# PRBonn/semantic_suma

Hardware: NVIDIA B200
Metric: scans_per_sec (higher is better)
Workload: dtype f32

## Files before the change

include/suma_b200.h:

```cpp
#ifndef SUMA_B200_H_
#define SUMA_B200_H_

#include <stdint.h>

#ifdef __cplusplus
extern "C" {
#endif

#define SB_VERSION 100

typedef enum sb_status {
  SB_OK = 0,
  SB_ERR_INVALID = -1,
  SB_ERR_CUDA = -2,
  SB_ERR_NOMEM = -3,
  SB_ERR_CAPACITY = -4,
  SB_ERR_STATE = -5,
  SB_ERR_NOGPU = -6
} sb_status;

typedef struct sb_params {
  int32_t data_width, data_height;
  float data_fov_up, data_fov_down;
  float min_depth, max_depth;
  int32_t model_width, model_height;
  float model_fov_up, model_fov_down;
  float model_min_depth, model_max_depth;
  int32_t max_iterations;
  double stopping_threshold, delta;
  float icp_max_distance, icp_max_angle;
  int32_t weighting;
  float factor;
  int32_t initialize_identity;
  int32_t bilinear_sampling;
  int32_t fallback_mode;
  float fallback_max_distance, fallback_max_angle;
  int32_t compose_rendering;
  float max_loop_closure_distance;
  float min_radius, max_radius, max_angle;
  float map_max_distance, map_max_angle;
  int32_t unstable_age, confidence_mode;
  float confidence_threshold;
  float p_stable, p_prior, sigma_angle, sigma_distance;
  int32_t use_stability, active_timestamps;
  float max_weight;
  int32_t weighting_scheme, averaging_scheme, update_always;
  int32_t submap_dimension;
  float submap_extent;
  int32_t partial_extraction;
  int32_t label_offset_quirk;
  int32_t render_after_update;
} sb_params;

typedef struct sb_surfel {
  float x, y, z, radius;
  float nx, ny, nz, confidence;
  uint32_t timestamp;
  float color, weight, count;
  float r, g, b, w;
} sb_surfel;

typedef struct sb_ctx sb_ctx;
typedef struct sb_frame sb_frame;

enum { SB_MAP_VERTEX = 0, SB_MAP_NORMAL = 1, SB_MAP_SEMANTIC = 2 };
enum { SB_FRAME_OLD = 0, SB_FRAME_NEW = 1, SB_FRAME_COMPOSED = 2 };
enum { SB_SLAM_CURRENT = 0, SB_SLAM_LAST = 1, SB_SLAM_CURRENT_MODEL = 2, SB_SLAM_LAST_MODEL = 3 };

int sb_default_params(sb_params* p);
int sb_create(const sb_params* p, int device, sb_ctx** out);
int sb_destroy(sb_ctx* ctx);
int sb_reset(sb_ctx* ctx);
int sb_set_params(sb_ctx* ctx, const sb_params* p);
const char* sb_last_error(const sb_ctx* ctx);
int sb_synchronize(sb_ctx* ctx);
int sb_device_count(void);
void* sb_stream(sb_ctx* ctx);
uint64_t sb_launch_count(const sb_ctx* ctx);

int sb_frame_create(sb_ctx* ctx, int width, int height, sb_frame** out);
int sb_frame_destroy(sb_frame* f);
int sb_frame_copy(sb_frame* dst, const sb_frame* src);
int sb_frame_download(const sb_frame* f, int which, float* dst );
int sb_frame_upload(sb_frame* f, int which, const float* src );
int sb_frame_size(const sb_frame* f, int* width, int* height);

int sb_preprocess(sb_ctx* ctx, const float* pts4, const float* labels, const float* probs, uint32_t n,
                  uint32_t timestamp, int pts_on_device, sb_frame* out);

int sb_map_render(sb_ctx* ctx, const float pose_old[16], const float pose_new[16], float conf_thr, sb_frame* out);
int sb_map_render_active(sb_ctx* ctx, const float pose[16], float conf_thr);
int sb_map_render_inactive(sb_ctx* ctx, const float pose[16], float conf_thr);
int sb_map_render_composed(sb_ctx* ctx, const float pose_old[16], const float pose_new[16], float conf_thr);
int sb_map_frame(sb_ctx* ctx, int which, sb_frame** out);

int sb_icp_jacobian(sb_ctx* ctx, const sb_frame* data, const sb_frame* model, const double pose[16], int iteration,
                    float max_distance, float max_angle_deg, int row_begin, int row_end, double out48[48],
                    int64_t raw32[32]);
void sb_icp_unpack(const int64_t raw32[32], double out48[48]);

int sb_icp_minimize(sb_ctx* ctx, const sb_frame* data, const sb_frame* model, const double T0[16], int max_iter,
                    double eps, double delta, float max_distance, float max_angle_deg, double pose_out[16],
                    double out48[48], int* iters, double* history, int* history_len);
void sb_se3_exp(const double x[6], double T[16]);
void sb_se3_log(const double T[16], double x[6]);
int sb_ldlt_solve6(const double A[36], const double b[6], double x[6]);
int sb_gn_step(const double out48[48], double last_error, double eps, double delta, double pose[16], double dx[6]);

int sb_map_update(sb_ctx* ctx, const float pose[16], const sb_frame* frame);
int sb_map_update_poses(sb_ctx* ctx, const float* poses16, uint32_t count);
int sb_map_size(sb_ctx* ctx, uint32_t* n);
int sb_map_timestamp(sb_ctx* ctx, uint32_t* t);
int sb_map_download(sb_ctx* ctx, sb_surfel* dst, uint32_t cap, uint32_t* n);
int sb_map_upload(sb_ctx* ctx, const sb_surfel* src, uint32_t n, uint32_t timestamp);
int sb_map_set_pose(sb_ctx* ctx, uint32_t t, const float pose[16]);
int sb_map_update_debug(sb_ctx* ctx, uint32_t* index_map, float* radius_map4, uint8_t* integrated,
                        uint32_t* n_updated, uint32_t* n_new);
int sb_map_submap_origin(sb_ctx* ctx, int32_t* i, int32_t* j, uint32_t* pending);

int sb_process_scan(sb_ctx* ctx, const float* pts4, const float* labels, const float* probs, uint32_t n,
                    int pts_on_device);
int sb_prefetch_scan(sb_ctx* ctx, const float* pts4, const float* labels, const float* probs, uint32_t n);
typedef struct sb_loop_params {
  float search_distance;
  float min_trajectory_distance;
  int32_t min_verifications;
  float residual_threshold;
  float outlier_threshold;
  float valid_threshold;
} sb_loop_params;
typedef struct sb_loop_info {
  uint32_t enabled, loop_count, time_without_loop_closure, candidates_tested, loop_edges_added, unverified;
  uint32_t already_verified, found_candidate, use_candidate, optimisation_requested;
  int32_t last_added_candidate;
  uint32_t n_edges, n_poses;
  float valid_ratio, outlier_ratio, rel_error;
  double residual_old, residual_new;
  double current_pose_old[16];
} sb_loop_info;
typedef struct sb_loop_edge {
  int32_t from, to;
  double rel_pose[16];
} sb_loop_edge;
void sb_default_loop_params(sb_loop_params* p);
int sb_set_loop_closure(sb_ctx* ctx, int enabled, const sb_loop_params* p );
int sb_get_loop_info(sb_ctx* ctx, sb_loop_info* out);
int sb_get_loop_edges(sb_ctx* ctx, sb_loop_edge* dst, uint32_t cap, uint32_t* n_total);
int sb_integrate_loop_closures(sb_ctx* ctx, const double* poses16, uint32_t n, uint32_t* integrated);
int sb_set_current_pose(sb_ctx* ctx, const double pose[16]);

int sb_get_pose(sb_ctx* ctx, double pose[16]);
int sb_get_last_pose(sb_ctx* ctx, double pose[16]);
int sb_timestamp(sb_ctx* ctx, uint32_t* t);
int sb_slam_frame(sb_ctx* ctx, int which, sb_frame** out);
int sb_get_statistics(sb_ctx* ctx, double stats[16]);

int sb_profile_enable(sb_ctx* ctx, int on);
int sb_profile_kernels(void);
const char* sb_profile_name(int id);
int sb_profile_collect(sb_ctx* ctx, double* total_ms, uint64_t* count, int cap);

int sb_comm_export(sb_ctx* ctx, uint8_t handle[64]);
int sb_comm_init(sb_ctx* ctx, int rank, int nranks, const uint8_t* handles , int row_begin,
                 int row_end);
int sb_comm_shutdown(sb_ctx* ctx);
typedef int (*sb_allreduce_fn)(void* user, int64_t* sums32);
int sb_comm_set_callback(sb_ctx* ctx, sb_allreduce_fn fn, void* user, int row_begin, int row_end);

#ifdef __cplusplus
}
#endif
#endif
```

semantic_suma_b200/api.py:

```python
import ctypes as C
import os

import numpy as np

from . import build as _build

SB_OK = 0
_ERRORS = {-1: "SB_ERR_INVALID", -2: "SB_ERR_CUDA", -3: "SB_ERR_NOMEM", -4: "SB_ERR_CAPACITY", -5: "SB_ERR_STATE",
           -6: "SB_ERR_NOGPU"}


class SumaError(RuntimeError):
    pass


class LoopParams(C.Structure):
    _fields_ = [("search_distance", C.c_float), ("min_trajectory_distance", C.c_float), ("min_verifications", C.c_int32),
                ("residual_threshold", C.c_float), ("outlier_threshold", C.c_float), ("valid_threshold", C.c_float)]


class LoopInfo(C.Structure):
    _fields_ = [(n, C.c_uint32) for n in ("enabled", "loop_count", "time_without_loop_closure", "candidates_tested",
                                          "loop_edges_added", "unverified", "already_verified", "found_candidate",
                                          "use_candidate", "optimisation_requested")] + \
               [("last_added_candidate", C.c_int32), ("n_edges", C.c_uint32), ("n_poses", C.c_uint32),
                ("valid_ratio", C.c_float), ("outlier_ratio", C.c_float), ("rel_error", C.c_float),
                ("residual_old", C.c_double), ("residual_new", C.c_double), ("current_pose_old", C.c_double * 16)]


class LoopEdge(C.Structure):
    _fields_ = [("from_", C.c_int32), ("to", C.c_int32), ("rel_pose", C.c_double * 16)]


class Params(C.Structure):
    _fields_ = [
        ("data_width", C.c_int32), ("data_height", C.c_int32),
        ("data_fov_up", C.c_float), ("data_fov_down", C.c_float),
        ("min_depth", C.c_float), ("max_depth", C.c_float),
        ("model_width", C.c_int32), ("model_height", C.c_int32),
        ("model_fov_up", C.c_float), ("model_fov_down", C.c_float),
        ("model_min_depth", C.c_float), ("model_max_depth", C.c_float),
        ("max_iterations", C.c_int32),
        ("stopping_threshold", C.c_double), ("delta", C.c_double),
        ("icp_max_distance", C.c_float), ("icp_max_angle", C.c_float),
        ("weighting", C.c_int32), ("factor", C.c_float),
        ("initialize_identity", C.c_int32), ("bilinear_sampling", C.c_int32),
        ("fallback_mode", C.c_int32),
        ("fallback_max_distance", C.c_float), ("fallback_max_angle", C.c_float),
        ("compose_rendering", C.c_int32), ("max_loop_closure_distance", C.c_float),
        ("min_radius", C.c_float), ("max_radius", C.c_float), ("max_angle", C.c_float),
        ("map_max_distance", C.c_float), ("map_max_angle", C.c_float),
        ("unstable_age", C.c_int32), ("confidence_mode", C.c_int32),
        ("confidence_threshold", C.c_float),
        ("p_stable", C.c_float), ("p_prior", C.c_float), ("sigma_angle", C.c_float), ("sigma_distance", C.c_float),
        ("use_stability", C.c_int32), ("active_timestamps", C.c_int32),
        ("max_weight", C.c_float),
        ("weighting_scheme", C.c_int32), ("averaging_scheme", C.c_int32), ("update_always", C.c_int32),
        ("submap_dimension", C.c_int32), ("submap_extent", C.c_float), ("partial_extraction", C.c_int32),
        ("label_offset_quirk", C.c_int32), ("render_after_update", C.c_int32),
    ]

    def as_dict(self):
        return {k: getattr(self, k) for k, _ in self._fields_}


XML_KEYS = {
    "max iterations": "max_iterations", "stopping threshold": "stopping_threshold", "icp-max-distance": "icp_max_distance",
    "icp-max-angle": "icp_max_angle", "fallback-max-distance": "fallback_max_distance",
    "fallback-max-angle": "fallback_max_angle", "map-max-distance": "map_max_distance",
    "map-max-angle": "map_max_angle", "submap-dimension": "submap_dimension", "submap-extent": "submap_extent",
    "partial-extraction": "partial_extraction",
}
_WEIGHTING = {"none": 0, "huber": 1, "turkey": 2, "stability": 3}

SURFEL_DTYPE = np.dtype([
    ("x", "f4"), ("y", "f4"), ("z", "f4"), ("radius", "f4"),
    ("nx", "f4"), ("ny", "f4"), ("nz", "f4"), ("confidence", "f4"),
    ("timestamp", "u4"), ("color", "f4"), ("weight", "f4"), ("count", "f4"),
    ("r", "f4"), ("g", "f4"), ("b", "f4"), ("w", "f4"),
])

_lib = None


def library_path():
    return _build.LIB


def lib(build_if_missing=True):
    global _lib
    if _lib is not None:
        return _lib
    path = _build.LIB
    if build_if_missing:
        try:
            path = _build.build()
        except Exception as e:
            if not os.path.exists(_build.LIB):
                raise SumaError("libsuma_b200.so is missing and could not be built: %s" % e)
    if not os.path.exists(path):
        raise SumaError("libsuma_b200.so not found at %s (run python -m semantic_suma_b200.build)" % path)
    L = C.CDLL(path)
    vp, u32, i32, f32, f64 = C.c_void_p, C.c_uint32, C.c_int32, C.c_float, C.c_double
    pf, pd, pv = C.POINTER(C.c_float), C.POINTER(C.c_double), C.POINTER(C.c_void_p)
    sig = {
        "sb_default_params": [C.POINTER(Params)],
        "sb_create": [C.POINTER(Params), C.c_int, pv],
        "sb_destroy": [vp], "sb_reset": [vp], "sb_set_params": [vp, C.POINTER(Params)], "sb_synchronize": [vp],
        "sb_frame_create": [vp, C.c_int, C.c_int, pv], "sb_frame_destroy": [vp], "sb_frame_copy": [vp, vp],
        "sb_frame_download": [vp, C.c_int, vp], "sb_frame_upload": [vp, C.c_int, vp],
        "sb_frame_size": [vp, C.POINTER(C.c_int), C.POINTER(C.c_int)],
        "sb_preprocess": [vp, vp, vp, vp, u32, u32, C.c_int, vp],
        "sb_map_render": [vp, pf, pf, f32, vp], "sb_map_render_active": [vp, pf, f32],
        "sb_map_render_inactive": [vp, pf, f32], "sb_map_render_composed": [vp, pf, pf, f32],
        "sb_map_frame": [vp, C.c_int, pv],
        "sb_icp_jacobian": [vp, vp, vp, pd, C.c_int, f32, f32, C.c_int, C.c_int, pd, C.POINTER(C.c_int64)],
        "sb_icp_minimize": [vp, vp, vp, pd, C.c_int, f64, f64, f32, f32, pd, pd, C.POINTER(C.c_int), pd,
                            C.POINTER(C.c_int)],
        "sb_gn_step": [pd, f64, f64, f64, pd, pd],
        "sb_ldlt_solve6": [pd, pd, pd],
        "sb_map_update": [vp, pf, vp], "sb_map_update_poses": [vp, pf, u32], "sb_map_set_pose": [vp, u32, pf],
        "sb_map_size": [vp, C.POINTER(u32)], "sb_map_timestamp": [vp, C.POINTER(u32)],
        "sb_map_download": [vp, vp, u32, C.POINTER(u32)], "sb_map_upload": [vp, vp, u32, u32],
        "sb_map_update_debug": [vp, vp, vp, vp, C.POINTER(u32), C.POINTER(u32)],
        "sb_map_submap_origin": [vp, C.POINTER(i32), C.POINTER(i32), C.POINTER(u32)],
        "sb_process_scan": [vp, vp, vp, vp, u32, C.c_int], "sb_prefetch_scan": [vp, vp, vp, vp, u32],
        "sb_set_loop_closure": [vp, C.c_int, vp], "sb_get_loop_info": [vp, vp], "sb_get_loop_edges": [vp, vp, u32, C.POINTER(u32)],
        "sb_set_current_pose": [vp, pd], "sb_default_loop_params": [vp],
        "sb_integrate_loop_closures": [vp, pd, u32, C.POINTER(u32)],
        "sb_get_pose": [vp, pd], "sb_get_last_pose": [vp, pd], "sb_timestamp": [vp, C.POINTER(u32)], "sb_slam_frame": [vp, C.c_int, pv],
        "sb_get_statistics": [vp, pd],
        "sb_comm_export": [vp, vp], "sb_comm_init": [vp, C.c_int, C.c_int, vp, C.c_int, C.c_int],
        "sb_comm_shutdown": [vp],
        "sb_comm_set_callback": [vp, vp, vp, C.c_int, C.c_int],
        "sb_profile_enable": [vp, C.c_int], "sb_profile_collect": [vp, pd, C.POINTER(C.c_uint64), C.c_int],
        "sb_profile_kernels": [],
    }
    for name, args in sig.items():
        fn = getattr(L, name)
        fn.argtypes = args
        fn.restype = C.c_int
    L.sb_last_error.argtypes = [vp]; L.sb_last_error.restype = C.c_char_p
    L.sb_stream.argtypes = [vp]; L.sb_stream.restype = vp
    L.sb_launch_count.argtypes = [vp]; L.sb_launch_count.restype = C.c_uint64
    L.sb_device_count.argtypes = []; L.sb_device_count.restype = C.c_int
    L.sb_profile_name.argtypes = [C.c_int]; L.sb_profile_name.restype = C.c_char_p
    L.sb_se3_exp.argtypes = [pd, pd]; L.sb_se3_exp.restype = None
    L.sb_se3_log.argtypes = [pd, pd]; L.sb_se3_log.restype = None
    L.sb_icp_unpack.argtypes = [C.POINTER(C.c_int64), pd]; L.sb_icp_unpack.restype = None
    _lib = L
    return L


EXPORTED_SYMBOLS = [
    "sb_default_params", "sb_create", "sb_destroy", "sb_reset", "sb_set_params", "sb_last_error", "sb_synchronize",
    "sb_device_count", "sb_stream", "sb_launch_count", "sb_frame_create", "sb_frame_destroy", "sb_frame_copy",
    "sb_frame_download", "sb_frame_upload", "sb_frame_size", "sb_preprocess", "sb_map_render", "sb_map_render_active",
    "sb_map_render_inactive", "sb_map_render_composed", "sb_map_frame", "sb_icp_jacobian", "sb_icp_unpack",
    "sb_icp_minimize", "sb_se3_exp", "sb_se3_log", "sb_ldlt_solve6", "sb_gn_step", "sb_map_update",
    "sb_map_update_poses", "sb_map_size", "sb_map_timestamp", "sb_map_download", "sb_map_upload", "sb_map_set_pose",
    "sb_map_update_debug", "sb_map_submap_origin", "sb_process_scan", "sb_prefetch_scan", "sb_get_pose", "sb_get_last_pose", "sb_timestamp", "sb_slam_frame",
    "sb_get_statistics", "sb_comm_export", "sb_comm_init", "sb_comm_shutdown", "sb_comm_set_callback",
    "sb_profile_enable", "sb_default_loop_params", "sb_set_loop_closure", "sb_get_loop_info", "sb_get_loop_edges",
    "sb_set_current_pose", "sb_integrate_loop_closures",
    "sb_profile_kernels", "sb_profile_name", "sb_profile_collect",
]


def default_params(**kw):
    p = Params()
    lib().sb_default_params(C.byref(p))
    for k, v in kw.items():
        k = XML_KEYS.get(k, k)
        if k == "weighting" and isinstance(v, str):
            v = _WEIGHTING[v]
        if not hasattr(p, k):
            raise KeyError(k)
        setattr(p, k, v)
    return p


def colmajor(T, dtype):
    return np.ascontiguousarray(np.asarray(T, dtype=dtype).T).reshape(16)


def from_colmajor(a):
    return np.asarray(a).reshape(4, 4).T.copy()


def _fp(a):
    return a.ctypes.data_as(C.POINTER(C.c_float))


def _dp(a):
    return a.ctypes.data_as(C.POINTER(C.c_double))


def _vp(a):
    if a is None:
        return None
    return C.c_void_p(a.ctypes.data)


class Context:

    def __init__(self, params, device=0):
        self.params = params
        self.h = C.c_void_p()
        rc = lib().sb_create(C.byref(params), device, C.byref(self.h))
        if rc != SB_OK:
            raise SumaError("sb_create failed: %s (libsuma_b200 needs a CUDA device; there is no CPU fallback)" %
                            _ERRORS.get(rc, rc))

    def check(self, rc, what=""):
        if rc != SB_OK:
            msg = lib().sb_last_error(self.h)
            raise SumaError("%s: %s %s" % (what, _ERRORS.get(rc, rc), msg.decode() if msg else ""))

    def close(self):
        if self.h:
            lib().sb_destroy(self.h)
            self.h = C.c_void_p()

    def __del__(self):
        try:
            self.close()
        except Exception:
            pass

    def synchronize(self):
        self.check(lib().sb_synchronize(self.h), "synchronize")

    def launch_count(self):
        return int(lib().sb_launch_count(self.h))

    def stream(self):
        return lib().sb_stream(self.h)

    def profile(self, on):
        self.check(lib().sb_profile_enable(self.h, 1 if on else 0), "profile_enable")

    def profile_collect(self):
        n = lib().sb_profile_kernels()
        ms = np.zeros(n); cnt = np.zeros(n, np.uint64)
        self.check(lib().sb_profile_collect(self.h, _dp(ms), cnt.ctypes.data_as(C.POINTER(C.c_uint64)), n), "profile")
        return {lib().sb_profile_name(i).decode(): (float(ms[i]), int(cnt[i])) for i in range(n) if cnt[i]}

    def set_params(self, params):
        self.check(lib().sb_set_params(self.h, C.byref(params)), "set_params")
        self.params = params


class Frame:

    def __init__(self, ctx, width=None, height=None, handle=None):
        self.ctx = ctx
        self._own = handle is None
        if handle is None:
            self.h = C.c_void_p()
            ctx.check(lib().sb_frame_create(ctx.h, width, height, C.byref(self.h)), "frame_create")
        else:
            self.h = C.c_void_p(handle)
        w, h = C.c_int(), C.c_int()
        lib().sb_frame_size(self.h, C.byref(w), C.byref(h))
        self.width, self.height = w.value, h.value

    def __del__(self):
        if getattr(self, "_own", False) and self.h and self.ctx.h:
            lib().sb_frame_destroy(self.h)
            self.h = None

    def _get(self, which):
        a = np.empty((self.height, self.width, 4), np.float32)
        self.ctx.check(lib().sb_frame_download(self.h, which, _vp(a)), "frame_download")
        return a

    def _set(self, which, a):
        a = np.ascontiguousarray(a, np.float32)
        assert a.shape == (self.height, self.width, 4)
        self.ctx.check(lib().sb_frame_upload(self.h, which, _vp(a)), "frame_upload")

    vertex_map = property(lambda s: s._get(0), lambda s, a: s._set(0, a))
    normal_map = property(lambda s: s._get(1), lambda s, a: s._set(1, a))
    semantic_map = property(lambda s: s._get(2), lambda s, a: s._set(2, a))

    def maps(self):
        return self._get(0), self._get(1), self._get(2)

    def upload(self, maps):
        for i, a in enumerate(maps):
            self._set(i, a)

    def copy(self, other):
        self.ctx.check(lib().sb_frame_copy(self.h, other.h), "frame_copy")


class Preprocessing:

    def __init__(self, ctx):
        self.ctx = ctx

    def process(self, points, frame, labels=None, probs=None, timestamp=100):
        pts = np.ascontiguousarray(points, np.float32)
        lab = None if labels is None else np.ascontiguousarray(labels, np.float32)
        prb = None if probs is None else np.ascontiguousarray(probs, np.float32)
        self.ctx.check(lib().sb_preprocess(self.ctx.h, _vp(pts), _vp(lab), _vp(prb), pts.shape[0], timestamp, 0, frame.h),
                       "preprocess")


class Frame2Model:

    def __init__(self, ctx, max_distance=None, max_angle=None):
        self.ctx = ctx
        p = ctx.params
        self.max_distance = p.icp_max_distance if max_distance is None else max_distance
        self.max_angle = p.icp_max_angle if max_angle is None else max_angle
        self.pose_ = np.eye(4)
        self.iteration_ = 0
        self.current = self.last = None
        self.out48 = np.zeros(48)
        self.raw32 = np.zeros(32, np.int64)

    def setData(self, current, last):
        self.current, self.last = current, last
        self.iteration_ = 0

    def initialize(self, T0):
        self.pose_ = np.array(T0, np.float64)

    def num_parameters(self):
        return 6

    def jacobianProducts(self, rows=None):
        pc = colmajor(self.pose_, np.float64)
        r0, r1 = rows if rows is not None else (0, self.ctx.params.data_height)
        self.ctx.check(lib().sb_icp_jacobian(self.ctx.h, self.current.h, self.last.h, _dp(pc), self.iteration_,
                                             self.max_distance, self.max_angle, r0, r1, _dp(self.out48),
                                             self.raw32.ctypes.data_as(C.POINTER(C.c_int64))), "icp_jacobian")
        o = self.out48
        return o[43], o[:36].reshape(6, 6).T.copy(), o[36:42].copy()

    def increment(self, delta):
        T = np.zeros(16)
        d = np.ascontiguousarray(delta, np.float64)
        lib().sb_se3_exp(_dp(d), _dp(T))
        self.pose_ = from_colmajor(T) @ self.pose_
        self.iteration_ += 1

    def pose(self):
        return self.pose_

    def valid(self):
        return int(self.out48[42])

    def outlier(self):
        return int(self.out48[44])

    def inlier(self):
        return int(self.out48[42]) - int(self.out48[44])

    def invalid(self):
        return int(self.out48[46])

    def inlier_residual(self):
        return float(np.float32(self.out48[45]))


class LieGaussNewton:

    def __init__(self, ctx):
        self.ctx = ctx
        p = ctx.params
        self.maxIter, self.epsilon, self.delta = p.max_iterations, p.stopping_threshold, p.delta
        self.Tk_ = np.eye(4)
        self.k_ = 0
        self.history_ = []
        self.out48 = np.zeros(48)

    def minimize(self, F, T0):
        T0c = colmajor(T0, np.float64)
        pose = np.zeros(16); out48 = np.zeros(48); it = C.c_int(0); hl = C.c_int(0)
        bounded = 1 <= self.maxIter <= 256
        hist = np.zeros((self.maxIter + 1) * 16 if bounded else 16)
        self.ctx.check(lib().sb_icp_minimize(self.ctx.h, F.current.h, F.last.h, _dp(T0c), self.maxIter, self.epsilon,
                                             self.delta, F.max_distance, F.max_angle, _dp(pose), _dp(out48),
                                             C.byref(it), _dp(hist) if bounded else None, C.byref(hl)), "icp_minimize")
        if not bounded:
            hl.value = 0
        self.Tk_ = from_colmajor(pose)
        self.k_ = it.value
        self.out48 = out48
        self.history_ = [from_colmajor(hist[16 * i:16 * i + 16]) for i in range(hl.value)]
        F.pose_ = self.Tk_.copy()
        F.out48 = out48
        return 0

    def minimize_host(self, F, T0):
        F.initialize(T0)
        last_error = float(np.finfo(np.float32).max)
        self.history_ = []
        k = 0
        while True:
            self.history_.append(F.pose().copy())
            if self.maxIter > 0 and k >= self.maxIter:
                break
            F.jacobianProducts()
            pose = colmajor(F.pose_, np.float64); dx = np.zeros(6)
            res = lib().sb_gn_step(_dp(F.out48), last_error, self.epsilon, self.delta, _dp(pose), _dp(dx))
            F.pose_ = from_colmajor(pose)
            F.iteration_ += 1
            last_error = F.out48[43]
            if res == 0:
                break
            k += 1
        self.Tk_, self.k_ = F.pose_.copy(), k
        return 0

    def pose(self):
        return self.Tk_

    def iterationCount(self):
        return self.k_

    def history(self):
        return self.history_


class SurfelMap:

    def __init__(self, ctx):
        self.ctx = ctx

    def update(self, pose, frame):
        pc = colmajor(pose, np.float32)
        self.ctx.check(lib().sb_map_update(self.ctx.h, _fp(pc), frame.h), "map_update")

    def render(self, pose_old, pose_new, frame, confidence_threshold):
        po, pn = colmajor(pose_old, np.float32), colmajor(pose_new, np.float32)
        self.ctx.check(lib().sb_map_render(self.ctx.h, _fp(po), _fp(pn), confidence_threshold, frame.h), "map_render")

    def render_active(self, pose, confidence_threshold):
        pc = colmajor(pose, np.float32)
        self.ctx.check(lib().sb_map_render_active(self.ctx.h, _fp(pc), confidence_threshold), "render_active")

    def render_inactive(self, pose, confidence_threshold):
        pc = colmajor(pose, np.float32)
        self.ctx.check(lib().sb_map_render_inactive(self.ctx.h, _fp(pc), confidence_threshold), "render_inactive")

    def render_composed(self, pose_old, pose_new, confidence_threshold):
        po, pn = colmajor(pose_old, np.float32), colmajor(pose_new, np.float32)
        self.ctx.check(lib().sb_map_render_composed(self.ctx.h, _fp(po), _fp(pn), confidence_threshold), "render_composed")

    def _frame(self, which):
        h = C.c_void_p()
        self.ctx.check(lib().sb_map_frame(self.ctx.h, which, C.byref(h)), "map_frame")
        return Frame(self.ctx, handle=h.value)

    def oldMapFrame(self):
        return self._frame(0)

    def newMapFrame(self):
        return self._frame(1)

    def composedFrame(self):
        return self._frame(2)

    def size(self):
        n = C.c_uint32()
        lib().sb_map_size(self.ctx.h, C.byref(n))
        return n.value

    def timestamp(self):
        n = C.c_uint32()
        lib().sb_map_timestamp(self.ctx.h, C.byref(n))
        return n.value

    def getAllSurfels(self):
        n = self.size()
        a = np.zeros(max(n, 1), SURFEL_DTYPE)
        k = C.c_uint32()
        self.ctx.check(lib().sb_map_download(self.ctx.h, _vp(a), n, C.byref(k)), "map_download")
        return a[:k.value]

    def upload(self, surfels, timestamp):
        a = np.ascontiguousarray(surfels, SURFEL_DTYPE)
        self.ctx.check(lib().sb_map_upload(self.ctx.h, _vp(a), a.shape[0], timestamp), "map_upload")

    def set_pose(self, t, pose):
        pc = colmajor(pose, np.float32)
        self.ctx.check(lib().sb_map_set_pose(self.ctx.h, t, _fp(pc)), "map_set_pose")

    def updatePoses(self, poses):
        a = np.ascontiguousarray(np.stack([colmajor(p, np.float32) for p in poses]), np.float32)
        self.ctx.check(lib().sb_map_update_poses(self.ctx.h, _fp(a), len(poses)), "update_poses")

    def update_debug(self):
        H, W = self.ctx.params.data_height, self.ctx.params.data_width
        idx = np.zeros((H, W), np.uint32); rad = np.zeros((H, W, 4), np.float32); integ = np.zeros((H, W), np.uint8)
        nu, nn = C.c_uint32(), C.c_uint32()
        self.ctx.check(lib().sb_map_update_debug(self.ctx.h, _vp(idx), _vp(rad), _vp(integ), C.byref(nu), C.byref(nn)),
                       "update_debug")
        return idx, rad, integ, nu.value, nn.value

    def submap_origin(self):
        i, j, p = C.c_int32(), C.c_int32(), C.c_uint32()
        lib().sb_map_submap_origin(self.ctx.h, C.byref(i), C.byref(j), C.byref(p))
        return i.value, j.value, p.value

    def reset(self):
        self.ctx.check(lib().sb_reset(self.ctx.h), "reset")


class SurfelMapping:

    def __init__(self, params, device=0):
        self.ctx = Context(params, device)
        self.map_ = SurfelMap(self.ctx)

    def enableLoopClosure(self, enabled=True, **kw):
        lp = LoopParams()
        lib().sb_default_loop_params(C.byref(lp))
        for k, v in kw.items():
            if not hasattr(lp, k):
                raise KeyError(k)
            setattr(lp, k, v)
        self.ctx.check(lib().sb_set_loop_closure(self.ctx.h, 1 if enabled else 0, C.byref(lp)), "set_loop_closure")

    def getLoopInfo(self):
        li = LoopInfo()
        self.ctx.check(lib().sb_get_loop_info(self.ctx.h, C.byref(li)), "get_loop_info")
        d = {n: getattr(li, n) for n, _ in LoopInfo._fields_ if n != "current_pose_old"}
        d["valid_ratio"] = np.float32(d["valid_ratio"]); d["outlier_ratio"] = np.float32(d["outlier_ratio"])
        d["rel_error"] = np.float32(d["rel_error"])
        d["current_pose_old"] = from_colmajor(np.array(li.current_pose_old))
        return d

    def getLoopEdges(self):
        n = C.c_uint32(0)
        self.ctx.check(lib().sb_get_loop_edges(self.ctx.h, None, 0, C.byref(n)), "get_loop_edges")
        arr = (LoopEdge * max(n.value, 1))()
        self.ctx.check(lib().sb_get_loop_edges(self.ctx.h, arr, n.value, C.byref(n)), "get_loop_edges")
        return [(arr[i].from_, arr[i].to, from_colmajor(np.array(arr[i].rel_pose))) for i in range(n.value)]

    def integrateLoopClosures(self, poses=None):
        n = C.c_uint32(0)
        if poses is None:
            self.ctx.check(lib().sb_integrate_loop_closures(self.ctx.h, None, 0, C.byref(n)), "integrate_loop_closures")
        else:
            a = np.ascontiguousarray([colmajor(P, np.float64) for P in poses], np.float64)
            self.ctx.check(lib().sb_integrate_loop_closures(self.ctx.h, _dp(a), a.shape[0], C.byref(n)),
                           "integrate_loop_closures")
        return int(n.value)

    def setCurrentPose(self, pose):
        self.ctx.check(lib().sb_set_current_pose(self.ctx.h, _dp(colmajor(pose, np.float64))), "set_current_pose")

    def processScan(self, points, labels=None, probs=None, on_device=False):
        if on_device:
            pp, pl, pq, n = points
            rc = lib().sb_process_scan(self.ctx.h, C.c_void_p(pp), C.c_void_p(pl) if pl else None,
                                       C.c_void_p(pq) if pq else None, n, 1)
        else:
            pts = np.ascontiguousarray(points, np.float32)
            lab = None if labels is None else np.ascontiguousarray(labels, np.float32)
            prb = None if probs is None else np.ascontiguousarray(probs, np.float32)
            rc = lib().sb_process_scan(self.ctx.h, _vp(pts), _vp(lab), _vp(prb), pts.shape[0], 0)
        self.ctx.check(rc, "process_scan")

    def process_scan_raw(self, ptr_pts, ptr_labels, ptr_probs, n, on_device):
        rc = lib().sb_process_scan(self.ctx.h, C.c_void_p(ptr_pts), C.c_void_p(ptr_labels) if ptr_labels else None,
                                   C.c_void_p(ptr_probs) if ptr_probs else None, n, 1 if on_device else 0)
        self.ctx.check(rc, "process_scan")

    def prefetch_scan_raw(self, ptr_pts, ptr_labels, ptr_probs, n):
        rc = lib().sb_prefetch_scan(self.ctx.h, C.c_void_p(ptr_pts), C.c_void_p(ptr_labels) if ptr_labels else None,
                                    C.c_void_p(ptr_probs) if ptr_probs else None, n)
        self.ctx.check(rc, "prefetch_scan")

    def getCurrentPose(self):
        a = np.zeros(16)
        lib().sb_get_pose(self.ctx.h, _dp(a))
        return from_colmajor(a)

    def getLastPose(self):
        a = np.zeros(16)
        lib().sb_get_last_pose(self.ctx.h, _dp(a))
        return from_colmajor(a)

    def timestamp(self):
        t = C.c_uint32()
        lib().sb_timestamp(self.ctx.h, C.byref(t))
        return t.value

    def getMap(self):
        return self.map_

    def _frame(self, which):
        h = C.c_void_p()
        self.ctx.check(lib().sb_slam_frame(self.ctx.h, which, C.byref(h)), "slam_frame")
        return Frame(self.ctx, handle=h.value)

    def getCurrentFrame(self):
        return self._frame(0)

    def getLastFrame(self):
        return self._frame(1)

    def getCurrentModelFrame(self):
        return self._frame(2)

    def getLastModelFrame(self):
        return self._frame(3)

    def getStatistics(self):
        a = np.zeros(16)
        lib().sb_get_statistics(self.ctx.h, _dp(a))
        return {"num_iterations": a[0], "F": a[1], "inlier": a[2], "outlier": a[3], "invalid": a[4],
                "inlier_residual": a[5], "track_loss": a[6], "surfels": a[7], "preprocessing-time": a[8],
                "icp-time": a[9], "mapping-time": a[10], "complete-time": a[11]}

    def reset(self):
        self.ctx.check(lib().sb_reset(self.ctx.h), "reset")
```

semantic_suma_b200/csrc/sb_api.cu:

```cuda
#include <chrono>
#include <cmath>
#include <cstddef>
#include <cstdio>
#include <cstdlib>
#include <map>
#include <string>
#include <utility>
#include <vector>

#include "sb_gn.cuh"
#include "sb_internal.cuh"
#include "../../include/suma_b200_loop.hpp"

using namespace sb;

struct sb_frame {
  sb_ctx* ctx;
  FrameDev d;
  float4* base;
};

struct DevTile {
  uint32_t slot = 0;
  bool known = false;
  uint32_t base = 0, count = 0;
};

struct sb_ctx {
  int device = 0;
  int sm_count = 148;
  cudaStream_t stream = nullptr;
  sb_params p;
  KParams kp;
  std::string err;
  uint64_t launches = 0;
  Profiler prof;

  PrepKeys prep;
  bool prepped_for_update = false;
  float4* d_pts = nullptr;
  float* d_labels = nullptr;
  float* d_probs = nullptr;
  size_t pts_cap = 0;
  struct PrefetchSlot {
    float4* pts = nullptr;
    float* labels = nullptr;
    float* probs = nullptr;
    const float* host_pts = nullptr;
    uint32_t n = 0;
    bool has_labels = false, has_probs = false, valid = false, in_use = false;
    cudaEvent_t done = nullptr;
    cudaEvent_t released = nullptr;
    bool has_released = false;
  };
  PrefetchSlot prefetch[3];
  cudaStream_t copy_stream = nullptr;

  GnState* gn = nullptr;
  GnState* gn2 = nullptr;
  long long* acc32 = nullptr;
  long long* acc_slots = nullptr;
  unsigned int* ticket = nullptr;
  void* h_pinned = nullptr;
  int icp_blocks = 296;
  int icp_coop_blocks = 0;
  unsigned int epoch_base = 1;
  unsigned long long* gn_pub = nullptr;
  int gn_use_cache = 1;
  bool close_loops = false;
  suma_b200::loop::State loop;
  double lastPose_old[16];

  SurfelPlanes A{}, T{}, G{}, X{};
  uint8_t* keep = nullptr;
  uint32_t* block_counts = nullptr;
  uint32_t* block_offsets = nullptr;
  unsigned long long* lb_desc = nullptr;
  uint32_t* lb_ticket = nullptr;
  uint32_t lb_gen = 0;
  uint32_t* d_counts = nullptr;
  float* poses = nullptr;
  float* poses_inv = nullptr;
  std::vector<float> h_poses, h_poses_inv;
  float* Mtab_old = nullptr;
  float* Mtab_new = nullptr;
  unsigned long long* key_old = nullptr;
  unsigned long long* key_new = nullptr;
  unsigned long long* key_comp = nullptr;
  unsigned long long* key_index = nullptr;
  float4* radius_map = nullptr;
  uint8_t* integrated = nullptr;
  uint32_t* group_counts = nullptr;
  sb_frame* f_old = nullptr;
  sb_frame* f_new = nullptr;
  sb_frame* f_comp = nullptr;
  uint32_t n_host = 0;
  uint32_t n_upper = 0;
  char* result_block = nullptr;
  PoseDev* pd = nullptr;
  uint32_t n_updated = 0, n_new = 0;
  uint32_t map_timestamp = 0;
  int32_t origin_i = 0, origin_j = 0;
  std::vector<std::pair<int32_t, int32_t>> extraction;
  std::map<std::pair<int32_t, int32_t>, DevTile> tiles;
  SurfelPlanes pool{};
  uint32_t* d_pool_top = nullptr;
  uint2* d_tile_rec = nullptr;
  uint32_t n_slots = 0;
  bool tiles_pending = false;

  struct RenderKey {
    float pose_old[16], pose_new[16];
    float conf_thr;
    uint32_t map_timestamp;
    uint64_t map_version;
    int compose;
    const sb_frame* out;
  } rkey{};
  bool rkey_valid = false;
  uint64_t map_version = 0;
  uint64_t renders_skipped = 0;

  sb_frame* cur = nullptr;
  sb_frame* last = nullptr;
  sb_frame* cur_model = nullptr;
  sb_frame* last_model = nullptr;
  uint32_t timestamp = 0;
  double currentPose[16], lastPose[16], currentPose_old[16], currentPose_new[16], lastIncrement[16];
  float confidence_threshold = 0.f, log_unstable_slam = 0.f;
  double stats[16];
  uint32_t trackLoss = 0;
  bool cur_has_semantics = false, last_has_semantics = false;

  long long* mailbox = nullptr;
  unsigned int* comm_epoch = nullptr;
  CommDev comm{};
  bool comm_on = false;
  sb_allreduce_fn comm_cb = nullptr;
  void* comm_cb_user = nullptr;
  int row_begin = 0, row_end = 0;
  std::vector<void*> peer_ptrs;
};

namespace {

int fail(sb_ctx* c, int code, const std::string& msg) {
  if (c) c->err = msg;
  return code;
}

#define SB_CUDA(ctx, call)                                                                              \
  do {                                                                                                  \
    cudaError_t e__ = (call);                                                                           \
    if (e__ != cudaSuccess)                                                                             \
      return fail(ctx, SB_ERR_CUDA, std::string(#call) + ": " + cudaGetErrorString(e__));               \
  } while (0)

Launch L_(sb_ctx* c) { return Launch{c->stream, &c->launches, &c->prof}; }

void ident_d(double* M) {
  for (int i = 0; i < 16; ++i) M[i] = (i % 5 == 0) ? 1.0 : 0.0;
}
Mat4 mat4_from(const float* m) {
  Mat4 r;
  memcpy(r.m, m, 64);
  return r;
}
void cast_f(const double* M, float* F) {
  for (int i = 0; i < 16; ++i) F[i] = (float)M[i];
}
double now_s() {
  return std::chrono::duration<double>(std::chrono::steady_clock::now().time_since_epoch()).count();
}
float deg2rad_f(float d) { return d * (float)(3.14159265358979323846 / 180.0); }

void derive(sb_ctx* c) {
  const sb_params& p = c->p;
  KParams& k = c->kp;
  memset(&k, 0, sizeof(k));
  k.W = p.data_width; k.H = p.data_height; k.Wm = p.model_width; k.Hm = p.model_height;
  k.fov_up = fabsf(p.data_fov_up); k.fov = fabsf(p.data_fov_up) + fabsf(p.data_fov_down);
  k.min_depth = p.min_depth; k.max_depth = p.max_depth;
  k.m_fov_up = fabsf(p.model_fov_up); k.m_fov = fabsf(p.model_fov_up) + fabsf(p.model_fov_down);
  k.m_min_depth = p.model_min_depth; k.m_max_depth = p.model_max_depth;
  k.weighting = p.weighting; k.bilinear = p.bilinear_sampling; k.factor = p.factor;
  k.use_stability = p.use_stability; k.unstable_age = p.unstable_age; k.confidence_mode = p.confidence_mode;
  k.active_timestamps = p.active_timestamps; k.weighting_scheme = p.weighting_scheme;
  k.averaging_scheme = p.averaging_scheme; k.update_always = p.update_always;
  k.confidence_threshold = p.confidence_threshold; k.p_stable = p.p_stable;
  k.p_unstable = 1.0f - p.p_stable;
  k.log_prior = (float)log(p.p_prior / (1.0 - p.p_prior));
  k.log_unstable = (float)log(k.p_unstable / (1.0 - k.p_unstable));
  k.sigma_angle = p.sigma_angle; k.sigma_distance = p.sigma_distance; k.max_weight = p.max_weight;
  float vfov = fabsf(p.data_fov_up) + fabsf(p.data_fov_down);
  float vpix = (float)tan(0.5f * ((double)vfov * 3.14159265358979323846 / 180.0) / (uint32_t)p.data_height);
  float hpix = (float)tan(0.5f * ((double)360.0f * 3.14159265358979323846 / 180.0) / (uint32_t)p.data_width);
  k.pixel_size = vpix > hpix ? vpix : hpix;
  k.min_radius = p.min_radius; k.max_radius = p.max_radius;
  k.radconf_angle_thresh = (float)cos((double)deg2rad_f(p.max_angle));
  k.update_angle_thresh = (float)sin((double)deg2rad_f(p.map_max_angle));
  k.map_max_distance = p.map_max_distance;
  k.max_loop_closure_distance = p.max_loop_closure_distance;
  k.label_offset_quirk = p.label_offset_quirk;
  c->confidence_threshold = p.confidence_threshold;
  float pu = 0.1f;
  c->log_unstable_slam = logf(pu / (1.0f - pu));
}

int alloc_planes(sb_ctx* c, SurfelPlanes* s, size_t n) {
  float4* base = nullptr;
  SB_CUDA(c, cudaMalloc(&base, n * 4 * sizeof(float4)));
  s->p0 = base; s->p1 = base + n; s->p2 = base + 2 * n; s->p3 = base + 3 * n;
  return SB_OK;
}
void free_planes(SurfelPlanes* s) {
  if (s->p0) cudaFree(s->p0);
  s->p0 = s->p1 = s->p2 = s->p3 = nullptr;
}

int frame_create(sb_ctx* c, int w, int h, sb_frame** out) {
  if (!c || w <= 0 || h <= 0 || !out) return fail(c, SB_ERR_INVALID, "frame_create: bad arguments");
  sb_frame* f = new sb_frame();
  f->ctx = c;
  size_t P = (size_t)w * h;
  cudaError_t e = cudaMalloc(&f->base, P * 3 * sizeof(float4));
  if (e != cudaSuccess) {
    delete f;
    return fail(c, SB_ERR_NOMEM, std::string("frame alloc: ") + cudaGetErrorString(e));
  }
  cudaMemsetAsync(f->base, 0, P * 3 * sizeof(float4), c->stream);
  f->d.W = w; f->d.H = h;
  f->d.vertex = f->base; f->d.normal = f->base + P; f->d.semantic = f->base + 2 * P;
  *out = f;
  return SB_OK;
}

int release_buffers(sb_ctx* c) {
  cudaFree(c->prep.img[0]); cudaFree(c->prep.img[1]);
  cudaFree(c->d_pts); cudaFree(c->d_labels); cudaFree(c->d_probs);
  cudaFree(c->gn); cudaFree(c->gn2); cudaFree(c->acc_slots); cudaFree(c->ticket); cudaFree(c->gn_pub);
  if (c->h_pinned) cudaFreeHost(c->h_pinned);
  free_planes(&c->A); free_planes(&c->T); free_planes(&c->G); free_planes(&c->X); free_planes(&c->pool);
  cudaFree(c->d_pool_top); cudaFree(c->d_tile_rec);
  cudaFree(c->keep); cudaFree(c->block_counts); cudaFree(c->block_offsets);
  cudaFree(c->lb_desc); cudaFree(c->lb_ticket);
  cudaFree(c->poses); cudaFree(c->poses_inv); cudaFree(c->Mtab_old); cudaFree(c->Mtab_new);
  cudaFree(c->key_old); cudaFree(c->key_index); cudaFree(c->radius_map); cudaFree(c->integrated); cudaFree(c->group_counts);
  sb_frame* fr[] = {c->f_old, c->f_new, c->f_comp, c->cur, c->last, c->cur_model, c->last_model};
  for (sb_frame* f : fr)
    if (f) {
      cudaFree(f->base);
      delete f;
    }
  cudaFree(c->mailbox);
  cudaFree(c->comm_epoch);
  cudaFree(c->result_block);
  return SB_OK;
}

int reset_state(sb_ctx* c) {
  c->rkey_valid = false;
  c->map_version += 1;
  c->n_host = 0; c->n_updated = 0; c->n_new = 0; c->map_timestamp = 0;
  c->origin_i = c->origin_j = 0;
  c->extraction.clear();
  c->tiles.clear();
  c->n_slots = 0;
  c->tiles_pending = false;
  c->stats[12] = 0.0;
  c->loop.reset();
  for (int i = 0; i < 16; ++i) c->lastPose_old[i] = (i % 5 == 0) ? 1.0 : 0.0;
  SB_CUDA(c, cudaMemsetAsync(c->d_pool_top, 0, 64, c->stream));
  c->h_poses.assign((size_t)kMaxPoses * 16, 0.0f);
  for (uint32_t t = 0; t < kMaxPoses; ++t)
    for (int i = 0; i < 4; ++i) c->h_poses[16 * (size_t)t + 5 * i] = 1.0f;
  c->h_poses_inv = c->h_poses;
  SB_CUDA(c, cudaMemcpyAsync(c->poses, c->h_poses.data(), (size_t)kMaxPoses * 64, cudaMemcpyHostToDevice, c->stream));
  SB_CUDA(c, cudaMemcpyAsync(c->poses_inv, c->h_poses.data(), (size_t)kMaxPoses * 64, cudaMemcpyHostToDevice, c->stream));
  SB_CUDA(c, cudaMemsetAsync(c->d_counts, 0, 16 * sizeof(uint32_t), c->stream));
  c->timestamp = 0;
  ident_d(c->currentPose); ident_d(c->lastPose); ident_d(c->currentPose_old); ident_d(c->currentPose_new);
  ident_d(c->lastIncrement);
  memset(c->stats, 0, sizeof(c->stats));
  c->trackLoss = 0;
  c->n_upper = 0;
  {
    static_assert(sizeof(PoseDev) <= 4096, "pinned staging");
    PoseDev& h = *reinterpret_cast<PoseDev*>(c->h_pinned);
    memset(&h, 0, sizeof(h));
    ident_d(h.currentPose); ident_d(h.lastPose); ident_d(h.lastIncrement); ident_d(h.increment); ident_d(h.T0);
    for (int i = 0; i < 4; ++i) h.P_active.m[5 * i] = h.invP_active.m[5 * i] = h.P_cur.m[5 * i] = h.invP_cur.m[5 * i] = 1.0f;
    SB_CUDA(c, cudaMemcpyAsync(c->pd, &h, sizeof(h), cudaMemcpyHostToDevice, c->stream));
  }
  c->cur_has_semantics = c->last_has_semantics = false;
  sb_frame* fr[] = {c->f_old, c->f_new, c->f_comp, c->cur, c->last, c->cur_model, c->last_model};
  for (sb_frame* f : fr)
    if (f) SB_CUDA(c, cudaMemsetAsync(f->base, 0, (size_t)f->d.W * f->d.H * 3 * sizeof(float4), c->stream));
  SB_CUDA(c, cudaStreamSynchronize(c->stream));
  return SB_OK;
}

int alloc_buffers(sb_ctx* c) {
  const sb_params& p = c->p;
  size_t Pd = (size_t)p.data_width * p.data_height, Pm = (size_t)p.model_width * p.model_height;
  static_assert(sizeof(PoseDev) <= 4096, "PoseDev must fit the first page of the result block");
  SB_CUDA(c, cudaMalloc(&c->result_block, 8192 + 64));
  SB_CUDA(c, cudaMemsetAsync(c->result_block, 0, 8192 + 64, c->stream));
  c->pd = reinterpret_cast<PoseDev*>(c->result_block);
  c->acc32 = reinterpret_cast<long long*>(c->result_block + 4096);
  c->d_counts = reinterpret_cast<uint32_t*>(c->result_block + 8192);
  const size_t Pk = preprocess_key_elems(p.data_width, p.data_height);
  for (int i = 0; i < 2; ++i) {
    SB_CUDA(c, cudaMalloc(&c->prep.img[i], Pk * 8));
    c->prep.tmap_ok[i] = make_key_tensor_map(&c->prep.tmap[i], c->prep.img[i], p.data_width, p.data_height);
  }
  c->prep.use_tma = true;
  if (const char* e = getenv("SUMA_B200_PREP_TMA")) c->prep.use_tma = atoi(e) != 0;
  c->pts_cap = Pd * 2 + 1024;
  SB_CUDA(c, cudaMalloc(&c->d_pts, c->pts_cap * 16));
  SB_CUDA(c, cudaMalloc(&c->d_labels, c->pts_cap * 4));
  SB_CUDA(c, cudaMalloc(&c->d_probs, c->pts_cap * 4));
  SB_CUDA(c, cudaMalloc(&c->gn, sizeof(GnState)));
  SB_CUDA(c, cudaMalloc(&c->gn2, sizeof(GnState)));
  SB_CUDA(c, cudaMemsetAsync(c->gn2, 0, sizeof(GnState), c->stream));
  SB_CUDA(c, cudaMalloc(&c->acc_slots, 1024 * 32 * sizeof(long long)));
  SB_CUDA(c, cudaMemsetAsync(c->acc_slots, 0, 1024 * 32 * sizeof(long long), c->stream));
  SB_CUDA(c, cudaMalloc(&c->ticket, 128));
  SB_CUDA(c, cudaMalloc(&c->gn_pub, 64 * 8));
  SB_CUDA(c, cudaMemsetAsync(c->gn_pub, 0, 64 * 8, c->stream));
  if (const char* e = getenv("SUMA_B200_GN_CACHE")) c->gn_use_cache = atoi(e) != 0;
  SB_CUDA(c, cudaMemsetAsync(c->ticket, 0, 128, c->stream));
  SB_CUDA(c, cudaMallocHost(&c->h_pinned, 65536));
  int r;
  if ((r = alloc_planes(c, &c->A, kMaxSurfels))) return r;
  if ((r = alloc_planes(c, &c->T, kMaxSurfels))) return r;
  if ((r = alloc_planes(c, &c->G, Pd))) return r;
  if ((r = alloc_planes(c, &c->X, 16))) return r;
  if ((r = alloc_planes(c, &c->pool, kTilePoolCap))) return r;
  SB_CUDA(c, cudaMalloc(&c->d_pool_top, 64));
  SB_CUDA(c, cudaMalloc(&c->d_tile_rec, (size_t)kMaxTileSlots * sizeof(uint2)));
  SB_CUDA(c, cudaMalloc(&c->keep, kMaxSurfels));
  size_t nb = (kMaxSurfels + 127) / 128 + 16;
  SB_CUDA(c, cudaMalloc(&c->block_counts, nb * 4));
  SB_CUDA(c, cudaMalloc(&c->block_offsets, nb * 4));
  SB_CUDA(c, cudaMalloc(&c->lb_desc, (nb + 16) * 8));
  SB_CUDA(c, cudaMemsetAsync(c->lb_desc, 0, (nb + 16) * 8, c->stream));
  SB_CUDA(c, cudaMalloc(&c->lb_ticket, 64));
  SB_CUDA(c, cudaMemsetAsync(c->lb_ticket, 0, 64, c->stream));
  SB_CUDA(c, cudaMalloc(&c->poses, (size_t)kMaxPoses * 64));
  SB_CUDA(c, cudaMalloc(&c->poses_inv, (size_t)kMaxPoses * 64));
  SB_CUDA(c, cudaMalloc(&c->Mtab_old, (size_t)kMaxPoses * 64));
  SB_CUDA(c, cudaMalloc(&c->Mtab_new, (size_t)kMaxPoses * 64));
  SB_CUDA(c, cudaMalloc(&c->key_old, Pm * 8 * 3));
  c->key_new = c->key_old + Pm;
  c->key_comp = c->key_old + 2 * Pm;
  SB_CUDA(c, cudaMemsetAsync(c->key_old, 0xff, Pm * 8 * 3, c->stream));
  for (int i = 0; i < 2; ++i)
    SB_CUDA(c, cudaMemsetAsync(c->prep.img[i], 0xff, preprocess_key_elems(c->p.data_width, c->p.data_height) * 8, c->stream));
  c->prep.cur = 0;
  SB_CUDA(c, cudaMalloc(&c->key_index, Pd * 8));
  SB_CUDA(c, cudaMalloc(&c->radius_map, Pd * 16));
  SB_CUDA(c, cudaMalloc(&c->integrated, Pd));
  SB_CUDA(c, cudaMalloc(&c->group_counts, kGroupCounts * 4));
  SB_CUDA(c, cudaMemsetAsync(c->group_counts, 0, kGroupCounts * 4, c->stream));
  SB_CUDA(c, cudaMalloc(&c->comm_epoch, 64));
  SB_CUDA(c, cudaMemsetAsync(c->comm_epoch, 0, 64, c->stream));
  if ((r = frame_create(c, p.model_width, p.model_height, &c->f_old))) return r;
  if ((r = frame_create(c, p.model_width, p.model_height, &c->f_new))) return r;
  if ((r = frame_create(c, p.model_width, p.model_height, &c->f_comp))) return r;
  if ((r = frame_create(c, p.data_width, p.data_height, &c->cur))) return r;
  if ((r = frame_create(c, p.data_width, p.data_height, &c->last))) return r;
  if ((r = frame_create(c, p.model_width, p.model_height, &c->cur_model))) return r;
  if ((r = frame_create(c, p.model_width, p.model_height, &c->last_model))) return r;
  return reset_state(c);
}

uint32_t n_grid(const sb_ctx* c) { return c->n_upper > c->n_host ? c->n_upper : c->n_host; }

int t_threshold(const sb_ctx* c) { return (int)(c->map_timestamp - kComposeAge); }

uint32_t pose_table_count(const sb_ctx* c) {
  uint32_t n = c->map_timestamp + 1;
  return n < kMaxPoses ? n : kMaxPoses;
}

int set_pose_entry(sb_ctx* c, uint32_t t, const float* pose) {
  c->map_version += 1;
  if (t >= kMaxPoses) return fail(c, SB_ERR_CAPACITY, "pose table full (10000 poses, SurfelMap.h:205)");
  memcpy(&c->h_poses[16 * (size_t)t], pose, 64);
  sbg::rigid_inverse_f(pose, &c->h_poses_inv[16 * (size_t)t]);
  SB_CUDA(c, cudaMemcpyAsync(c->poses + 16 * (size_t)t, &c->h_poses[16 * (size_t)t], 64, cudaMemcpyHostToDevice, c->stream));
  SB_CUDA(c, cudaMemcpyAsync(c->poses_inv + 16 * (size_t)t, &c->h_poses_inv[16 * (size_t)t], 64, cudaMemcpyHostToDevice,
                             c->stream));
  return SB_OK;
}

FrameDev null_frame() {
  FrameDev f;
  f.W = f.H = 0;
  f.vertex = f.normal = f.semantic = nullptr;
  return f;
}

int render_full(sb_ctx* c, const float* pose_old, const float* pose_new, float conf_thr, sb_frame* out,
                const Mat4* inv_dev = nullptr, bool table_ready = false) {
  if (!inv_dev && c->rkey_valid && c->rkey.out == out && c->rkey.map_version == c->map_version &&
      c->rkey.map_timestamp == c->map_timestamp && c->rkey.compose == c->p.compose_rendering &&
      memcmp(&c->rkey.conf_thr, &conf_thr, 4) == 0 && memcmp(c->rkey.pose_old, pose_old, 64) == 0 &&
      memcmp(c->rkey.pose_new, pose_new, 64) == 0) {
    c->renders_skipped += 1;
    return SB_OK;
  }
  const KParams& kp = c->kp;
  Launch L = L_(c);
  size_t Pm = (size_t)kp.Wm * kp.Hm;
  float inv_old[16] = {0}, inv_new[16] = {0};
  if (!inv_dev) {
    sbg::rigid_inverse_f(pose_old, inv_old);
    sbg::rigid_inverse_f(pose_new, inv_new);
  }
  const bool same = inv_dev != nullptr || memcmp(pose_old, pose_new, 64) == 0;
  uint32_t np = pose_table_count(c);
  if (!table_ready) launch_pose_products(L, mat4_from(inv_old), inv_dev, c->poses, c->Mtab_old, np);
  float* Mnew = c->Mtab_old;
  if (!same) {
    launch_pose_products(L, mat4_from(inv_new), nullptr, c->poses, c->Mtab_new, np);
    Mnew = c->Mtab_new;
  }
  if (c->p.compose_rendering) {
    RenderTargets t{c->key_old, c->key_new, nullptr};
    int thr = t_threshold(c);
    if (same) {
      launch_render_scatter(L, kp, c->A, c->d_counts, n_grid(c), c->Mtab_old, conf_thr, thr, 1, 1, 0, t);
    } else {
      RenderTargets to{c->key_old, nullptr, nullptr}, tn{nullptr, c->key_new, nullptr};
      launch_render_scatter(L, kp, c->A, c->d_counts, n_grid(c), c->Mtab_old, conf_thr, thr, 1, 0, 0, to);
      launch_render_scatter(L, kp, c->A, c->d_counts, n_grid(c), Mnew, conf_thr, thr, 0, 1, 0, tn);
    }
    launch_render_resolve(L, kp, c->A, c->Mtab_old, Mnew, t, c->f_old->d, c->f_new->d, c->f_comp->d, out->d, null_frame(), 0, 0);
  } else {
    RenderTargets t{nullptr, c->key_new, nullptr};
    launch_render_scatter(L, kp, c->A, c->d_counts, n_grid(c), c->Mtab_old, conf_thr, 0, 0, 1, 0, t);
    launch_render_resolve(L, kp, c->A, c->Mtab_old, c->Mtab_old, t, null_frame(), c->f_new->d, null_frame(), null_frame(),
                          null_frame(), 0, 0);
    SB_CUDA(c, cudaMemcpyAsync(c->f_old->base, c->f_new->base, Pm * 48, cudaMemcpyDeviceToDevice, c->stream));
    SB_CUDA(c, cudaMemcpyAsync(out->base, c->f_new->base, Pm * 48, cudaMemcpyDeviceToDevice, c->stream));
  }
  if (inv_dev) {
    c->rkey_valid = false;
    return SB_OK;
  }
  memcpy(c->rkey.pose_old, pose_old, 64);
  memcpy(c->rkey.pose_new, pose_new, 64);
  c->rkey.conf_thr = conf_thr;
  c->rkey.map_timestamp = c->map_timestamp;
  c->rkey.map_version = c->map_version;
  c->rkey.compose = c->p.compose_rendering;
  c->rkey.out = out;
  c->rkey_valid = true;
  return SB_OK;
}

int render_single(sb_ctx* c, const float* pose, float conf_thr, int which, const Mat4* inv_dev = nullptr,
                  bool table_ready = false, sb_frame* copy_to = nullptr) {
  c->rkey_valid = false;
  const KParams& kp = c->kp;
  Launch L = L_(c);
  size_t Pm = (size_t)kp.Wm * kp.Hm;
  float inv[16] = {0};
  if (pose) sbg::rigid_inverse_f(pose, inv);
  if (!table_ready) launch_pose_products(L, mat4_from(inv), inv_dev, c->poses, c->Mtab_old, pose_table_count(c));
  unsigned long long* key = which ? c->key_new : c->key_old;
  RenderTargets t{which ? nullptr : key, which ? key : nullptr, nullptr};
  launch_render_scatter(L, kp, c->A, c->d_counts, n_grid(c), c->Mtab_old, conf_thr, t_threshold(c), which ? 0 : 1,
                        which ? 1 : 0, 0, t);
  launch_render_resolve(L, kp, c->A, c->Mtab_old, c->Mtab_old, t, c->f_old->d, c->f_new->d, null_frame(), null_frame(),
                        (copy_to && which) ? copy_to->d : null_frame(), 1, 0);
  if (copy_to && !which)
    SB_CUDA(c, cudaMemcpyAsync(copy_to->base, c->f_old->base, Pm * 48, cudaMemcpyDeviceToDevice, c->stream));
  return SB_OK;
}

int gn_fail(sb_ctx* c) {
  cudaMemsetAsync(c->ticket, 0, 128, c->stream);
  cudaMemsetAsync(c->acc_slots, 0, 1024 * 32 * sizeof(long long), c->stream);
  cudaMemsetAsync(&c->pd->gn_error, 0, sizeof(int), c->stream);
  cudaStreamSynchronize(c->stream);
  return fail(c, SB_ERR_STATE, "Gauss-Newton kernel timed out waiting for a block or a peer GPU");
}

unsigned int next_epoch_base(sb_ctx* c, int max_iter) {
  unsigned int b = c->epoch_base;
  c->epoch_base += (unsigned int)max_iter + 8u;
  return b;
}

IcpArgs icp_args(sb_ctx* c, const sb_frame* data, const sb_frame* model, float max_distance, float max_angle_deg,
                 int row_begin, int row_end, bool semantics) {
  IcpArgs a;
  a.data_v = data->d.vertex; a.data_n = data->d.normal; a.data_s = data->d.semantic;
  a.model_v = model->d.vertex; a.model_n = model->d.normal; a.model_s = model->d.semantic;
  a.distance_thresh = max_distance;
  a.angle_thresh = (float)cos((double)max_angle_deg * 3.14159265358979323846 / 180.0);
  a.row_begin = row_begin; a.row_end = row_end;
  a.has_semantics = semantics ? 1 : 0;
  a.Wm = model->d.W; a.Hm = model->d.H;
  {
    int rows = row_end - row_begin;
    int step = (int)(rows * 0.6180339887) | 1;
    auto gcd = [](int x, int y) { while (y) { int t = x % y; x = y; y = t; } return x; };
    while (rows > 1 && gcd(step, rows) != 1) step += 2;
    a.row_step = rows > 1 ? step % rows : 1;
    if (a.row_step == 0) a.row_step = 1;
  }
  return a;
}

int icp_check(sb_ctx* c, const sb_frame* data, const sb_frame* model) {
  if (!c || !data || !model) return fail(c, SB_ERR_INVALID, "icp: null argument");
  const bool model_ok = (model->d.W == c->kp.Wm && model->d.H == c->kp.Hm) || (model->d.W == c->kp.W && model->d.H == c->kp.H);
  if (data->d.W != c->kp.W || data->d.H != c->kp.H || !model_ok)
    return fail(c, SB_ERR_INVALID, "icp: frame size does not match data_/model_ width/height");
  return SB_OK;
}

int icp_jacobian_raw(sb_ctx* c, const sb_frame* data, const sb_frame* model, const double* pose, int iteration,
                     float max_distance, float max_angle_deg, int r0, int r1, bool semantics, long long* raw) {
  IcpArgs a = icp_args(c, data, model, max_distance, max_angle_deg, r0, r1, semantics);
  Mat4 P;
  for (int i = 0; i < 16; ++i) P.m[i] = (float)pose[i];
  launch_icp_jacobian(L_(c), c->kp, a, P, iteration, c->acc32, c->acc_slots, c->ticket + 16, c->icp_blocks);
  SB_CUDA(c, cudaMemcpyAsync(c->h_pinned, c->acc32, 32 * sizeof(long long), cudaMemcpyDeviceToHost, c->stream));
  SB_CUDA(c, cudaStreamSynchronize(c->stream));
  memcpy(raw, c->h_pinned, 32 * sizeof(long long));
  return SB_OK;
}

struct GnHead {
  double pose[16];
  double last_error;
  double out48[48];
  int k, done, history_len, error;
};

int icp_minimize_callback(sb_ctx* c, const sb_frame* data, const sb_frame* model, const double* T0, int max_iter,
                          double eps, double delta, float max_distance, float max_angle_deg, bool semantics) {
  const bool striped = c->comm_cb != nullptr;
  IcpArgs a = icp_args(c, data, model, max_distance, max_angle_deg, striped ? c->row_begin : 0, striped ? c->row_end : c->kp.H,
                       semantics);
  std::vector<double> hist;
  GnHead h;
  memset(&h, 0, sizeof(h));
  memcpy(h.pose, T0, sizeof(h.pose));
  h.last_error = (double)3.402823466e+38f;
  int k = 0;
  for (;;) {
    hist.insert(hist.end(), h.pose, h.pose + 16);
    if (k >= max_iter) break;
    Mat4 P;
    for (int i = 0; i < 16; ++i) P.m[i] = (float)h.pose[i];
    launch_icp_jacobian(L_(c), c->kp, a, P, k, c->acc32, c->acc_slots, c->ticket + 16, c->icp_blocks);
    SB_CUDA(c, cudaMemcpyAsync(c->h_pinned, c->acc32, 32 * sizeof(long long), cudaMemcpyDeviceToHost, c->stream));
    SB_CUDA(c, cudaStreamSynchronize(c->stream));
    long long raw[32];
    memcpy(raw, c->h_pinned, sizeof(raw));
    if (c->comm_cb && c->comm_cb(c->comm_cb_user, (int64_t*)raw) != 0) return fail(c, SB_ERR_STATE, "all-reduce callback failed");
    sbg::unpack48(raw, h.out48);
    double dx[6];
    int result = sbg::gn_step(h.out48, h.last_error, eps, delta, h.pose, dx);
    h.last_error = h.out48[43];
    if (result == 0) break;
    ++k;
  }
  h.k = k;
  h.done = 1;
  size_t hb = hist.size() * sizeof(double);
  if (hb > 32768) hb = 32768;
  h.history_len = (int)(hb / 128);
  char* hp = (char*)c->h_pinned + 16384;
  memcpy(hp, &h, sizeof(h));
  memcpy(hp + 1024, hist.data(), hb);
  SB_CUDA(c, cudaMemcpyAsync(c->gn, hp, sizeof(h), cudaMemcpyHostToDevice, c->stream));
  SB_CUDA(c, cudaMemcpyAsync((char*)c->gn + offsetof(GnState, history), hp + 1024, hb, cudaMemcpyHostToDevice, c->stream));
  SB_CUDA(c, cudaStreamSynchronize(c->stream));
  return SB_OK;
}

int icp_minimize_enqueue(sb_ctx* c, const sb_frame* data, const sb_frame* model, const double* T0, int max_iter,
                         double eps, double delta, float max_distance, float max_angle_deg, bool semantics) {
  if (max_iter <= 0 || max_iter > kMaxGnIter) max_iter = kMaxGnIter;
  if (c->comm_cb) return icp_minimize_callback(c, data, model, T0, max_iter, eps, delta, max_distance, max_angle_deg, semantics);
  int r0 = 0, r1 = c->kp.H;
  if (c->comm_on) {
    r0 = c->row_begin;
    r1 = c->row_end;
  }
  if (const char* dr = getenv("SUMA_B200_DEBUG_ROWS")) {
    int a0 = 0, a1 = 0;
    if (sscanf(dr, "%d,%d", &a0, &a1) == 2 && a0 >= 0 && a1 <= c->kp.H && a0 < a1) {
      r0 = a0;
      r1 = a1;
    }
  }
  IcpArgs a = icp_args(c, data, model, max_distance, max_angle_deg, r0, r1, semantics);
  Mat4d T;
  memcpy(T.m, T0, sizeof(T.m));
  Launch L = L_(c);
  if (c->icp_coop_blocks > 0) {
    launch_gn_init(L, c->gn, T, c->acc32);
    GnJob job;
    memset(&job, 0, sizeof(job));
    job.mode = GN_PLAIN;
    job.a = a;
    job.st = c->gn;
    job.max_iter = max_iter;
    job.eps = eps;
    job.delta = delta;
    job.epoch_base = next_epoch_base(c, max_iter);
    job.use_cache = c->gn_use_cache;
    if (launch_gn_persistent(L, c->kp, job, c->acc_slots, c->ticket, c->gn_pub, c->comm_on ? &c->comm : nullptr,
                             c->icp_coop_blocks) == 0)
      return SB_OK;
    cudaGetLastError();
    c->icp_coop_blocks = 0;
  }
  if (c->comm_on) return fail(c, SB_ERR_STATE, "the fused peer exchange needs a cooperative launch");
  return icp_minimize_callback(c, data, model, T0, max_iter, eps, delta, max_distance, max_angle_deg, semantics);
}

int icp_minimize_fetch(sb_ctx* c, double* pose_out, double* out48, int* iters, double* history, int* history_len) {
  SB_CUDA(c, cudaMemcpyAsync(c->h_pinned, c->gn, sizeof(GnHead), cudaMemcpyDeviceToHost, c->stream));
  SB_CUDA(c, cudaStreamSynchronize(c->stream));
  GnHead h;
  memcpy(&h, c->h_pinned, sizeof(h));
  if (h.error) return gn_fail(c);
  if (pose_out) memcpy(pose_out, h.pose, sizeof(h.pose));
  if (out48) memcpy(out48, h.out48, sizeof(h.out48));
  if (iters) *iters = h.k;
  if (history_len) *history_len = h.history_len;
  if (history && h.history_len > 0) {
    SB_CUDA(c, cudaMemcpy(history, (const char*)c->gn + offsetof(GnState, history), (size_t)h.history_len * 128,
                          cudaMemcpyDeviceToHost));
  }
  return SB_OK;
}

float2 submap_center(const sb_ctx* c, int32_t i, int32_t j) {
  return make_float2((float)(2.0 * i * c->p.submap_extent), (float)(2.0 * j * c->p.submap_extent));
}

int fetch_counts(sb_ctx* c, uint32_t* dst, int n) {
  SB_CUDA(c, cudaMemcpyAsync(c->h_pinned, c->d_counts, n * sizeof(uint32_t), cudaMemcpyDeviceToHost, c->stream));
  SB_CUDA(c, cudaStreamSynchronize(c->stream));
  memcpy(dst, c->h_pinned, n * sizeof(uint32_t));
  return SB_OK;
}

int refresh_tile_records(sb_ctx* c) {
  if (!c->tiles_pending || c->n_slots == 0) return SB_OK;
  std::vector<uint2> rec(c->n_slots);
  SB_CUDA(c, cudaMemcpyAsync(rec.data(), c->d_tile_rec, (size_t)c->n_slots * sizeof(uint2), cudaMemcpyDeviceToHost,
                             c->stream));
  SB_CUDA(c, cudaStreamSynchronize(c->stream));
  {
    uint32_t top[2] = {0, 0};
    SB_CUDA(c, cudaMemcpy(top, c->d_pool_top, sizeof(top), cudaMemcpyDeviceToHost));
    if (top[1] != (uint32_t)c->stats[12]) {
      c->stats[12] = top[1];
      c->err = "submap tile pool exhausted: " + std::to_string(top[1]) + " surfels of leaving tiles were dropped";
    }
  }
  for (auto& kv : c->tiles) {
    DevTile& t = kv.second;
    if (!t.known) {
      t.base = rec[t.slot].x;
      t.count = rec[t.slot].y;
      t.known = true;
    }
  }
  c->tiles_pending = false;
  return SB_OK;
}

int append_tiles(sb_ctx* c, int32_t i0, int32_t j0, int di, int dj) {
  const int dim = c->p.submap_dimension;
  int r;
  bool appended = false;
  for (int32_t k = -dim; k <= dim; ++k) {
    auto it = c->tiles.find(std::make_pair(i0 + di * k, j0 + dj * k));
    if (it == c->tiles.end()) continue;
    if (!it->second.known && (r = refresh_tile_records(c))) return r;
    const DevTile& t = it->second;
    uint32_t room = kMaxSurfels - c->n_host;
    uint32_t n = t.count < room ? t.count : room;
    if (n == 0) continue;
    SB_CUDA(c, cudaMemcpyAsync(c->A.p0 + c->n_host, c->pool.p0 + t.base, (size_t)n * 16, cudaMemcpyDeviceToDevice, c->stream));
    SB_CUDA(c, cudaMemcpyAsync(c->A.p1 + c->n_host, c->pool.p1 + t.base, (size_t)n * 16, cudaMemcpyDeviceToDevice, c->stream));
    SB_CUDA(c, cudaMemcpyAsync(c->A.p2 + c->n_host, c->pool.p2 + t.base, (size_t)n * 16, cudaMemcpyDeviceToDevice, c->stream));
    SB_CUDA(c, cudaMemcpyAsync(c->A.p3 + c->n_host, c->pool.p3 + t.base, (size_t)n * 16, cudaMemcpyDeviceToDevice, c->stream));
    c->n_host += n;
    c->n_upper = c->n_host;
    appended = true;
  }
  if (appended) {
    SB_CUDA(c, cudaMemcpyAsync(c->d_counts, &c->n_host, 4, cudaMemcpyHostToDevice, c->stream));
    SB_CUDA(c, cudaStreamSynchronize(c->stream));
  }
  return SB_OK;
}

int extract_surfels(sb_ctx* c, bool partially) {
  Launch L = L_(c);
  while (!c->extraction.empty()) {
    std::pair<int32_t, int32_t> idx = c->extraction.back();
    c->extraction.pop_back();
    if (c->n_slots >= kMaxTileSlots) return fail(c, SB_ERR_CAPACITY, "tile cache: out of record slots");
    float2 ctr = submap_center(c, idx.first, idx.second);
    uint32_t slot = c->n_slots++;
    launch_extract_to_pool(L, c->A, c->d_counts, c->n_host, c->poses, ctr, c->p.submap_extent, c->keep, c->block_counts,
                           c->block_offsets, c->pool, kTilePoolCap, c->d_pool_top, c->d_tile_rec + slot, kExtractCap);
    DevTile t;
    t.slot = slot;
    t.known = false;
    c->tiles[idx] = t;
    c->tiles_pending = true;
    if (partially) break;
  }
  return SB_OK;
}

int update_active_submaps(sb_ctx* c, const float* pose) {
  const int dim = c->p.submap_dimension;
  const float ext = c->p.submap_extent;
  float2 ctr = submap_center(c, c->origin_i, c->origin_j);
  float changex = pose[12] - ctr.x, changey = pose[13] - ctr.y;
  float factor = 1.1f;
  int r;
  if (fabsf(changex) > factor * ext || fabsf(changey) > factor * ext) {
    if (fabsf(changex) > factor * ext) {
      int dir = changex < 0 ? -1 : 1;
      for (int32_t k = -dim; k <= dim; ++k) c->extraction.push_back(std::make_pair(c->origin_i - dir * dim, c->origin_j + k));
      c->origin_i += dir;
      if ((r = append_tiles(c, c->origin_i + dir * dim, c->origin_j, 0, 1))) return r;
    }
    if (fabsf(changey) > factor * ext) {
      int dir = changey < 0 ? -1 : 1;
      for (int32_t k = -dim; k <= dim; ++k) c->extraction.push_back(std::make_pair(c->origin_i + k, c->origin_j - dir * dim));
      c->origin_j += dir;
      if ((r = append_tiles(c, c->origin_i, c->origin_j + dir * dim, 1, 0))) return r;
    }
  }
  if (!c->extraction.empty()) return extract_surfels(c, c->p.partial_extraction != 0);
  return SB_OK;
}

int map_update(sb_ctx* c, const float* pose, const sb_frame* frame, const Mat4* pose_dev = nullptr,
               const Mat4* inv_dev = nullptr, bool table_ready = false) {
  c->map_version += 1;
  const KParams& kp = c->kp;
  Launch L = L_(c);
  const size_t Pd = (size_t)kp.W * kp.H;
  const bool deferred = pose_dev != nullptr;
  int r;
  float inv_pose[16] = {0}, pose_h[16] = {0};
  if (!deferred) {
    if (c->map_timestamp < kMaxPoses) {
      if ((r = set_pose_entry(c, c->map_timestamp, pose))) return r;
    }
    sbg::rigid_inverse_f(pose, inv_pose);
    memcpy(pose_h, pose, 64);
  }
  if (!table_ready) launch_pose_products(L, mat4_from(inv_pose), inv_dev, c->poses, c->Mtab_old, pose_table_count(c));
  if (!(c->prepped_for_update && frame == c->cur)) launch_radius(L, kp, frame->d, c->radius_map, c->key_index, c->integrated, c->group_counts);
  c->prepped_for_update = false;
  launch_index_scatter(L, kp, c->A, c->d_counts, n_grid(c), c->Mtab_old, c->key_index);
  float2 ctr = submap_center(c, c->origin_i, c->origin_j);
  float extent = 2.0f * c->p.submap_dimension * c->p.submap_extent + c->p.submap_extent;
  if (c->p.partial_extraction && !c->extraction.empty()) extent += 2.0f * c->p.submap_extent;
  launch_update_surfels(L, kp, c->A, c->T, c->d_counts, n_grid(c), mat4_from(pose_h), mat4_from(inv_pose), pose_dev,
                        inv_dev, c->poses, c->poses_inv, c->key_index, c->radius_map, frame->d, (int)c->map_timestamp,
                        ctr, extent, c->integrated, c->keep, c->block_counts, c->group_counts);
  launch_compact_update(L, c->T, c->keep, c->block_counts, c->group_counts, c->d_counts, n_grid(c), c->A, kMaxSurfels,
                        c->d_counts + 1, c->d_counts + 2);
  c->lb_gen = (c->lb_gen + 1) & 0x3fffffffu;
  if (c->lb_gen == 0) c->lb_gen = 1;
  launch_gen_compact(L, kp, frame->d, c->radius_map, c->integrated, c->poses, (int)c->map_timestamp, ctr, extent, c->A,
                     c->lb_desc, c->lb_ticket, c->lb_gen, kMaxSurfels, c->d_counts);
  uint64_t up = (uint64_t)n_grid(c) + Pd;
  c->n_upper = up > kMaxSurfels ? kMaxSurfels : (uint32_t)up;
  if (deferred) {
    c->map_timestamp += 1;
    return SB_OK;
  }
  uint32_t cnt[4];
  if ((r = fetch_counts(c, cnt, 4))) return r;
  c->n_host = cnt[0];
  c->n_upper = cnt[0];
  c->n_updated = cnt[2];
  c->n_new = cnt[3];
  if ((r = update_active_submaps(c, pose))) return r;
  c->map_timestamp += 1;
  return SB_OK;
}

float conf_threshold(const sb_ctx* c) {
  float ct = c->confidence_threshold;
  if (c->timestamp < 10) {
    float alpha = (float)c->timestamp / 10.0f;
    ct = (float)((1.0 - (double)alpha) * (double)c->log_unstable_slam + (double)(alpha * c->confidence_threshold));
  }
  return ct;
}

int grow_point_buffers(sb_ctx* c, size_t n) {
  if (n <= c->pts_cap) return SB_OK;
  size_t cap = n + n / 4 + 1024;
  SB_CUDA(c, cudaStreamSynchronize(c->stream));
  if (c->copy_stream) SB_CUDA(c, cudaStreamSynchronize(c->copy_stream));
  float4* np = nullptr; float* nl = nullptr; float* nq = nullptr;
  if (cudaMalloc(&np, cap * 16) != cudaSuccess || cudaMalloc(&nl, cap * 4) != cudaSuccess ||
      cudaMalloc(&nq, cap * 4) != cudaSuccess) {
    cudaFree(np); cudaFree(nl); cudaFree(nq);
    cudaGetLastError();
    return fail(c, SB_ERR_CAPACITY, "out of device memory for the scan staging buffers");
  }
  cudaFree(c->d_pts); cudaFree(c->d_labels); cudaFree(c->d_probs);
  c->d_pts = np; c->d_labels = nl; c->d_probs = nq;
  for (auto& sl : c->prefetch) {
    cudaFree(sl.pts); cudaFree(sl.labels); cudaFree(sl.probs);
    sl.pts = nullptr; sl.labels = nullptr; sl.probs = nullptr;
    sl.valid = false; sl.in_use = false; sl.has_released = false;
  }
  c->pts_cap = cap;
  return SB_OK;
}

int upload_scan(sb_ctx* c, const float* pts4, const float* labels, const float* probs, uint32_t n, int on_device,
                const float4** d_pts, const float** d_labels, const float** d_probs) {
  if (on_device) {
    *d_pts = reinterpret_cast<const float4*>(pts4);
    *d_labels = labels;
    *d_probs = probs;
    return SB_OK;
  }
  int rg = grow_point_buffers(c, n);
  if (rg) return rg;
  if (c->copy_stream) {
    for (auto& sl : c->prefetch)
      if (sl.in_use) {
        SB_CUDA(c, cudaEventRecord(sl.released, c->stream));
        sl.has_released = true;
        sl.in_use = false;
      }
    for (auto& sl : c->prefetch) {
      if (!sl.valid || sl.host_pts != pts4 || sl.n != n || sl.has_labels != (labels != nullptr) ||
          sl.has_probs != (probs != nullptr))
        continue;
      SB_CUDA(c, cudaStreamWaitEvent(c->stream, sl.done, 0));
      sl.valid = false;
      sl.in_use = true;
      *d_pts = sl.pts;
      *d_labels = labels ? sl.labels : nullptr;
      *d_probs = probs ? sl.probs : nullptr;
      return SB_OK;
    }
  }
  if (n) SB_CUDA(c, cudaMemcpyAsync(c->d_pts, pts4, (size_t)n * 16, cudaMemcpyHostToDevice, c->stream));
  if (labels && n) SB_CUDA(c, cudaMemcpyAsync(c->d_labels, labels, (size_t)n * 4, cudaMemcpyHostToDevice, c->stream));
  if (probs && n) SB_CUDA(c, cudaMemcpyAsync(c->d_probs, probs, (size_t)n * 4, cudaMemcpyHostToDevice, c->stream));
  *d_pts = c->d_pts;
  *d_labels = labels ? c->d_labels : nullptr;
  *d_probs = probs ? c->d_probs : nullptr;
  return SB_OK;
}

int render_composed_internal(sb_ctx* c, const float* pose_old, const float* pose_new, float conf_thr) {
  c->rkey_valid = false;
  const KParams& kp = c->kp;
  Launch L = L_(c);
  size_t Pm = (size_t)kp.Wm * kp.Hm;
  float inv_old[16], inv_new[16];
  sbg::rigid_inverse_f(pose_old, inv_old);
  sbg::rigid_inverse_f(pose_new, inv_new);
  uint32_t np = pose_table_count(c);
  launch_pose_products(L, mat4_from(inv_old), nullptr, c->poses, c->Mtab_old, np);
  launch_pose_products(L, mat4_from(inv_new), nullptr, c->poses, c->Mtab_new, np);
  RenderTargets t{nullptr, nullptr, c->key_comp};
  int thr = t_threshold(c);
  launch_render_scatter(L, kp, c->A, c->d_counts, n_grid(c), c->Mtab_old, conf_thr, thr, 1, 0, 1, t);
  launch_render_scatter(L, kp, c->A, c->d_counts, n_grid(c), c->Mtab_new, conf_thr, thr, 0, 1, 1, t);
  launch_render_resolve(L, kp, c->A, c->Mtab_old, c->Mtab_new, t, null_frame(), null_frame(), c->f_comp->d, null_frame(),
                        null_frame(), 1, 1);
  SB_CUDA(c, cudaGetLastError());
  return SB_OK;
}

int update_pose_enqueue(sb_ctx* c, bool* tables_ready) {
  const sb_params& p = c->p;
  const bool sem = c->cur_has_semantics;
  *tables_ready = false;
  int r;
  Launch L = L_(c);
  const uint32_t np = pose_table_count(c);
  int max_iter = p.max_iterations;
  if (max_iter <= 0 || max_iter > kMaxGnIter) max_iter = kMaxGnIter;
  const int r0 = c->comm_on ? c->row_begin : 0, r1 = c->comm_on ? c->row_end : c->kp.H;
  if (!c->comm_cb && c->icp_coop_blocks > 0) {
    GnJob job;
    memset(&job, 0, sizeof(job));
    job.mode = GN_MAIN;
    job.a = icp_args(c, c->cur, c->f_new, p.icp_max_distance, p.icp_max_angle, r0, r1, sem);
    job.st = c->gn;
    job.pd = c->pd;
    job.Mtab = c->Mtab_old;
    job.poses = c->poses;
    job.n_poses = np;
    job.initialize_identity = p.initialize_identity;
    job.fallback_mode = p.fallback_mode;
    job.timestamp = c->timestamp;
    job.max_iter = max_iter;
    job.eps = p.stopping_threshold;
    job.delta = p.delta;
    job.epoch_base = next_epoch_base(c, max_iter);
    job.use_cache = c->gn_use_cache;
    if (launch_gn_persistent(L, c->kp, job, c->acc_slots, c->ticket, c->gn_pub, c->comm_on ? &c->comm : nullptr,
                             c->icp_coop_blocks) != 0) {
      cudaGetLastError();
      return fail(c, SB_ERR_CUDA, "cooperative launch of the Gauss-Newton kernel failed");
    }
    if ((r = render_single(c, nullptr, conf_threshold(c), 1, &c->pd->invP_active, true, c->last_model))) return r;
    GnJob post;
    memset(&post, 0, sizeof(post));
    post.mode = GN_POST;
    post.a = icp_args(c, c->cur, c->f_new, p.icp_max_distance, p.icp_max_angle, 0, c->kp.H, sem);
    post.fb = icp_args(c, c->cur, c->last, p.fallback_max_distance, p.fallback_max_angle, r0, r1,
                       sem && c->last_has_semantics);
    post.st = c->gn2;
    post.pd = c->pd;
    post.stats32 = c->acc32;
    post.poses = c->poses;
    post.poses_inv = c->poses_inv;
    post.t_map = c->map_timestamp;
    post.Mtab = c->Mtab_old;
    post.n_poses = np;
    post.fallback_mode = p.fallback_mode;
    post.timestamp = c->timestamp;
    post.max_iter = max_iter;
    post.eps = p.stopping_threshold;
    post.delta = p.delta;
    post.epoch_base = next_epoch_base(c, max_iter);
    post.use_cache = 0;
    if (launch_gn_persistent(L, c->kp, post, c->acc_slots, c->ticket, c->gn_pub, c->comm_on ? &c->comm : nullptr,
                             c->icp_coop_blocks) != 0) {
      cudaGetLastError();
      return fail(c, SB_ERR_CUDA, "cooperative launch of the Gauss-Newton kernel failed");
    }
    *tables_ready = true;
    return SB_OK;
  }
  double T0[16];
  if (!p.initialize_identity) memcpy(T0, c->lastIncrement, sizeof(T0)); else ident_d(T0);
  if ((r = icp_minimize_enqueue(c, c->cur, c->f_new, T0, p.max_iterations, p.stopping_threshold, p.delta,
                                p.icp_max_distance, p.icp_max_angle, sem)))
    return r;
  Mat4d T0v;
  memcpy(T0v.m, T0, sizeof(T0v.m));
  launch_pose_after_icp(L, c->gn, c->pd, T0v, c->timestamp, p.fallback_mode);
  if ((r = render_single(c, nullptr, conf_threshold(c), 1, &c->pd->invP_active, false, c->last_model))) return r;
  {
    IcpArgs a = icp_args(c, c->cur, c->f_new, p.icp_max_distance, p.icp_max_angle, 0, c->kp.H, sem);
    Mat4 I;
    for (int i = 0; i < 16; ++i) I.m[i] = (i % 5 == 0) ? 1.0f : 0.0f;
    launch_icp_jacobian(L, c->kp, a, I, 0, c->acc32, c->acc_slots, c->ticket + 16, c->icp_blocks);
  }
  if (p.fallback_mode) {
    int fb = 0;
    SB_CUDA(c, cudaMemcpyAsync(c->h_pinned, (const char*)c->pd + offsetof(PoseDev, fallback), sizeof(int),
                               cudaMemcpyDeviceToHost, c->stream));
    SB_CUDA(c, cudaStreamSynchronize(c->stream));
    memcpy(&fb, c->h_pinned, sizeof(int));
    if (fb) {
      GnState* keep = c->gn;
      c->gn = c->gn2;
      int rr = icp_minimize_callback(c, c->cur, c->last, T0, max_iter, p.stopping_threshold, p.delta,
                                     p.fallback_max_distance, p.fallback_max_angle, sem && c->last_has_semantics);
      c->gn = keep;
      if (rr) return rr;
    }
  }
  launch_pose_finalize(L, c->gn2, c->pd, 1, c->poses, c->poses_inv, c->map_timestamp);
  return SB_OK;
}

struct CudaLoopBackend {
  sb_ctx* c;
  int err = 0;
  float confidence_threshold() { return conf_threshold(c); }
  void render_inactive(const float* pose, float ct) {
    if (!err) err = render_single(c, pose, ct, 0);
  }
  void render_composed(const float* pose_old, const float* pose_new, float ct) {
    if (!err) err = render_composed_internal(c, pose_old, pose_new, ct);
  }
  int minimize_old(const double* T0, double* pose_out, double* out48) {
    int iters = 0;
    if (!err)
      err = icp_minimize_enqueue(c, c->cur, c->f_old, T0, c->p.max_iterations, c->p.stopping_threshold, c->p.delta,
                                 c->p.icp_max_distance, c->p.icp_max_angle, c->cur_has_semantics);
    if (!err) err = icp_minimize_fetch(c, pose_out, out48, &iters, nullptr, nullptr);
    return iters;
  }
  void evaluate(int model, const double* pose, int iteration, double* out48) {
    long long raw[32];
    memset(raw, 0, sizeof(raw));
    if (!err)
      err = icp_jacobian_raw(c, c->cur, model == 0 ? c->f_old : c->f_comp, pose, iteration, c->p.icp_max_distance,
                             c->p.icp_max_angle, 0, c->kp.H, c->cur_has_semantics, raw);
    sbg::unpack48(raw, out48);
  }
};

void absorb_pose_block(sb_ctx* c, const PoseDev& pdh, const char* hp, bool had_icp) {
  memcpy(c->lastPose, pdh.lastPose, sizeof(c->lastPose));
  memcpy(c->currentPose, pdh.currentPose, sizeof(c->currentPose));
  memcpy(c->lastPose_old, c->currentPose_old, sizeof(c->lastPose_old));
  memcpy(c->currentPose_old, pdh.currentPose, sizeof(c->currentPose));
  memcpy(c->currentPose_new, pdh.currentPose, sizeof(c->currentPose));
  memcpy(c->lastIncrement, pdh.lastIncrement, sizeof(c->lastIncrement));
  c->trackLoss = (uint32_t)pdh.trackLoss;
  if (had_icp) {
    long long raw[32];
    double r48[48];
    memcpy(raw, hp + 4096, sizeof(raw));
    sbg::unpack48(raw, r48);
    c->stats[0] = pdh.icp_iterations;
    c->stats[1] = r48[43];
    c->stats[3] = r48[44];
    c->stats[2] = (double)((uint32_t)r48[42] - (uint32_t)r48[44]);
    c->stats[4] = r48[46];
    c->stats[5] = (float)r48[45];
    suma_b200::loop::OptResult& rn = c->loop.result_new;
    rn.error = r48[43];
    rn.outlier = (uint32_t)(float)r48[44];
    rn.valid = (uint32_t)r48[42];
    rn.inlier = rn.valid - rn.outlier;
    rn.invalid = (uint32_t)(float)r48[46];
    rn.residual = rn.error / (rn.inlier + rn.outlier);
    rn.inlier_residual = (float)r48[45] / rn.inlier;
  }
  c->stats[6] = c->trackLoss;
}

int loop_closure_step(sb_ctx* c) {
  namespace lp = suma_b200::loop;
  if (c->comm_on || c->comm_cb) return fail(c, SB_ERR_STATE, "loop closure is not available in row-striped multi-GPU mode");
  char* hp = (char*)c->h_pinned;
  SB_CUDA(c, cudaMemcpyAsync(hp, c->result_block, 8192 + 64, cudaMemcpyDeviceToHost, c->stream));
  const double t_enqueued = now_s();
  SB_CUDA(c, cudaStreamSynchronize(c->stream));
  const double t_synced = now_s();
  PoseDev pdh;
  memcpy(&pdh, hp, sizeof(pdh));
  if (pdh.gn_error) return gn_fail(c);
  absorb_pose_block(c, pdh, hp, true);
  lp::Poses P;
  memcpy(P.current.m, c->currentPose, 128);
  memcpy(P.current_old.m, c->currentPose_old, 128);
  memcpy(P.current_new.m, c->currentPose_new, 128);
  memcpy(P.last_old.m, c->lastPose_old, 128);
  memcpy(P.last_increment.m, c->lastIncrement, 128);
  lp::M4 inc;
  memcpy(inc.m, pdh.increment, 128);
  c->loop.after_update_pose(c->timestamp, inc, P.current);
  CudaLoopBackend be{c};
  lp::check_loop_closure(c->loop, be, c->timestamp, P);
  if (be.err) return be.err;
  memcpy(c->currentPose_old, P.current_old.m, 128);
  return SB_OK;
}

}

extern "C" {

int sb_default_params(sb_params* p) {
  if (!p) return SB_ERR_INVALID;
  memset(p, 0, sizeof(*p));
  p->data_width = 900; p->data_height = 64;
  p->data_fov_up = 3.0f; p->data_fov_down = -25.0f;
  p->min_depth = 2.0f; p->max_depth = 75.0f;
  p->model_width = 900; p->model_height = 64;
  p->model_fov_up = 3.0f; p->model_fov_down = -25.0f;
  p->model_min_depth = 2.0f; p->model_max_depth = 75.0f;
  p->max_iterations = 33; p->stopping_threshold = 0.0001f; p->delta = 0.0001f;
  p->icp_max_distance = 2.0f; p->icp_max_angle = 30.0f;
  p->weighting = 1; p->factor = 0.5f;
  p->initialize_identity = 0; p->bilinear_sampling = 1;
  p->fallback_mode = 1; p->fallback_max_distance = 0.5f; p->fallback_max_angle = 30.0f;
  p->compose_rendering = 1; p->max_loop_closure_distance = 8.0f;
  p->min_radius = 0.03f; p->max_radius = 1.0f; p->max_angle = 90.0f;
  p->map_max_distance = 0.2f; p->map_max_angle = 45.0f;
  p->unstable_age = 3; p->confidence_mode = 3; p->confidence_threshold = 0.0f;
  p->p_stable = 0.6f; p->p_prior = 0.5f; p->sigma_angle = 1.0f; p->sigma_distance = 1.0f;
  p->use_stability = 1; p->active_timestamps = 100; p->max_weight = 20.0f;
  p->weighting_scheme = 0; p->averaging_scheme = 0; p->update_always = 0;
  p->submap_dimension = 4; p->submap_extent = 10.0f; p->partial_extraction = 1;
  p->label_offset_quirk = 1; p->render_after_update = 1;
  return SB_OK;
}

int sb_device_count(void) {
  int n = 0;
  if (cudaGetDeviceCount(&n) != cudaSuccess) return 0;
  return n;
}

static int check_params(const sb_params* p) {
  if (!p) return SB_ERR_INVALID;
  if (p->data_width <= 0 || p->data_height <= 0 || p->model_width <= 0 || p->model_height <= 0) return SB_ERR_INVALID;
  if ((size_t)p->data_width * p->data_height > (1u << 24)) return SB_ERR_INVALID;
  if (!(p->max_depth > p->min_depth) || !(p->model_max_depth > p->model_min_depth)) return SB_ERR_INVALID;
  return SB_OK;
}

int sb_create(const sb_params* p, int device, sb_ctx** out) {
  if (!out || check_params(p)) return SB_ERR_INVALID;
  int n = 0;
  if (cudaGetDeviceCount(&n) != cudaSuccess || n == 0) return SB_ERR_NOGPU;
  if (device < 0 || device >= n) return SB_ERR_INVALID;
  sb_ctx* c = new sb_ctx();
  c->device = device;
  c->p = *p;
  if (cudaSetDevice(device) != cudaSuccess) {
    delete c;
    return SB_ERR_CUDA;
  }
  cudaDeviceProp prop;
  if (cudaGetDeviceProperties(&prop, device) == cudaSuccess) c->sm_count = prop.multiProcessorCount;
  c->icp_blocks = icp_grid_blocks(c->sm_count);
  {
    int coop = 0;
    cudaDeviceGetAttribute(&coop, cudaDevAttrCooperativeLaunch, device);
    int maxb = coop ? gn_persistent_max_blocks(c->sm_count) : 0;
    c->icp_coop_blocks = maxb < c->icp_blocks ? maxb : c->icp_blocks;
    if (c->icp_coop_blocks > 0) c->icp_coop_blocks = icp_balanced_blocks(p->data_width * p->data_height, c->icp_coop_blocks);
    c->icp_blocks = icp_balanced_blocks(p->data_width * p->data_height, c->icp_blocks);
    if (getenv("SUMA_B200_NO_PERSISTENT_GN")) c->icp_coop_blocks = 0;
    if (getenv("SUMA_B200_ICP_BLOCKS")) {
      int b = atoi(getenv("SUMA_B200_ICP_BLOCKS"));
      if (b > 0 && b <= maxb && b <= 1024) c->icp_coop_blocks = b;
    }
  }
  if (cudaStreamCreateWithFlags(&c->stream, cudaStreamNonBlocking) != cudaSuccess) {
    delete c;
    return SB_ERR_CUDA;
  }
  derive(c);
  int r = alloc_buffers(c);
  if (r != SB_OK) {
    fprintf(stderr, "sb_create: %s\n", c->err.c_str());
    release_buffers(c);
    cudaStreamDestroy(c->stream);
    delete c;
    return r;
  }
  *out = c;
  return SB_OK;
}

int sb_destroy(sb_ctx* c) {
  if (!c) return SB_ERR_INVALID;
  cudaSetDevice(c->device);
  cudaStreamSynchronize(c->stream);
  sb_comm_shutdown(c);
  release_buffers(c);
  for (auto& sl : c->prefetch) {
    cudaFree(sl.pts); cudaFree(sl.labels); cudaFree(sl.probs);
    if (sl.done) cudaEventDestroy(sl.done);
    if (sl.released) cudaEventDestroy(sl.released);
  }
  if (c->copy_stream) cudaStreamDestroy(c->copy_stream);
  for (auto& r : c->prof.recs) {
    cudaEventDestroy(r.e0);
    cudaEventDestroy(r.e1);
  }
  for (cudaEvent_t e : c->prof.pool) cudaEventDestroy(e);
  cudaStreamDestroy(c->stream);
  delete c;
  return SB_OK;
}

int sb_reset(sb_ctx* c) {
  if (!c) return SB_ERR_INVALID;
  cudaSetDevice(c->device);
  return reset_state(c);
}

int sb_set_params(sb_ctx* c, const sb_params* p) {
  if (!c || check_params(p)) return fail(c, SB_ERR_INVALID, "set_params: bad parameters");
  if (p->data_width != c->p.data_width || p->data_height != c->p.data_height || p->model_width != c->p.model_width ||
      p->model_height != c->p.model_height)
    return fail(c, SB_ERR_STATE, "set_params: image sizes are fixed at sb_create (as in SurfelMapping's constructor)");
  c->p = *p;
  derive(c);
  c->rkey_valid = false;
  return SB_OK;
}

const char* sb_last_error(const sb_ctx* c) { return c ? c->err.c_str() : "null context"; }

int sb_synchronize(sb_ctx* c) {
  if (!c) return SB_ERR_INVALID;
  SB_CUDA(c, cudaStreamSynchronize(c->stream));
  return SB_OK;
}

void* sb_stream(sb_ctx* c) { return c ? (void*)c->stream : nullptr; }
uint64_t sb_launch_count(const sb_ctx* c) { return c ? c->launches : 0; }

int sb_frame_create(sb_ctx* c, int w, int h, sb_frame** out) {
  if (!c) return SB_ERR_INVALID;
  cudaSetDevice(c->device);
  return frame_create(c, w, h, out);
}
int sb_frame_destroy(sb_frame* f) {
  if (!f) return SB_ERR_INVALID;
  cudaStreamSynchronize(f->ctx->stream);
  cudaFree(f->base);
  delete f;
  return SB_OK;
}
int sb_frame_copy(sb_frame* dst, const sb_frame* src) {
  if (!dst || !src || dst->d.W != src->d.W || dst->d.H != src->d.H) return SB_ERR_INVALID;
  sb_ctx* c = dst->ctx;
  c->rkey_valid = false;
  SB_CUDA(c, cudaMemcpyAsync(dst->base, src->base, (size_t)src->d.W * src->d.H * 48, cudaMemcpyDeviceToDevice, c->stream));
  return SB_OK;
}
static float4* frame_plane(const sb_frame* f, int which) {
  return which == SB_MAP_VERTEX ? f->d.vertex : (which == SB_MAP_NORMAL ? f->d.normal : f->d.semantic);
}
int sb_frame_download(const sb_frame* f, int which, float* dst) {
  if (!f || !dst || which < 0 || which > 2) return SB_ERR_INVALID;
  sb_ctx* c = f->ctx;
  SB_CUDA(c, cudaMemcpyAsync(dst, frame_plane(f, which), (size_t)f->d.W * f->d.H * 16, cudaMemcpyDeviceToHost, c->stream));
  SB_CUDA(c, cudaStreamSynchronize(c->stream));
  return SB_OK;
}
int sb_frame_upload(sb_frame* f, int which, const float* src) {
  if (!f || !src || which < 0 || which > 2) return SB_ERR_INVALID;
  sb_ctx* c = f->ctx;
  c->rkey_valid = false;
  SB_CUDA(c, cudaMemcpyAsync(frame_plane(f, which), src, (size_t)f->d.W * f->d.H * 16, cudaMemcpyHostToDevice, c->stream));
  SB_CUDA(c, cudaStreamSynchronize(c->stream));
  return SB_OK;
}
int sb_frame_size(const sb_frame* f, int* w, int* h) {
  if (!f) return SB_ERR_INVALID;
  if (w) *w = f->d.W;
  if (h) *h = f->d.H;
  return SB_OK;
}

int sb_preprocess(sb_ctx* c, const float* pts4, const float* labels, const float* probs, uint32_t n, uint32_t timestamp,
                  int on_device, sb_frame* out) {
  if (!c || !out || (!pts4 && n)) return fail(c, SB_ERR_INVALID, "preprocess: null argument");
  if (out->d.W != c->kp.W || out->d.H != c->kp.H) return fail(c, SB_ERR_INVALID, "preprocess: frame size mismatch");
  cudaSetDevice(c->device);
  const float4* dp; const float* dl; const float* dq;
  int r = upload_scan(c, pts4, labels, probs, n, on_device, &dp, &dl, &dq);
  if (r) return r;
  launch_preprocess(L_(c), c->kp, dp, dl, dq, n, timestamp, c->prep, out->d, nullptr, nullptr, nullptr, nullptr);
  SB_CUDA(c, cudaGetLastError());
  return SB_OK;
}

int sb_map_render(sb_ctx* c, const float pose_old[16], const float pose_new[16], float conf_thr, sb_frame* out) {
  if (!c || !pose_old || !pose_new || !out) return fail(c, SB_ERR_INVALID, "map_render: null argument");
  if (out->d.W != c->kp.Wm || out->d.H != c->kp.Hm) return fail(c, SB_ERR_INVALID, "map_render: frame size mismatch");
  cudaSetDevice(c->device);
  int r = render_full(c, pose_old, pose_new, conf_thr, out);
  if (r) return r;
  SB_CUDA(c, cudaGetLastError());
  return SB_OK;
}
int sb_map_render_active(sb_ctx* c, const float pose[16], float conf_thr) {
  if (!c || !pose) return fail(c, SB_ERR_INVALID, "map_render_active: null argument");
  cudaSetDevice(c->device);
  int r = render_single(c, pose, conf_thr, 1);
  if (r) return r;
  SB_CUDA(c, cudaGetLastError());
  return SB_OK;
}
int sb_map_render_inactive(sb_ctx* c, const float pose[16], float conf_thr) {
  if (!c || !pose) return fail(c, SB_ERR_INVALID, "map_render_inactive: null argument");
  cudaSetDevice(c->device);
  int r = render_single(c, pose, conf_thr, 0);
  if (r) return r;
  SB_CUDA(c, cudaGetLastError());
  return SB_OK;
}
int sb_map_render_composed(sb_ctx* c, const float pose_old[16], const float pose_new[16], float conf_thr) {
  if (!c || !pose_old || !pose_new) return fail(c, SB_ERR_INVALID, "map_render_composed: null argument");
  cudaSetDevice(c->device);
  return render_composed_internal(c, pose_old, pose_new, conf_thr);
}
int sb_map_frame(sb_ctx* c, int which, sb_frame** out) {
  if (!c || !out || which < 0 || which > 2) return SB_ERR_INVALID;
  *out = which == SB_FRAME_OLD ? c->f_old : (which == SB_FRAME_NEW ? c->f_new : c->f_comp);
  return SB_OK;
}

void sb_icp_unpack(const int64_t raw32[32], double out48[48]) { sbg::unpack48((const long long*)raw32, out48); }

int sb_icp_jacobian(sb_ctx* c, const sb_frame* data, const sb_frame* model, const double pose[16], int iteration,
                    float max_distance, float max_angle_deg, int row_begin, int row_end, double out48[48],
                    int64_t raw32[32]) {
  int r = icp_check(c, data, model);
  if (r) return r;
  if (!pose || row_begin < 0 || row_end > c->kp.H || row_begin > row_end)
    return fail(c, SB_ERR_INVALID, "icp_jacobian: bad pose / row range");
  cudaSetDevice(c->device);
  long long raw[32];
  if ((r = icp_jacobian_raw(c, data, model, pose, iteration, max_distance, max_angle_deg, row_begin, row_end, true, raw)))
    return r;
  if (raw32) memcpy(raw32, raw, sizeof(raw));
  if (out48) sbg::unpack48(raw, out48);
  return SB_OK;
}

int sb_icp_minimize(sb_ctx* c, const sb_frame* data, const sb_frame* model, const double T0[16], int max_iter, double eps,
                    double delta, float max_distance, float max_angle_deg, double pose_out[16], double out48[48],
                    int* iters, double* history, int* history_len) {
  int r = icp_check(c, data, model);
  if (r) return r;
  if (!T0) return fail(c, SB_ERR_INVALID, "icp_minimize: null T0");
  if (history && (max_iter <= 0 || max_iter > kMaxGnIter))
    return fail(c, SB_ERR_INVALID, "icp_minimize: with a history buffer max_iter must be in [1, 256]");
  cudaSetDevice(c->device);
  if ((r = icp_minimize_enqueue(c, data, model, T0, max_iter, eps, delta, max_distance, max_angle_deg, true))) return r;
  if ((r = icp_minimize_fetch(c, pose_out, out48, iters, history, history_len))) return r;
  SB_CUDA(c, cudaGetLastError());
  return SB_OK;
}

void sb_se3_exp(const double x[6], double T[16]) { sbg::se3_exp(x, T); }

void sb_se3_log(const double M[16], double x[6]) {
  for (int i = 0; i < 6; ++i) x[i] = 0.0;
  double d = 0.5 * (((M[0] + M[5]) + M[10]) - 1.0);
  double K[9] = {0, 0, 0, 0, 0, 0, 0, 0, 0};
  if (d < 1 - 1e-10) {
    double theta = acos(d);
    double f = theta / (2 * sin(theta));
    for (int r = 0; r < 3; ++r)
      for (int cc = 0; cc < 3; ++cc) K[r * 3 + cc] = f * (M[cc * 4 + r] - M[r * 4 + cc]);
    x[3] = K[2 * 3 + 1]; x[4] = K[0 * 3 + 2]; x[5] = K[1 * 3 + 0];
  }
  double theta = sqrt((x[3] * x[3] + x[4] * x[4]) + x[5] * x[5]);
  x[0] = M[12]; x[1] = M[13]; x[2] = M[14];
  if (fabs(theta) > 1e-10) {
    double half = 0.5 * theta;
    double beta = 1 / (theta * theta) * (1 - theta * cos(half) / (2 * sin(half)));
    double t[3] = {M[12], M[13], M[14]};
    for (int r = 0; r < 3; ++r) {
      double acc = 0;
      for (int cc = 0; cc < 3; ++cc) {
        double k2 = (K[r * 3 + 0] * K[0 * 3 + cc] + K[r * 3 + 1] * K[1 * 3 + cc]) + K[r * 3 + 2] * K[2 * 3 + cc];
        double Vi = ((r == cc ? 1.0 : 0.0) + (-0.5) * K[r * 3 + cc]) + beta * k2;
        acc += Vi * t[cc];
      }
      x[r] = acc;
    }
  }
}

int sb_ldlt_solve6(const double A[36], const double b[6], double x[6]) {
  sbg::ldlt_solve6(A, b, x);
  return SB_OK;
}
int sb_gn_step(const double out48[48], double last_error, double eps, double delta, double pose[16], double dx[6]) {
  return sbg::gn_step(out48, last_error, eps, delta, pose, dx);
}

int sb_map_update(sb_ctx* c, const float pose[16], const sb_frame* frame) {
  if (!c || !pose || !frame) return fail(c, SB_ERR_INVALID, "map_update: null argument");
  if (frame->d.W != c->kp.W || frame->d.H != c->kp.H) return fail(c, SB_ERR_INVALID, "map_update: frame size mismatch");
  cudaSetDevice(c->device);
  int r = map_update(c, pose, frame);
  if (r) return r;
  SB_CUDA(c, cudaGetLastError());
  return SB_OK;
}

int sb_map_update_poses(sb_ctx* c, const float* poses16, uint32_t count) {
  if (!c || (!poses16 && count)) return SB_ERR_INVALID;
  cudaSetDevice(c->device);
  for (uint32_t t = 0; t < count && t < kMaxPoses; ++t) {
    int r = set_pose_entry(c, t, poses16 + 16 * (size_t)t);
    if (r) return r;
  }
  return SB_OK;
}
int sb_map_set_pose(sb_ctx* c, uint32_t t, const float pose[16]) {
  if (!c || !pose) return SB_ERR_INVALID;
  cudaSetDevice(c->device);
  return set_pose_entry(c, t, pose);
}
int sb_map_size(sb_ctx* c, uint32_t* n) {
  if (!c || !n) return SB_ERR_INVALID;
  *n = c->n_host;
  return SB_OK;
}
int sb_map_timestamp(sb_ctx* c, uint32_t* t) {
  if (!c || !t) return SB_ERR_INVALID;
  *t = c->map_timestamp;
  return SB_OK;
}
int sb_map_download(sb_ctx* c, sb_surfel* dst, uint32_t cap, uint32_t* n) {
  if (!c || (!dst && cap)) return SB_ERR_INVALID;
  cudaSetDevice(c->device);
  uint32_t k = c->n_host < cap ? c->n_host : cap;
  if (n) *n = k;
  if (k == 0) return SB_OK;
  launch_soa_to_aos(L_(c), c->A, reinterpret_cast<sb_surfel*>(c->T.p0), k);
  SB_CUDA(c, cudaMemcpyAsync(dst, c->T.p0, (size_t)k * 64, cudaMemcpyDeviceToHost, c->stream));
  SB_CUDA(c, cudaStreamSynchronize(c->stream));
  return SB_OK;
}
int sb_map_upload(sb_ctx* c, const sb_surfel* src, uint32_t n, uint32_t timestamp) {
  if (!c || (!src && n)) return SB_ERR_INVALID;
  if (n > kMaxSurfels) return fail(c, SB_ERR_CAPACITY, "map_upload: more than 4194304 surfels");
  cudaSetDevice(c->device);
  if (n) {
    SB_CUDA(c, cudaMemcpyAsync(c->T.p0, src, (size_t)n * 64, cudaMemcpyHostToDevice, c->stream));
    launch_aos_to_soa(L_(c), reinterpret_cast<const sb_surfel*>(c->T.p0), c->A, 0, n);
  }
  c->n_host = n;
  c->n_upper = n;
  c->map_timestamp = timestamp;
  c->map_version += 1;
  SB_CUDA(c, cudaMemcpyAsync(c->d_counts, &c->n_host, 4, cudaMemcpyHostToDevice, c->stream));
  SB_CUDA(c, cudaStreamSynchronize(c->stream));
  return SB_OK;
}
int sb_map_update_debug(sb_ctx* c, uint32_t* index_map, float* radius_map4, uint8_t* integrated, uint32_t* n_updated,
                        uint32_t* n_new) {
  if (!c) return SB_ERR_INVALID;
  cudaSetDevice(c->device);
  size_t Pd = (size_t)c->kp.W * c->kp.H;
  SB_CUDA(c, cudaStreamSynchronize(c->stream));
  if (index_map) {
    std::vector<unsigned long long> keys(Pd);
    SB_CUDA(c, cudaMemcpy(keys.data(), c->key_index, Pd * 8, cudaMemcpyDeviceToHost));
    for (size_t i = 0; i < Pd; ++i) index_map[i] = keys[i] == ~0ull ? 0u : (uint32_t)(keys[i] & 0xffffffffull) + 1u;
  }
  if (radius_map4) SB_CUDA(c, cudaMemcpy(radius_map4, c->radius_map, Pd * 16, cudaMemcpyDeviceToHost));
  if (integrated) SB_CUDA(c, cudaMemcpy(integrated, c->integrated, Pd, cudaMemcpyDeviceToHost));
  if (n_updated) *n_updated = c->n_updated;
  if (n_new) *n_new = c->n_new;
  return SB_OK;
}
int sb_map_submap_origin(sb_ctx* c, int32_t* i, int32_t* j, uint32_t* pending) {
  if (!c) return SB_ERR_INVALID;
  if (i) *i = c->origin_i;
  if (j) *j = c->origin_j;
  if (pending) *pending = (uint32_t)c->extraction.size();
  return SB_OK;
}

int sb_process_scan(sb_ctx* c, const float* pts4, const float* labels, const float* probs, uint32_t n, int on_device) {
  if (!c || (!pts4 && n)) return fail(c, SB_ERR_INVALID, "process_scan: null argument");
  cudaSetDevice(c->device);
  const sb_params& p = c->p;
  Launch L = L_(c);
  double t_all = now_s();
  const float4* dp; const float* dl; const float* dq;
  int r = upload_scan(c, pts4, labels, probs, n, on_device, &dp, &dl, &dq);
  if (r) return r;
  std::swap(c->cur, c->last);
  std::swap(c->cur_model, c->last_model);
  c->last_has_semantics = c->cur_has_semantics;
  c->cur_has_semantics = labels != nullptr;
  launch_preprocess(L, c->kp, dp, dl, dq, n, c->timestamp, c->prep, c->cur->d, c->radius_map, c->key_index, c->integrated,
                    c->group_counts);
  c->prepped_for_update = true;
  float ct = conf_threshold(c);
  float Pold[16], Pnew[16];
  cast_f(c->currentPose_old, Pold);
  cast_f(c->currentPose_new, Pnew);
  if ((r = render_full(c, Pold, Pnew, ct, c->last_model))) return r;
  const bool had_icp = c->timestamp > 0;
  bool tables_ready = false;
  bool loop_ran = false;
  if (had_icp) {
    if ((r = update_pose_enqueue(c, &tables_ready))) return r;
    if (c->close_loops) {
      if ((r = loop_closure_step(c))) return r;
      tables_ready = false;
      loop_ran = true;
    }
  } else {
    launch_pose_finalize(L, c->gn2, c->pd, 0, c->poses, c->poses_inv, c->map_timestamp);
  }
  const uint32_t t_map = c->map_timestamp;
  if ((r = map_update(c, nullptr, c->cur, &c->pd->P_cur, &c->pd->invP_cur, tables_ready))) return r;
  float ct2 = conf_threshold(c);
  if (p.render_after_update) {
    if ((r = render_full(c, nullptr, nullptr, ct2, c->cur_model, &c->pd->invP_cur, true))) return r;
  }
  char* hp = (char*)c->h_pinned;
  SB_CUDA(c, cudaMemcpyAsync(hp, c->result_block, 8192 + 64, cudaMemcpyDeviceToHost, c->stream));
  const double t_enqueued = now_s();
  SB_CUDA(c, cudaStreamSynchronize(c->stream));
  const double t_synced = now_s();
  SB_CUDA(c, cudaGetLastError());
  PoseDev pdh;
  memcpy(&pdh, hp, sizeof(pdh));
  if (pdh.gn_error) return gn_fail(c);
  if (!loop_ran) absorb_pose_block(c, pdh, hp, had_icp);
  uint32_t cnt[4];
  memcpy(cnt, hp + 8192, sizeof(cnt));
  c->n_host = cnt[0];
  c->n_upper = cnt[0];
  c->n_updated = cnt[2];
  c->n_new = cnt[3];
  if (t_map < kMaxPoses) {
    memcpy(&c->h_poses[16 * (size_t)t_map], pdh.P_cur.m, 64);
    sbg::rigid_inverse_f(pdh.P_cur.m, &c->h_poses_inv[16 * (size_t)t_map]);
  }
  if (p.render_after_update) {
    memcpy(c->rkey.pose_old, pdh.P_cur.m, 64);
    memcpy(c->rkey.pose_new, pdh.P_cur.m, 64);
    c->rkey.conf_thr = ct2;
    c->rkey.map_timestamp = c->map_timestamp;
    c->rkey.map_version = c->map_version;
    c->rkey.compose = c->p.compose_rendering;
    c->rkey.out = c->cur_model;
    c->rkey_valid = true;
  }
  {
    const uint64_t v0 = c->map_version;
    const uint32_t n0 = c->n_host;
    if ((r = update_active_submaps(c, pdh.P_cur.m))) return r;
    if (c->n_host != n0) {
      c->map_version = v0 + 1;
      c->rkey_valid = false;
      if (p.render_after_update && (r = render_full(c, pdh.P_cur.m, pdh.P_cur.m, ct2, c->cur_model))) return r;
    }
  }
  c->stats[7] = c->n_host;
  const double t_end = now_s();
  c->stats[8] = t_enqueued - t_all;
  c->stats[9] = t_synced - t_enqueued;
  c->stats[10] = t_end - t_synced;
  c->stats[11] = t_end - t_all;
  c->timestamp += 1;
  return SB_OK;
}

int sb_prefetch_scan(sb_ctx* c, const float* pts4, const float* labels, const float* probs, uint32_t n) {
  if (!c || (!pts4 && n)) return fail(c, SB_ERR_INVALID, "prefetch_scan: null argument");
  cudaSetDevice(c->device);
  int rg = grow_point_buffers(c, n);
  if (rg) return rg;
  if (!c->copy_stream) {
    SB_CUDA(c, cudaStreamCreateWithFlags(&c->copy_stream, cudaStreamNonBlocking));
    for (auto& sl : c->prefetch) {
      SB_CUDA(c, cudaEventCreateWithFlags(&sl.done, cudaEventDisableTiming));
      SB_CUDA(c, cudaEventCreateWithFlags(&sl.released, cudaEventDisableTiming));
    }
  }
  for (auto& sl : c->prefetch)
    if (!sl.pts) {
      SB_CUDA(c, cudaMalloc(&sl.pts, c->pts_cap * 16));
      SB_CUDA(c, cudaMalloc(&sl.labels, c->pts_cap * 4));
      SB_CUDA(c, cudaMalloc(&sl.probs, c->pts_cap * 4));
    }
  sb_ctx::PrefetchSlot* slot = nullptr;
  for (auto& sl : c->prefetch)
    if (!sl.valid && !sl.in_use) {
      slot = &sl;
      break;
    }
  if (!slot) return fail(c, SB_ERR_STATE, "prefetch_scan: two scans are already staged");
  if (slot->has_released) SB_CUDA(c, cudaStreamWaitEvent(c->copy_stream, slot->released, 0));
  if (n) SB_CUDA(c, cudaMemcpyAsync(slot->pts, pts4, (size_t)n * 16, cudaMemcpyHostToDevice, c->copy_stream));
  if (labels && n) SB_CUDA(c, cudaMemcpyAsync(slot->labels, labels, (size_t)n * 4, cudaMemcpyHostToDevice, c->copy_stream));
  if (probs && n) SB_CUDA(c, cudaMemcpyAsync(slot->probs, probs, (size_t)n * 4, cudaMemcpyHostToDevice, c->copy_stream));
  SB_CUDA(c, cudaEventRecord(slot->done, c->copy_stream));
  slot->host_pts = pts4;
  slot->n = n;
  slot->has_labels = labels != nullptr;
  slot->has_probs = probs != nullptr;
  slot->valid = true;
  return SB_OK;
}

void sb_default_loop_params(sb_loop_params* p) {
  if (!p) return;
  p->search_distance = 50.0f;
  p->min_trajectory_distance = 200.0f;
  p->min_verifications = 5;
  p->residual_threshold = 1.15f;
  p->outlier_threshold = 1.1f;
  p->valid_threshold = 0.95f;
}

int sb_set_loop_closure(sb_ctx* c, int enabled, const sb_loop_params* p) {
  if (!c) return SB_ERR_INVALID;
  sb_loop_params d;
  sb_default_loop_params(&d);
  if (p) d = *p;
  c->loop.p.search_distance = d.search_distance;
  c->loop.p.min_trajectory_distance = d.min_trajectory_distance;
  c->loop.p.min_verifications = d.min_verifications;
  c->loop.p.residual_threshold = d.residual_threshold;
  c->loop.p.outlier_threshold = d.outlier_threshold;
  c->loop.p.valid_threshold = d.valid_threshold;
  if (enabled && !c->close_loops) c->loop.reset();
  c->close_loops = enabled != 0;
  return SB_OK;
}

int sb_get_loop_info(sb_ctx* c, sb_loop_info* o) {
  if (!c || !o) return SB_ERR_INVALID;
  const suma_b200::loop::State& L = c->loop;
  memset(o, 0, sizeof(*o));
  o->enabled = c->close_loops ? 1u : 0u;
  o->loop_count = L.loop_count;
  o->time_without_loop_closure = L.time_without_loop_closure;
  o->candidates_tested = L.candidates_tested;
  o->loop_edges_added = L.loop_edges_added;
  o->unverified = (uint32_t)L.unverified.size();
  o->already_verified = L.already_verified ? 1u : 0u;
  o->found_candidate = L.found_candidate ? 1u : 0u;
  o->use_candidate = L.use_candidate ? 1u : 0u;
  o->optimisation_requested = L.optimisation_requested ? 1u : 0u;
  o->last_added_candidate = L.last_added_candidate;
  o->n_edges = (uint32_t)L.graph.edges.size();
  o->n_poses = (uint32_t)L.graph.poses.size();
  o->valid_ratio = L.stat_valid_ratio;
  o->outlier_ratio = L.stat_outlier_ratio;
  o->rel_error = L.stat_rel_error;
  o->residual_old = L.result_old.residual;
  o->residual_new = L.result_new.residual;
  memcpy(o->current_pose_old, c->currentPose_old, sizeof(o->current_pose_old));
  return SB_OK;
}

int sb_get_loop_edges(sb_ctx* c, sb_loop_edge* dst, uint32_t cap, uint32_t* n) {
  if (!c || (!dst && cap)) return SB_ERR_INVALID;
  const auto& E = c->loop.graph.edges;
  uint32_t k = (uint32_t)E.size() < cap ? (uint32_t)E.size() : cap;
  for (uint32_t i = 0; i < k; ++i) {
    dst[i].from = E[i].from;
    dst[i].to = E[i].to;
    memcpy(dst[i].rel_pose, E[i].rel.m, 128);
  }
  if (n) *n = (uint32_t)E.size();
  return SB_OK;
}

int sb_integrate_loop_closures(sb_ctx* c, const double* poses16, uint32_t n, uint32_t* integrated) {
  namespace lp = suma_b200::loop;
  if (integrated) *integrated = 0;
  if (!c) return SB_ERR_INVALID;
  cudaSetDevice(c->device);
  lp::State& S = c->loop;
  if (!c->close_loops || !S.optimisation_requested) return SB_OK;
  std::vector<lp::M4> opt;
  if (poses16) {
    if (n <= (uint32_t)S.before_id) return fail(c, SB_ERR_INVALID, "integrate_loop_closures: fewer poses than the graph held at the request");
    opt.resize(n);
    for (uint32_t i = 0; i < n; ++i) memcpy(opt[i].m, poses16 + 16 * (size_t)i, 128);
  } else {
    opt.assign(S.graph.poses.begin(), S.graph.poses.begin() + (long)S.requested_size);
  }
  lp::M4 cur, cold, cnew;
  memcpy(cur.m, c->currentPose, 128);
  memcpy(cold.m, c->currentPose_old, 128);
  memcpy(cnew.m, c->currentPose_new, 128);
  std::vector<lp::M4> all = S.integrate(opt, cur, cold, cnew);
  if (all.empty()) return fail(c, SB_ERR_STATE, "integrate_loop_closures: no optimisation request pending");
  std::vector<float> pf(all.size() * 16);
  for (size_t t = 0; t < all.size(); ++t) lp::to_float(all[t], &pf[16 * t]);
  int r = sb_map_update_poses(c, pf.data(), (uint32_t)all.size());
  if (r) return r;
  memcpy(c->currentPose_old, cold.m, 128);
  memcpy(c->currentPose_new, cnew.m, 128);
  if ((r = sb_set_current_pose(c, cur.m))) return r;
  if (integrated) *integrated = (uint32_t)all.size();
  return SB_OK;
}

int sb_set_current_pose(sb_ctx* c, const double pose[16]) {
  if (!c || !pose) return SB_ERR_INVALID;
  cudaSetDevice(c->device);
  memcpy(c->currentPose, pose, sizeof(c->currentPose));
  SB_CUDA(c, cudaMemcpyAsync((char*)c->pd + offsetof(PoseDev, currentPose), c->currentPose, sizeof(c->currentPose),
                             cudaMemcpyHostToDevice, c->stream));
  SB_CUDA(c, cudaStreamSynchronize(c->stream));
  c->rkey_valid = false;
  return SB_OK;
}

int sb_get_pose(sb_ctx* c, double pose[16]) {
  if (!c || !pose) return SB_ERR_INVALID;
  memcpy(pose, c->currentPose, sizeof(c->currentPose));
  return SB_OK;
}
int sb_get_last_pose(sb_ctx* c, double pose[16]) {
  if (!c || !pose) return SB_ERR_INVALID;
  memcpy(pose, c->lastPose, sizeof(c->lastPose));
  return SB_OK;
}
int sb_timestamp(sb_ctx* c, uint32_t* t) {
  if (!c || !t) return SB_ERR_INVALID;
  *t = c->timestamp;
  return SB_OK;
}
int sb_slam_frame(sb_ctx* c, int which, sb_frame** out) {
  if (!c || !out || which < 0 || which > 3) return SB_ERR_INVALID;
  sb_frame* f[4] = {c->cur, c->last, c->cur_model, c->last_model};
  *out = f[which];
  return SB_OK;
}
int sb_get_statistics(sb_ctx* c, double stats[16]) {
  if (!c || !stats) return SB_ERR_INVALID;
  memcpy(stats, c->stats, sizeof(c->stats));
  return SB_OK;
}


int sb_profile_enable(sb_ctx* c, int on) {
  if (!c) return SB_ERR_INVALID;
  c->prof.on = on != 0;
  return SB_OK;
}
int sb_profile_kernels(void) { return K_COUNT; }
const char* sb_profile_name(int id) { return kernel_name(id); }
int sb_profile_collect(sb_ctx* c, double* total_ms, uint64_t* count, int cap) {
  if (!c || !total_ms || !count || cap < K_COUNT) return SB_ERR_INVALID;
  cudaSetDevice(c->device);
  SB_CUDA(c, cudaStreamSynchronize(c->stream));
  for (int i = 0; i < K_COUNT; ++i) {
    total_ms[i] = 0.0;
    count[i] = 0;
  }
  for (auto& r : c->prof.recs) {
    float ms = 0.f;
    if (cudaEventElapsedTime(&ms, r.e0, r.e1) == cudaSuccess) {
      total_ms[r.id] += ms;
      count[r.id] += 1;
    }
    c->prof.pool.push_back(r.e0);
    c->prof.pool.push_back(r.e1);
  }
  c->prof.recs.clear();
  return SB_OK;
}

int sb_comm_export(sb_ctx* c, uint8_t handle[64]) {
  if (!c || !handle) return SB_ERR_INVALID;
  cudaSetDevice(c->device);
  if (!c->mailbox) {
    SB_CUDA(c, cudaMalloc(&c->mailbox, 2u << 20));
  }
  SB_CUDA(c, cudaStreamSynchronize(c->stream));
  SB_CUDA(c, cudaMemset(c->mailbox, 0, 2u << 20));
  cudaIpcMemHandle_t h;
  SB_CUDA(c, cudaIpcGetMemHandle(&h, c->mailbox));
  static_assert(sizeof(h) == 64, "cudaIpcMemHandle_t is 64 bytes");
  memcpy(handle, &h, 64);
  return SB_OK;
}

int sb_comm_init(sb_ctx* c, int rank, int nranks, const uint8_t* handles, int row_begin, int row_end) {
  if (!c || !handles || nranks < 1 || nranks > 8 || rank < 0 || rank >= nranks)
    return fail(c, SB_ERR_INVALID, "comm_init: bad rank / nranks (max 8)");
  if (row_begin < 0 || row_end > c->kp.H || row_begin > row_end) return fail(c, SB_ERR_INVALID, "comm_init: bad rows");
  if (!c->mailbox) return fail(c, SB_ERR_STATE, "comm_init: call sb_comm_export first");
  cudaSetDevice(c->device);
  memset(&c->comm, 0, sizeof(c->comm));
  c->comm.rank = rank;
  c->comm.nranks = nranks;
  c->comm.epoch = c->comm_epoch;
  c->peer_ptrs.clear();
  for (int r = 0; r < nranks; ++r) {
    if (r == rank) {
      c->comm.mailbox[r] = c->mailbox;
      continue;
    }
    cudaIpcMemHandle_t h;
    memcpy(&h, handles + 64 * (size_t)r, 64);
    void* ptr = nullptr;
    SB_CUDA(c, cudaIpcOpenMemHandle(&ptr, h, cudaIpcMemLazyEnablePeerAccess));
    c->comm.mailbox[r] = (long long*)ptr;
    c->peer_ptrs.push_back(ptr);
  }
  SB_CUDA(c, cudaMemset(c->comm_epoch, 0, 64));
  c->row_begin = row_begin;
  c->row_end = row_end;
  c->comm_on = nranks > 1 || getenv("SUMA_B200_SELF_COMM") != nullptr;
  return SB_OK;
}

int sb_comm_set_callback(sb_ctx* c, sb_allreduce_fn fn, void* user, int row_begin, int row_end) {
  if (!c) return SB_ERR_INVALID;
  if (fn && (row_begin < 0 || row_end > c->kp.H || row_begin > row_end)) return fail(c, SB_ERR_INVALID, "comm: bad rows");
  if (fn && c->comm_on) return fail(c, SB_ERR_STATE, "comm: the fused peer-memory mode is already active");
  c->comm_cb = fn;
  c->comm_cb_user = user;
  if (fn) {
    c->row_begin = row_begin;
    c->row_end = row_end;
  }
  return SB_OK;
}

int sb_comm_shutdown(sb_ctx* c) {
  if (!c) return SB_ERR_INVALID;
  c->comm_cb = nullptr;
  for (void* p : c->peer_ptrs) cudaIpcCloseMemHandle(p);
  c->peer_ptrs.clear();
  c->comm_on = false;
  return SB_OK;
}

}
```

semantic_suma_b200/csrc/sb_icp.cu:

```cuda
#include "sb_gn.cuh"
#include "sb_internal.cuh"

namespace sb {
using namespace sbm;

constexpr int kIcpThreads = 256;

int icp_grid_blocks(int sm_count) { return sm_count * 2; }

int icp_balanced_blocks(int pixels, int max_blocks) {
  int units = (pixels + kIcpThreads - 1) / kIcpThreads;
  if (max_blocks < 1) max_blocks = 1;
  int u = (units + max_blocks - 1) / max_blocks;
  int blocks = (units + u - 1) / u;
  return blocks < 1 ? 1 : blocks;
}

__device__ __forceinline__ float4 tex_border(const float4* __restrict__ img, int W, int H, int x, int y) {
  if (x < 0 || x >= W || y < 0 || y >= H) return make_float4(0.f, 0.f, 0.f, 0.f);
  return __ldg(img + (size_t)y * W + x);
}

struct Bilin {
  int i0, j0;
  float w00, w10, w01, w11;
};
__device__ __forceinline__ Bilin bilin_setup(float u, float v) {
  Bilin b;
  float a = u - 0.5f, c = v - 0.5f;
  float fa = floorf(a), fc = floorf(c);
  b.i0 = (int)fa;
  b.j0 = (int)fc;
  float al = a - fa, be = c - fc;
  b.w00 = (1.0f - al) * (1.0f - be);
  b.w10 = al * (1.0f - be);
  b.w01 = (1.0f - al) * be;
  b.w11 = al * be;
  return b;
}
__device__ __forceinline__ float4 sample_bilin(const float4* __restrict__ img, int W, int H, const Bilin& b) {
  float4 t00 = tex_border(img, W, H, b.i0, b.j0);
  float4 t10 = tex_border(img, W, H, b.i0 + 1, b.j0);
  float4 t01 = tex_border(img, W, H, b.i0, b.j0 + 1);
  float4 t11 = tex_border(img, W, H, b.i0 + 1, b.j0 + 1);
  float4 r;
  r.x = ((b.w00 * t00.x + b.w10 * t10.x) + b.w01 * t01.x) + b.w11 * t11.x;
  r.y = ((b.w00 * t00.y + b.w10 * t10.y) + b.w01 * t01.y) + b.w11 * t11.y;
  r.z = ((b.w00 * t00.z + b.w10 * t10.z) + b.w01 * t01.z) + b.w11 * t11.z;
  r.w = ((b.w00 * t00.w + b.w10 * t10.w) + b.w01 * t01.w) + b.w11 * t11.w;
  return r;
}

struct Acc {
  long long s[29];
  int n_valid, n_outlier, n_invalid;
};

__device__ __forceinline__ void icp_pixel_v(const KParams& kp, const IcpArgs& a, const float* M, int pix, float4 Vd, float4 Nd,
                                            int iteration, Acc& acc) {
  float e_d = Vd.w + Nd.w;
  if (!(e_d > 1.5f)) {
    acc.n_invalid += 1;
    return;
  }
  V3 v_d = xform_point(M, mk3(Vd.x, Vd.y, Vd.z));
  V3 n_d = xform_dir(M, mk3(Nd.x, Nd.y, Nd.z));
  float depth = len3(v_d);
  float yaw = atan2f_(v_d.y, v_d.x);
  float pitch = -asinf_(v_d.z / depth);
  float px = 0.5f * ((-yaw * kInvPi) + 1.0f);
  float py = 1.0f - (kRad2Deg * pitch + kp.fov_up) / kp.fov;
  float ix = px * (float)a.Wm, iy = py * (float)a.Hm;
  if (!(ix >= 0.0f && ix < (float)a.Wm && iy >= 0.0f && iy < (float)a.Hm)) {
    acc.n_invalid += 1;
    return;
  }
  float4 Vm, Nm;
  Bilin b;
  int tx = 0, ty = 0;
  if (kp.bilinear) {
    b = bilin_setup(ix, iy);
    Vm = sample_bilin(a.model_v, a.Wm, a.Hm, b);
    Nm = sample_bilin(a.model_n, a.Wm, a.Hm, b);
  } else {
    tx = (int)floorf(ix);
    ty = (int)floorf(iy);
    Vm = tex_border(a.model_v, a.Wm, a.Hm, tx, ty);
    Nm = tex_border(a.model_n, a.Wm, a.Hm, tx, ty);
  }
  float e_m = Vm.w + Nm.w;
  if (!(e_m > 1.5f)) {
    acc.n_invalid += 1;
    return;
  }
  V3 v_m = mk3(Vm.x, Vm.y, Vm.z), n_m = mk3(Nm.x, Nm.y, Nm.z);
  bool inlier = true;
  if (len3(sub3(v_m, v_d)) > a.distance_thresh) inlier = false;
  if (dot3(n_m, n_d) < a.angle_thresh) inlier = false;
  float residual = dot3(n_m, sub3(v_d, v_m));
  V3 cp = cross3(v_d, n_m);
  float weight = 1.0f;
  if (kp.weighting == 4 || kp.weighting == 1) {
    if (fabsf(residual) > kp.factor) weight = kp.factor / fabsf(residual);
  } else if (kp.weighting == 2 && iteration > 0) {
    if (fabsf(residual) > kp.factor) {
      weight = 0.0f;
    } else {
      float alpha = residual / kp.factor;
      weight = 1.0f - alpha * alpha;
      weight = weight * weight;
    }
  }
  if (a.has_semantics) {
    float4 Sm = kp.bilinear ? sample_bilin(a.model_s, a.Wm, a.Hm, b) : tex_border(a.model_s, a.Wm, a.Hm, tx, ty);
    float4 Sd = __ldg(a.data_s + pix);
    float data_label = Sd.x * 255.0f, data_prob = Sd.w, model_label = Sm.x * 255.0f;
    if (is_movable(model_label)) {
      if (roundf_(data_label) != roundf_(model_label))
        weight = weight * (1.0f - data_prob);
      else
        weight = weight * data_prob;
    }
  }
  acc.n_valid += 1;
  float wr = weight * residual;
  acc.s[27] += fix30(wr * residual);
  if (inlier) {
    const float J[6] = {n_m.x, n_m.y, n_m.z, cp.x, cp.y, cp.z};
    int k = 0;
#pragma unroll
    for (int c = 0; c < 6; ++c) {
      float wc = weight * J[c];
#pragma unroll
      for (int r = c; r < 6; ++r) acc.s[k++] += fix30(wc * J[r]);
    }
#pragma unroll
    for (int r = 0; r < 6; ++r) acc.s[21 + r] += fix30(wr * J[r]);
    acc.s[28] += fix30(wr * residual);
  } else {
    acc.n_outlier += 1;
  }
}

__device__ __forceinline__ void icp_pixel(const KParams& kp, const IcpArgs& a, const float* M, int pix, int iteration,
                                          Acc& acc) {
  icp_pixel_v(kp, a, M, pix, __ldg(a.data_v + pix), __ldg(a.data_n + pix), iteration, acc);
}

__device__ __forceinline__ long long warp_sum_ll(long long v) {
#pragma unroll
  for (int o = 16; o > 0; o >>= 1) v += __shfl_down_sync(0xffffffffu, v, o);
  return v;
}

template <bool kFence>
__device__ __forceinline__ void block_reduce_to_global(Acc& acc, long long* __restrict__ g_acc) {
  __shared__ long long sm[kIcpThreads / 32][32];
  const int lane = threadIdx.x & 31, warp = threadIdx.x >> 5;
#pragma unroll
  for (int i = 0; i < 29; ++i) {
    long long v = warp_sum_ll(acc.s[i]);
    if (lane == 0) sm[warp][i] = v;
  }
  int nv = __reduce_add_sync(0xffffffffu, acc.n_valid);
  int no = __reduce_add_sync(0xffffffffu, acc.n_outlier);
  int ni = __reduce_add_sync(0xffffffffu, acc.n_invalid);
  if (lane == 0) {
    sm[warp][29] = nv;
    sm[warp][30] = no;
    sm[warp][31] = ni;
  }
  __syncthreads();
  if (warp == 0) {
    long long v = 0;
#pragma unroll
    for (int w = 0; w < kIcpThreads / 32; ++w) v += sm[w][lane];
    if (v != 0) atomicAdd((unsigned long long*)(g_acc + lane), (unsigned long long)v);
    if (kFence) __threadfence();
  }
}

__device__ __forceinline__ long long warp_transpose_reduce(long long (&v)[32], int lane) {
#pragma unroll
  for (int half = 16; half >= 1; half >>= 1) {
    const bool upper = (lane & half) != 0;
#pragma unroll
    for (int i = 0; i < half; ++i) {
      long long keep = upper ? v[i + half] : v[i];
      long long send = upper ? v[i] : v[i + half];
      long long recv = __shfl_xor_sync(0xffffffffu, send, half);
      v[i] = keep + recv;
    }
  }
  return v[0];
}

constexpr int kAccReplicas = 8;

__device__ __forceinline__ void block_reduce_to_replica(Acc& acc, long long* __restrict__ replicas) {
  __shared__ long long sm[kIcpThreads / 32][32];
  const int lane = threadIdx.x & 31, warp = threadIdx.x >> 5;
  long long v[32];
#pragma unroll
  for (int i = 0; i < 29; ++i) v[i] = acc.s[i];
  v[29] = acc.n_valid;
  v[30] = acc.n_outlier;
  v[31] = acc.n_invalid;
  sm[warp][lane] = warp_transpose_reduce(v, lane);
  __syncthreads();
  if (warp == 0) {
    long long t = 0;
#pragma unroll
    for (int w = 0; w < kIcpThreads / 32; ++w) t += sm[w][lane];
    if (t != 0)
      atomicAdd((unsigned long long*)(replicas + (size_t)(blockIdx.x % kAccReplicas) * 32 + lane), (unsigned long long)t);
  }
}

__device__ __forceinline__ long long sum_replicas(const long long* __restrict__ replicas, int lane) {
  long long r[kAccReplicas];
#pragma unroll
  for (int i = 0; i < kAccReplicas; ++i) r[i] = *(const volatile long long*)(replicas + (size_t)i * 32 + lane);
  long long tot = 0;
#pragma unroll
  for (int i = 0; i < kAccReplicas; ++i) tot += r[i];
  return tot;
}
__device__ __forceinline__ void clear_replicas(long long* __restrict__ replicas, int lane) {
#pragma unroll
  for (int i = 0; i < kAccReplicas; ++i) replicas[(size_t)i * 32 + lane] = 0;
}

__device__ __forceinline__ void icp_accumulate(const KParams& kp, const IcpArgs& a, const float* M, int iteration,
                                               Acc& acc) {
#pragma unroll
  for (int i = 0; i < 29; ++i) acc.s[i] = 0;
  acc.n_valid = acc.n_outlier = acc.n_invalid = 0;
  const int begin = a.row_begin * kp.W, end = a.row_end * kp.W;
  for (int pix = begin + blockIdx.x * blockDim.x + threadIdx.x; pix < end; pix += gridDim.x * blockDim.x)
    icp_pixel(kp, a, M, pix, iteration, acc);
}

__global__ void __launch_bounds__(kIcpThreads) k_icp_jacobian(KParams kp, IcpArgs a, Mat4 pose, int iteration,
                                                              long long* __restrict__ g_acc,
                                                              long long* __restrict__ slots, unsigned int* ticket) {
  float M[16];
#pragma unroll
  for (int i = 0; i < 16; ++i) M[i] = pose.m[i];
  Acc acc;
  icp_accumulate(kp, a, M, iteration, acc);
  block_reduce_to_replica(acc, slots);
  __shared__ bool is_last;
  __syncthreads();
  if (threadIdx.x == 0) {
    __threadfence();
    unsigned int t = atomicAdd(ticket, 1u);
    is_last = (t == gridDim.x - 1);
  }
  __syncthreads();
  if (!is_last || threadIdx.x >= 32) return;
  __threadfence();
  long long tot = sum_replicas(slots, threadIdx.x);
  clear_replicas(slots, threadIdx.x);
  g_acc[threadIdx.x] = tot;
  if (threadIdx.x == 0) *ticket = 0;
}

void launch_icp_jacobian(const Launch& L, const KParams& kp, const IcpArgs& a, const Mat4& pose, int iteration,
                         long long* acc32, long long* slots, unsigned int* ticket, int blocks) {
  {
    ScopedKernel sk(L, K_ICP_JACOBIAN);
    k_icp_jacobian<<<blocks, kIcpThreads, 0, L.stream>>>(kp, a, pose, iteration, acc32, slots, ticket);
  }
}

__device__ void pose_after_icp_body(const double* gn_pose, int gn_k, PoseDev* pd, const double* T0, uint32_t timestamp,
                                    int fallback_mode) {
  double inc[16], inv_last[16], delta[16], Pn[16];
  for (int i = 0; i < 16; ++i) pd->T0[i] = T0[i];
  for (int i = 0; i < 16; ++i) inc[i] = gn_pose[i];
  for (int i = 0; i < 16; ++i) pd->increment[i] = inc[i];
  pd->icp_iterations = gn_k;
  sbg::rigid_inverse_d(pd->lastIncrement, inv_last);
  mat4_mul<double>(inv_last, inc, delta);
  mat4_mul<double>(pd->currentPose, inc, Pn);
  for (int i = 0; i < 16; ++i) pd->P_active.m[i] = (float)Pn[i];
  sbg::rigid_inverse_f(pd->P_active.m, pd->invP_active.m);
  float t_err = (float)sqrt((delta[12] * delta[12] + delta[13] * delta[13]) + delta[14] * delta[14]);
  float angle = (float)(0.5 * (((delta[0] + delta[5]) + delta[10]) - 1.0));
  float ca = angle < 1.0f ? angle : 1.0f;
  ca = ca > -1.0f ? ca : -1.0f;
  float r_err = acosf_(ca);
  pd->t_err = t_err;
  pd->r_err = r_err;
  int fb = (timestamp > 1 && ((double)t_err > 0.4 || (double)r_err > 0.1) && fallback_mode) ? 1 : 0;
  pd->fallback = fb;
  if (fb) pd->trackLoss += 1;
}

__device__ void pose_finalize_body(const double* recovery_pose, PoseDev* pd, int had_icp, float* poses, float* poses_inv,
                                   uint32_t t) {
  if (had_icp) {
    double inc[16], np[16];
    if (pd->fallback)
      for (int i = 0; i < 16; ++i) inc[i] = recovery_pose[i];
    else
      for (int i = 0; i < 16; ++i) inc[i] = pd->increment[i];
    for (int i = 0; i < 16; ++i) pd->lastPose[i] = pd->currentPose[i];
    mat4_mul<double>(pd->currentPose, inc, np);
    for (int i = 0; i < 16; ++i) {
      pd->currentPose[i] = np[i];
      pd->lastIncrement[i] = inc[i];
      pd->increment[i] = inc[i];
    }
  }
  for (int i = 0; i < 16; ++i) pd->P_cur.m[i] = (float)pd->currentPose[i];
  sbg::rigid_inverse_f(pd->P_cur.m, pd->invP_cur.m);
  if (t < kMaxPoses) {
    float inv[16];
    sbg::rigid_inverse_f(pd->P_cur.m, inv);
    for (int i = 0; i < 16; ++i) {
      poses[16 * (size_t)t + i] = pd->P_cur.m[i];
      poses_inv[16 * (size_t)t + i] = inv[i];
    }
  }
}

__global__ void k_gn_init(GnState* st, Mat4d T0, long long* acc32) {
  int i = threadIdx.x;
  if (i < 16) st->pose[i] = T0.m[i];
  if (i < 32) acc32[i] = 0;
  if (i < 48) st->out48[i] = 0.0;
  if (i == 0) {
    st->last_error = (double)3.402823466e+38f;
    st->k = 0;
    st->done = 0;
    st->history_len = 0;
    st->error = 0;
  }
}

void launch_gn_init(const Launch& L, GnState* st, const Mat4d& T0, long long* acc32) {
  {
    ScopedKernel sk(L, K_GN_INIT);
    k_gn_init<<<1, 64, 0, L.stream>>>(st, T0, acc32);
  }
}

__global__ void k_pose_after_icp(const GnState* __restrict__ gn, PoseDev* __restrict__ pd, Mat4d T0, uint32_t timestamp,
                                 int fallback_mode) {
  if (threadIdx.x != 0) return;
  pose_after_icp_body(gn->pose, gn->k, pd, T0.m, timestamp, fallback_mode);
}
void launch_pose_after_icp(const Launch& L, const GnState* gn, PoseDev* pd, const Mat4d& T0, uint32_t timestamp,
                           int fallback_mode) {
  {
    ScopedKernel sk(L, K_GN_INIT);
    k_pose_after_icp<<<1, 32, 0, L.stream>>>(gn, pd, T0, timestamp, fallback_mode);
  }
}

__global__ void k_pose_finalize(const GnState* __restrict__ gn, PoseDev* __restrict__ pd, int had_icp,
                                float* __restrict__ poses, float* __restrict__ poses_inv, uint32_t t) {
  if (threadIdx.x != 0) return;
  pose_finalize_body(gn->pose, pd, had_icp, poses, poses_inv, t);
}
void launch_pose_finalize(const Launch& L, const GnState* gn, PoseDev* pd, int had_icp, float* poses, float* poses_inv,
                          uint32_t t) {
  {
    ScopedKernel sk(L, K_GN_INIT);
    k_pose_finalize<<<1, 32, 0, L.stream>>>(gn, pd, had_icp, poses, poses_inv, t);
  }
}

struct GnShared {
  double A[36];
  double O[48];
  double P[16];
  double E[16];
  double dx[6];
  int perm[6];
  int result;
};

__device__ __forceinline__ void tri_cr(int k, int& c, int& r) {
  const int start[6] = {0, 6, 11, 15, 18, 20};
  c = 0;
#pragma unroll
  for (int i = 1; i < 6; ++i)
    if (k >= start[i]) c = i;
  r = c + (k - start[c]);
}

__device__ __forceinline__ unsigned long long globaltimer_ns() {
  unsigned long long t;
  asm volatile("mov.u64 %0, %%globaltimer;" : "=l"(t));
  return t;
}
constexpr unsigned long long kSpinTimeoutNs = 10ull * 1000ull * 1000ull * 1000ull;

__device__ void gn_step_warp(GnShared& sh, long long raw, int lane, double last_error, double eps, double delta_thr) {
  const double s = 1.0 / 1073741824.0;
  if (lane < 21) {
    int c, r;
    tri_cr(lane, c, r);
    double v = (double)raw * s;
    sh.O[c * 6 + r] = v;
    sh.O[r * 6 + c] = v;
  } else if (lane < 27) {
    sh.O[36 + (lane - 21)] = (double)raw * s;
  } else if (lane == 27) {
    sh.O[43] = (double)raw * s;
  } else if (lane == 28) {
    sh.O[45] = (double)raw * s;
  } else if (lane == 29) {
    sh.O[42] = (double)raw;
  } else if (lane == 30) {
    sh.O[44] = (double)raw;
  } else {
    sh.O[46] = (double)raw;
    sh.O[47] = 0.0;
  }
  __syncwarp();
  double* A = sh.A;
  for (int i = lane; i < 36; i += 32) A[i] = sh.O[i];
  if (lane < 6) sh.perm[lane] = lane;
  __syncwarp();
#pragma unroll 1
  for (int k = 0; k < 6; ++k) {
    int piv = k;
    double best = fabs(A[k * 6 + k]);
    for (int i = k + 1; i < 6; ++i) {
      double v = fabs(A[i * 6 + i]);
      if (v > best) {
        best = v;
        piv = i;
      }
    }
    __syncwarp();
    if (piv != k) {
      if (lane < 6) {
        double t = A[k * 6 + lane];
        A[k * 6 + lane] = A[piv * 6 + lane];
        A[piv * 6 + lane] = t;
      }
      __syncwarp();
      if (lane < 6) {
        double t = A[lane * 6 + k];
        A[lane * 6 + k] = A[lane * 6 + piv];
        A[lane * 6 + piv] = t;
      }
      if (lane == 0) {
        int t = sh.perm[k];
        sh.perm[k] = sh.perm[piv];
        sh.perm[piv] = t;
      }
      __syncwarp();
    }
    double dk = A[k * 6 + k];
    if (dk == 0.0) continue;
    if (lane > k && lane < 6) A[k * 6 + lane] = A[k * 6 + lane] / dk;
    __syncwarp();
    if (lane < 21) {
      int c, r;
      tri_cr(lane, c, r);
      if (c > k) {
        double v = A[c * 6 + r] - (A[k * 6 + r] * dk) * A[k * 6 + c];
        A[c * 6 + r] = v;
        A[r * 6 + c] = v;
      }
    }
    __syncwarp();
  }
  if (lane == 0) {
    double y[6], dx[6];
#pragma unroll
    for (int i = 0; i < 6; ++i) y[i] = -sh.O[36 + sh.perm[i]];
#pragma unroll
    for (int i = 0; i < 6; ++i)
#pragma unroll
      for (int k = 0; k < i; ++k) y[i] = y[i] - A[k * 6 + i] * y[k];
#pragma unroll
    for (int i = 0; i < 6; ++i) y[i] = (A[i * 6 + i] == 0.0) ? 0.0 : y[i] / A[i * 6 + i];
#pragma unroll
    for (int i = 5; i >= 0; --i)
#pragma unroll
      for (int k = i + 1; k < 6; ++k) y[i] = y[i] - A[i * 6 + k] * y[k];
#pragma unroll
    for (int i = 0; i < 6; ++i) sh.dx[sh.perm[i]] = y[i];
#pragma unroll
    for (int i = 0; i < 6; ++i) dx[i] = sh.dx[i];
    int result = 1;
    double current_error = sh.O[43];
    double linf = 0.0, maxc = sh.O[36];
#pragma unroll
    for (int i = 0; i < 6; ++i) {
      if (fabs(dx[i]) > linf) linf = fabs(dx[i]);
      if (sh.O[36 + i] > maxc) maxc = sh.O[36 + i];
    }
    if (linf < delta_thr) result = 0;
    if (fabs(maxc) < eps) result = 0;
    if (current_error < last_error && fabs(current_error - last_error) < eps) result = 0;
    sh.result = result;
    double E[16];
    sbg::se3_exp(dx, E);
#pragma unroll
    for (int i = 0; i < 16; ++i) sh.E[i] = E[i];
  }
  __syncwarp();
  double pn = 0.0;
  if (lane < 16) {
    int c = lane >> 2, r = lane & 3;
    const double* Ea = sh.E;
    const double* B = sh.P;
    pn = ((Ea[0 * 4 + r] * B[c * 4 + 0] + Ea[1 * 4 + r] * B[c * 4 + 1]) + Ea[2 * 4 + r] * B[c * 4 + 2]) +
         Ea[3 * 4 + r] * B[c * 4 + 3];
  }
  __syncwarp();
  if (lane < 16) sh.P[lane] = pn;
  __syncwarp();
}

__device__ bool comm_allreduce32_warp(const CommDev& cd, long long& raw, int lane) {
  unsigned int epoch = 0;
  if (lane == 0) {
    epoch = *cd.epoch + 1u;
    *cd.epoch = epoch;
  }
  epoch = __shfl_sync(0xffffffffu, epoch, 0);
  const int slot = (int)(epoch & 1u);
  const unsigned long long tag = (unsigned long long)epoch << 32;
  const unsigned long long w_lo = tag | (unsigned long long)(unsigned int)((unsigned long long)raw & 0xffffffffull);
  const unsigned long long w_hi = tag | (unsigned long long)(unsigned int)((unsigned long long)raw >> 32);
  for (int r = 0; r < cd.nranks; ++r) {
    volatile unsigned long long* dst =
        reinterpret_cast<volatile unsigned long long*>(cd.mailbox[r]) + ((size_t)(slot * 8 + cd.rank)) * 64;
    dst[lane] = w_lo;
    dst[32 + lane] = w_hi;
  }
  volatile unsigned long long* mine = reinterpret_cast<volatile unsigned long long*>(cd.mailbox[cd.rank]);
  const unsigned long long t0 = globaltimer_ns();
  unsigned long long tot = 0;
  int ok = 1;
  for (int r = 0; r < cd.nranks && ok; ++r) {
    volatile unsigned long long* src = mine + ((size_t)(slot * 8 + r)) * 64;
    unsigned long long lo = src[lane], hi = src[32 + lane];
    unsigned int spins = 0;
    while ((unsigned int)(lo >> 32) != epoch || (unsigned int)(hi >> 32) != epoch) {
      if ((++spins & 1023u) == 0u && globaltimer_ns() - t0 > kSpinTimeoutNs) {
        ok = 0;
        break;
      }
      lo = src[lane];
      hi = src[32 + lane];
    }
    tot += (lo & 0xffffffffull) | (hi << 32);
  }
  ok = __all_sync(0xffffffffu, ok);
  raw = (long long)tot;
  return ok != 0;
}

__device__ __forceinline__ void load_mat_cg(const float* table, int idx, float* M) {
  const float4* t = reinterpret_cast<const float4*>(table + 16 * (size_t)idx);
  float4 a = __ldcg(t), b = __ldcg(t + 1), c = __ldcg(t + 2), d = __ldcg(t + 3);
  M[0] = a.x; M[1] = a.y; M[2] = a.z; M[3] = a.w;
  M[4] = b.x; M[5] = b.y; M[6] = b.z; M[7] = b.w;
  M[8] = c.x; M[9] = c.y; M[10] = c.z; M[11] = c.w;
  M[12] = d.x; M[13] = d.y; M[14] = d.z; M[15] = d.w;
}

template <int kGnCachePix>
__global__ void __launch_bounds__(kIcpThreads, 2) k_gn_persistent(KParams kp, GnJob job, long long* __restrict__ slots,
                                                               unsigned int* ticket, unsigned long long* pub,
                                                               CommDev cd) {
  __shared__ GnShared sh;
  __shared__ bool is_last;
  __shared__ double s_pose[16];
  __shared__ double s_last_error;
  __shared__ int s_done, s_error;
  __shared__ float4 s_dv[kGnCachePix][kIcpThreads], s_dn[kGnCachePix][kIcpThreads];
  const int lane = threadIdx.x & 31, warp = threadIdx.x >> 5;
  GnState* st = job.st;
  PoseDev* pd = job.pd;
  if (threadIdx.x == 0) s_error = 0;
  const int px_begin = job.a.row_begin * kp.W, px_end = job.a.row_end * kp.W;
  const int px_stride = gridDim.x * blockDim.x, px_first = px_begin + blockIdx.x * blockDim.x + threadIdx.x;
  const bool cached = job.use_cache && job.mode != GN_POST && (px_end - px_begin) <= kGnCachePix * px_stride;
  if (cached) {
#pragma unroll
    for (int j = 0; j < kGnCachePix; ++j) {
      const int pix = px_first + j * px_stride;
      if (pix < px_end) {
        s_dv[j][threadIdx.x] = __ldg(job.a.data_v + pix);
        s_dn[j][threadIdx.x] = __ldg(job.a.data_n + pix);
      }
    }
  }
  for (unsigned int it = 0;; ++it) {
    if (warp == 0) {
      if (it == 0) {
        if (job.mode == GN_PLAIN) {
          if (lane < 16) s_pose[lane] = st->pose[lane];
          if (lane == 17) s_done = st->done;
        } else {
          if (lane < 16) {
            double v = (lane % 5 == 0) ? 1.0 : 0.0;
            if (job.mode == GN_MAIN && !job.initialize_identity) v = pd->lastIncrement[lane];
            s_pose[lane] = v;
          }
          if (lane == 17) s_done = 0;
        }
      } else {
        const unsigned int want = (job.epoch_base + it) & 0x7fffffffu;
        const unsigned long long t0 = globaltimer_ns();
        unsigned int spins = 0;
        unsigned long long w = *(volatile unsigned long long*)&pub[lane];
        unsigned long long w2 = lane < 2 ? *(volatile unsigned long long*)&pub[32 + lane] : 0ull;
        bool timed_out = false;
        while ((((unsigned int)(w >> 32)) & 0x7fffffffu) != want ||
               (lane < 2 && (((unsigned int)(w2 >> 32)) & 0x7fffffffu) != want)) {
          if ((++spins & 4095u) == 0u && globaltimer_ns() - t0 > kSpinTimeoutNs) {
            timed_out = true;
            break;
          }
          w = *(volatile unsigned long long*)&pub[lane];
          if (lane < 2) w2 = *(volatile unsigned long long*)&pub[32 + lane];
        }
        if (__any_sync(0xffffffffu, timed_out)) {
          if (lane == 0) s_error = 1;
        }
        const unsigned int lo = __shfl_sync(0xffffffffu, (unsigned int)w, 2 * (lane & 15));
        const unsigned int hi = __shfl_sync(0xffffffffu, (unsigned int)w, 2 * (lane & 15) + 1);
        if (lane < 16) s_pose[lane] = __hiloint2double((int)hi, (int)lo);
        if (lane == 17) s_done = (int)((w >> 63) & 1ull);
        const unsigned int e_lo = __shfl_sync(0xffffffffu, (unsigned int)w2, 0);
        const unsigned int e_hi = __shfl_sync(0xffffffffu, (unsigned int)w2, 1);
        if (lane == 18) s_last_error = __hiloint2double((int)e_hi, (int)e_lo);
      }
    }
    __syncthreads();
    if (s_error) {
      if (threadIdx.x == 0) {
        *(volatile int*)&st->error = 1;
        if (pd) *(volatile int*)&pd->gn_error = 1;
      }
      return;
    }
    if (s_done) {
      __threadfence();
      break;
    }
    long long* const my_slots = slots + (size_t)(it & 1u) * kAccReplicas * 32;
    const bool stats_pass = job.mode == GN_POST && it == 0;
    const bool recovery = job.mode == GN_POST && it > 0;
    const int k = job.mode == GN_POST ? (int)it - 1 : (int)it;
    float M[16];
#pragma unroll
    for (int i = 0; i < 16; ++i) M[i] = (float)s_pose[i];
    Acc acc;
    if (cached) {
#pragma unroll
      for (int i = 0; i < 29; ++i) acc.s[i] = 0;
      acc.n_valid = acc.n_outlier = acc.n_invalid = 0;
#pragma unroll
      for (int j = 0; j < kGnCachePix; ++j) {
        const int pix = px_first + j * px_stride;
        if (pix < px_end) icp_pixel_v(kp, job.a, M, pix, s_dv[j][threadIdx.x], s_dn[j][threadIdx.x], k, acc);
      }
    } else {
      icp_accumulate(kp, recovery ? job.fb : job.a, M, stats_pass ? 0 : k, acc);
    }
    __syncthreads();
    block_reduce_to_replica(acc, my_slots);
    __syncthreads();
    if (threadIdx.x == 0) {
      __threadfence();
      unsigned int t = atomicAdd(ticket, 1u);
      is_last = (t == (it + 1u) * gridDim.x - 1u);
    }
    __syncthreads();
    if (is_last && warp == 0) {
      __threadfence();
      long long raw = sum_replicas(my_slots, lane);
      int done = 0, error = 0;
      double pv = 0.0;
      if (stats_pass) {
        job.stats32[lane] = raw;
        const int fb = job.fallback_mode ? *(volatile int*)&pd->fallback : 0;
        if (fb) {
          if (lane < 16) {
            pv = pd->T0[lane];
            st->pose[lane] = pv;
          }
          if (lane == 0) {
            st->last_error = (double)3.402823466e+38f;
            st->k = 0;
            st->history_len = 0;
          }
        } else {
          done = 1;
        }
      } else {
        double last_error = (double)3.402823466e+38f;
        if (k > 0) last_error = s_last_error;
        if (cd.epoch) error = comm_allreduce32_warp(cd, raw, lane) ? 0 : 1;
        if (lane < 16) sh.P[lane] = s_pose[lane];
        int hl = k;
        if (lane < 16) st->history[hl * 16 + lane] = s_pose[lane];
        ++hl;
        __syncwarp();
        gn_step_warp(sh, raw, lane, last_error, job.eps, job.delta);
        if (lane < 16) {
          pv = sh.P[lane];
          st->pose[lane] = pv;
        }
        for (int i = lane; i < 48; i += 32) st->out48[i] = sh.O[i];
        int kk = k;
        if (sh.result == 0) {
          done = 1;
        } else {
          ++kk;
          if (kk >= job.max_iter) {
            if (lane < 16) st->history[hl * 16 + lane] = sh.P[lane];
            ++hl;
            done = 1;
          }
        }
        if (error) done = 1;
        if (lane == 0) {
          st->last_error = sh.O[43];
          st->k = kk;
          st->history_len = hl;
        }
        __syncwarp();
      }
      if (done && lane == 0 && !error) {
        if (job.mode == GN_MAIN) {
          double T0[16];
          for (int i = 0; i < 16; ++i) T0[i] = job.initialize_identity ? ((i % 5 == 0) ? 1.0 : 0.0) : pd->lastIncrement[i];
          pose_after_icp_body(sh.P, st->k, pd, T0, job.timestamp, job.fallback_mode);
        } else if (job.mode == GN_POST) {
          pose_finalize_body(st->pose, pd, 1, job.poses, job.poses_inv, job.t_map);
        }
      }
      if (lane == 0) {
        if (error) {
          st->error = 1;
          if (pd) pd->gn_error = 1;
        }
        st->done = done;
        if (done) *ticket = 0;
      }
      if (done) {
        clear_replicas(my_slots, lane);
        __threadfence();
      }
      __syncwarp();
      {
        const double src = __shfl_sync(0xffffffffu, pv, lane >> 1);
        const unsigned int half = (lane & 1) ? (unsigned int)__double2hiint(src) : (unsigned int)__double2loint(src);
        const unsigned int tag = ((job.epoch_base + it + 1u) & 0x7fffffffu) | (done ? 0x80000000u : 0u);
        *(volatile unsigned long long*)&pub[lane] = ((unsigned long long)tag << 32) | (unsigned long long)half;
        if (lane < 2) {
          const double le = stats_pass ? 0.0 : sh.O[43];
          const unsigned int eh = lane ? (unsigned int)__double2hiint(le) : (unsigned int)__double2loint(le);
          *(volatile unsigned long long*)&pub[32 + lane] = ((unsigned long long)tag << 32) | (unsigned long long)eh;
        }
      }
      if (!done) clear_replicas(my_slots, lane);
    }
    if (is_last) __syncthreads();
  }
  if (job.Mtab) {
    if (*(volatile int*)&pd->gn_error) return;
    const float* A = job.mode == GN_MAIN ? pd->invP_active.m : pd->invP_cur.m;
    float a[16];
#pragma unroll
    for (int i = 0; i < 16; ++i) a[i] = *(volatile const float*)&A[i];
    for (uint32_t t = blockIdx.x * blockDim.x + threadIdx.x; t < job.n_poses; t += gridDim.x * blockDim.x) {
      float b[16], c[16];
      load_mat_cg(job.poses, (int)t, b);
      mat4_mul<float>(a, b, c);
      float4* o = reinterpret_cast<float4*>(job.Mtab + 16 * (size_t)t);
      o[0] = make_float4(c[0], c[1], c[2], c[3]);
      o[1] = make_float4(c[4], c[5], c[6], c[7]);
      o[2] = make_float4(c[8], c[9], c[10], c[11]);
      o[3] = make_float4(c[12], c[13], c[14], c[15]);
    }
  }
}

int gn_persistent_max_blocks(int sm_count) {
  int per_sm = 0;
  int per_sm4 = 0;
  if (cudaOccupancyMaxActiveBlocksPerMultiprocessor(&per_sm, k_gn_persistent<2>, kIcpThreads, 0) != cudaSuccess) return 0;
  if (cudaOccupancyMaxActiveBlocksPerMultiprocessor(&per_sm4, k_gn_persistent<4>, kIcpThreads, 0) != cudaSuccess) return 0;
  return (per_sm < per_sm4 ? per_sm : per_sm4) * sm_count;
}

int launch_gn_persistent(const Launch& L, const KParams& kp, const GnJob& job, long long* slots, unsigned int* ticket,
                         unsigned long long* pub, const CommDev* comm, int blocks) {
  CommDev cd;
  if (comm) {
    cd = *comm;
  } else {
    memset(&cd, 0, sizeof(cd));
    cd.nranks = 1;
  }
  KParams kpv = kp;
  GnJob jv = job;
  void* args[] = {&kpv, &jv, &slots, &ticket, &pub, &cd};
  cudaError_t e;
  {
    ScopedKernel sk(L, job.mode == GN_POST ? K_ICP_POST : K_ICP_FUSED);
    const long long px = (long long)(job.a.row_end - job.a.row_begin) * kp.W, per_pass = (long long)blocks * kIcpThreads;
    const bool deep = job.use_cache && job.mode != GN_POST && px > 2 * per_pass && px <= 4 * per_pass;
    e = cudaLaunchCooperativeKernel(deep ? (void*)k_gn_persistent<4> : (void*)k_gn_persistent<2>, dim3(blocks),
                                    dim3(kIcpThreads), args, 0, L.stream);
  }
  return e == cudaSuccess ? 0 : -1;
}

}
```

semantic_suma_b200/csrc/sb_internal.cuh:

```cuda
#pragma once

#include <cuda.h>
#include <cuda_runtime.h>
#include <stdint.h>
#include <string.h>

#include <vector>

#include "../../include/suma_b200.h"
#include "sb_math.cuh"

namespace sb {

constexpr uint32_t kMaxSurfels = 2048u * 2048u;
constexpr uint32_t kMaxPoses = 10000u;
constexpr uint32_t kExtractCap = 500000u;
constexpr uint32_t kComposeAge = 100u;
constexpr int kMaxGnIter = 256;
constexpr uint32_t kTilePoolCap = 16u * 1024u * 1024u;
constexpr uint32_t kMaxTileSlots = 16384u;
constexpr int kGroupCounts = 256;

struct KParams {
  int W, H, Wm, Hm;
  float fov_up, fov, min_depth, max_depth;
  float m_fov_up, m_fov, m_min_depth, m_max_depth;
  int weighting, bilinear;
  float factor;
  int use_stability, unstable_age, confidence_mode, active_timestamps;
  int weighting_scheme, averaging_scheme, update_always;
  float confidence_threshold, p_stable, p_unstable, log_prior, log_unstable;
  float sigma_angle, sigma_distance, max_weight;
  float pixel_size, min_radius, max_radius, radconf_angle_thresh, update_angle_thresh, map_max_distance;
  float max_loop_closure_distance;
  int label_offset_quirk;
};

struct FrameDev {
  int W, H;
  float4* vertex;
  float4* normal;
  float4* semantic;
};

struct SurfelPlanes {
  float4* p0;
  float4* p1;
  float4* p2;
  float4* p3;
};

struct GnState {
  double pose[16];
  double last_error;
  double out48[48];
  int k;
  int done;
  int history_len;
  int error;
  double history[(kMaxGnIter + 1) * 16];
};

struct IcpArgs {
  const float4* data_v; const float4* data_n; const float4* data_s;
  const float4* model_v; const float4* model_n; const float4* model_s;
  float distance_thresh, angle_thresh;
  int row_begin, row_end;
  int has_semantics;
  int row_step;
  int Wm, Hm;
};

struct CommDev {
  int rank, nranks;
  long long* mailbox[8];
  unsigned int* epoch;
};

struct Mat4 {
  float m[16];
};
struct Mat4d {
  double m[16];
};

struct PoseDev {
  double currentPose[16], lastPose[16], lastIncrement[16], increment[16], T0[16];
  Mat4 P_active, invP_active;
  Mat4 P_cur, invP_cur;
  int fallback;
  int trackLoss;
  int icp_iterations;
  int gn_error;
  float t_err, r_err;
  int pad2[2];
};

enum KernelId {
  K_FILL = 0, K_PROJECT_SCATTER, K_PREPROCESS_TILE, K_ICP_JACOBIAN, K_GN_INIT,
  K_ICP_FUSED, K_POSE_PRODUCTS, K_RENDER_SCATTER, K_RENDER_RESOLVE, K_INDEX_SCATTER, K_RADIUS, K_UPDATE_SURFELS,
  K_GEN_SURFELS, K_EXTRACT_FLAGS, K_SCAN_BLOCKS, K_COMPACT_SCATTER, K_AOS_TO_SOA, K_SOA_TO_AOS, K_ICP_POST, K_COUNT
};
const char* kernel_name(int id);

struct Profiler {
  bool on = false;
  struct Rec { int id; cudaEvent_t e0, e1; };
  std::vector<Rec> recs;
  std::vector<cudaEvent_t> pool;
  cudaEvent_t get() {
    if (!pool.empty()) { cudaEvent_t e = pool.back(); pool.pop_back(); return e; }
    cudaEvent_t e; cudaEventCreate(&e); return e;
  }
};

struct Launch {
  cudaStream_t stream;
  uint64_t* counter;
  Profiler* prof;
};

struct ScopedKernel {
  const Launch& L;
  int slot = -1;
  ScopedKernel(const Launch& l, int id) : L(l) {
    ++*L.counter;
    if (L.prof && L.prof->on) {
      Profiler::Rec r{id, L.prof->get(), L.prof->get()};
      cudaEventRecord(r.e0, L.stream);
      L.prof->recs.push_back(r);
      slot = (int)L.prof->recs.size() - 1;
    }
  }
  ~ScopedKernel() {
    if (slot >= 0) cudaEventRecord(L.prof->recs[slot].e1, L.stream);
  }
};

struct PrepKeys {
  unsigned long long* img[2] = {nullptr, nullptr};
  int cur = 0;
  bool use_tma = false;
  bool tmap_ok[2] = {false, false};
  CUtensorMap tmap[2];
};
size_t preprocess_key_elems(int W, int H);
bool make_key_tensor_map(CUtensorMap* out, const unsigned long long* keys, int W, int H);
void launch_preprocess(const Launch& L, const KParams& kp, const float4* pts, const float* labels, const float* probs,
                       uint32_t n, uint32_t timestamp, PrepKeys& keys, FrameDev out, float4* radius_map,
                       unsigned long long* index_keys, uint8_t* integrated, uint32_t* group_counts);

void launch_icp_jacobian(const Launch& L, const KParams& kp, const IcpArgs& a, const Mat4& pose, int iteration,
                         long long* acc32, long long* slots, unsigned int* ticket, int blocks);
enum GnMode { GN_PLAIN = 0, GN_MAIN = 1, GN_POST = 2 };
struct GnJob {
  int mode;
  IcpArgs a;
  IcpArgs fb;
  GnState* st;
  PoseDev* pd;
  long long* stats32;
  float* poses; float* poses_inv; uint32_t t_map;
  float* Mtab; uint32_t n_poses;
  int initialize_identity, fallback_mode;
  uint32_t timestamp;
  int max_iter;
  double eps, delta;
  unsigned int epoch_base;
  int use_cache;
};
void launch_gn_init(const Launch& L, GnState* st, const Mat4d& T0, long long* acc32);
int launch_gn_persistent(const Launch& L, const KParams& kp, const GnJob& job, long long* slots, unsigned int* ticket,
                         unsigned long long* pub, const CommDev* comm, int blocks);
int gn_persistent_max_blocks(int sm_count);
void launch_pose_after_icp(const Launch& L, const GnState* gn, PoseDev* pd, const Mat4d& T0, uint32_t timestamp,
                           int fallback_mode);
void launch_pose_finalize(const Launch& L, const GnState* gn, PoseDev* pd, int had_icp, float* poses, float* poses_inv,
                          uint32_t t);
int icp_grid_blocks(int sm_count);
int icp_balanced_blocks(int pixels, int max_blocks);

struct RenderTargets {
  unsigned long long* key_old;
  unsigned long long* key_new;
  unsigned long long* key_comp;
};
void launch_pose_products(const Launch& L, const Mat4& A, const Mat4* A_dev, const float* poses, float* out,
                          uint32_t count);
void launch_render_scatter(const Launch& L, const KParams& kp, SurfelPlanes s, const uint32_t* n_dev, uint32_t n_upper,
                           const float* M, float conf_thr, int t_thr, int emit_old, int emit_new, int lequal,
                           RenderTargets t);
void launch_render_resolve(const Launch& L, const KParams& kp, SurfelPlanes s, const float* M_old, const float* M_new,
                           RenderTargets t, FrameDev f_old, FrameDev f_new, FrameDev f_comp, FrameDev f_out,
                           FrameDev f_copy, int keep_semantic, int lequal);
void launch_index_scatter(const Launch& L, const KParams& kp, SurfelPlanes s, const uint32_t* n_dev, uint32_t n_upper,
                          const float* M, unsigned long long* keys);
void launch_radius(const Launch& L, const KParams& kp, FrameDev frame, float4* radius_map, unsigned long long* index_keys,
                   uint8_t* integrated, uint32_t* group_counts);
void launch_compact_update(const Launch& L, SurfelPlanes src, const uint8_t* keep, const uint32_t* block_counts,
                           const uint32_t* group_counts, const uint32_t* n_dev, uint32_t n_upper, SurfelPlanes dst,
                           uint32_t cap, uint32_t* count_out, uint32_t* kept_out);
void launch_update_surfels(const Launch& L, const KParams& kp, SurfelPlanes src, SurfelPlanes tmp, const uint32_t* n_dev,
                           uint32_t n_upper, const Mat4& pose, const Mat4& inv_pose, const Mat4* pose_dev,
                           const Mat4* inv_pose_dev, const float* poses,
                           const float* poses_inv, const unsigned long long* index_keys, const float4* radius_map,
                           FrameDev frame, int timestamp, float2 submap_center, float submap_extent,
                           uint8_t* integrated, uint8_t* keep, uint32_t* block_counts, uint32_t* group_counts);
void launch_gen_compact(const Launch& L, const KParams& kp, FrameDev frame, const float4* radius_map,
                        const uint8_t* integrated, const float* poses, int timestamp, float2 submap_center,
                        float submap_extent, SurfelPlanes map, unsigned long long* desc, uint32_t* ticket, uint32_t gen,
                        uint32_t cap, uint32_t* counts);
void launch_extract_to_pool(const Launch& L, SurfelPlanes map, const uint32_t* n_dev, uint32_t n_upper, const float* poses,
                            float2 center, float extent, uint8_t* keep, uint32_t* block_counts, uint32_t* block_offsets,
                            SurfelPlanes pool, uint32_t pool_cap, uint32_t* pool_top, uint2* rec, uint32_t tile_cap);
void launch_extract_flags(const Launch& L, SurfelPlanes s, const uint32_t* n_dev, uint32_t n_upper, const float* poses,
                          float2 center, float extent, uint8_t* keep, uint32_t* block_counts);
void launch_aos_to_soa(const Launch& L, const sb_surfel* aos, SurfelPlanes s, uint32_t offset, uint32_t n);
void launch_soa_to_aos(const Launch& L, SurfelPlanes s, sb_surfel* aos, uint32_t n);

}
```

Measured before the change: 1866.

## Solve Gauss-Newton step in warp registers and add optional phase tracing

Replaces the shared-memory Gauss-Newton step with a register and warp-shuffle pivoted LDLT solve plus SE3 update, which shortens the serial step one warp runs between grid-wide ICP passes. It also stops rebalancing the cooperative block count and changes the cached-pixel indexing in the persistent kernel. An optional globaltimer trace, enabled through an environment variable, records per-pass phases and comes with a profiling script. The trace adds null checks on the hot path, and the shuffle-based solve must match the previous numerics.

Result: slower. 1838, median of 6 (-1.5%).

```diff
diff --git a/include/suma_b200.h b/include/suma_b200.h
--- a/include/suma_b200.h
+++ b/include/suma_b200.h
@@ -160,6 +160,8 @@
 const char* sb_profile_name(int id);
 int sb_profile_collect(sb_ctx* ctx, double* total_ms, uint64_t* count, int cap);
 
+long long sb_gn_trace_download(sb_ctx* ctx, uint64_t* out, long long cap);
+
 int sb_comm_export(sb_ctx* ctx, uint8_t handle[64]);
 int sb_comm_init(sb_ctx* ctx, int rank, int nranks, const uint8_t* handles , int row_begin,
                  int row_end);
diff --git a/profiles/gn_phases.py b/profiles/gn_phases.py
--- /dev/null
+++ b/profiles/gn_phases.py
@@ -0,0 +1,138 @@
+import argparse
+import json
+import os
+import statistics
+import sys
+
+ROOT = os.path.dirname(os.path.dirname(os.path.abspath(__file__)))
+sys.path.insert(0, ROOT)
+
+import numpy as np
+
+HEAD, ITERS, STEP = 16, 32, 4
+
+
+def parse(rec):
+    blocks, passes = int(rec[1]), int(rec[2])
+    n = min(passes, ITERS)
+    step = rec[HEAD:HEAD + ITERS * STEP].reshape(ITERS, STEP)[:n].astype(np.int64)
+    o = HEAD + ITERS * STEP
+    pas = rec[o:o + ITERS * blocks * 3].reshape(ITERS, blocks, 3)[:n].astype(np.int64)
+    o += ITERS * blocks * 3
+    blk = rec[o:o + blocks * 2].reshape(blocks, 2).astype(np.int64)
+    return dict(mode=int(rec[0]), blocks=blocks, passes=passes, head=rec[:HEAD].astype(np.int64), step=step, pas=pas,
+                blk=blk)
+
+
+def phases(r):
+    out = {}
+    step, pas, blk = r["step"], r["pas"], r["blk"]
+    rel = pas[:, :, 0]
+    acc = pas[:, :, 1]
+    tick = pas[:, :, 2]
+    n = step.shape[0]
+    for i in range(n):
+        row = {
+            "release_spread": rel[i].max() - rel[i].min(),
+            "accumulate_max": (acc[i] - rel[i]).max(),
+            "accumulate_median": int(np.median(acc[i] - rel[i])),
+            "reduce_and_ticket_median": int(np.median(tick[i] - acc[i])),
+            "straggler": tick[i].max() - np.median(tick[i]),
+            "sums_read": step[i, 1] - step[i, 0],
+            "step_solve": step[i, 2] - step[i, 1],
+            "publish": step[i, 3] - step[i, 2],
+        }
+        if i + 1 < n:
+            row["handover"] = rel[i + 1].min() - step[i, 3]
+            row["iteration"] = rel[i + 1].min() - rel[i].min()
+        out.setdefault("passes", []).append(row)
+    h = r["head"]
+    out["bookkeeping"] = h[5] - h[4]
+    out["final_publish_to_exit"] = blk[:, 1].max() - step[n - 1, 3]
+    out["launch_first_entry_to_first_release"] = rel[0].min() - blk[:, 0].min()
+    out["launch"] = blk[:, 1].max() - blk[:, 0].min()
+    return out
+
+
+def timer_resolution(records):
+    vals = []
+    for r in records:
+        for a in (r["pas"].reshape(-1), r["step"].reshape(-1), r["blk"].reshape(-1)):
+            vals.append(a[a > 0])
+    v = np.unique(np.concatenate(vals))
+    d = np.diff(v)
+    d = d[d > 0]
+    return int(d.min()) if d.size else 0, int(np.gcd.reduce(d)) if d.size else 0
+
+
+def main():
+    ap = argparse.ArgumentParser()
+    ap.add_argument("--workload", default="hdl64_2048_geometric")
+    ap.add_argument("--steps", type=int, default=40)
+    ap.add_argument("--warmup", type=int, default=5)
+    ap.add_argument("--preroll", type=int, default=60)
+    ap.add_argument("--out", default=None)
+    args = ap.parse_args()
+    os.environ["SUMA_B200_GN_TRACE"] = "1"
+    import bench
+    w = bench.WORKLOADS[args.workload]
+    pre = args.preroll + args.warmup
+    scans = bench.generate_scans(w, pre + args.steps, seed=1337)
+    import torch
+    from semantic_suma_b200 import api
+    slam = api.SurfelMapping(api.default_params(**bench.param_kwargs(w)), device=0)
+    ctx = slam.ctx
+    stream = torch.cuda.ExternalStream(ctx.stream(), device=0)
+    flush = torch.empty(256 * 1024 * 1024, dtype=torch.uint8, device="cuda")
+    dev = [torch.from_numpy(p).cuda() for p, _, _ in scans]
+    torch.cuda.synchronize()
+    slam.reset()
+    for f in range(pre):
+        slam.process_scan_raw(dev[f].data_ptr(), 0, 0, dev[f].shape[0], True)
+    ctx.synchronize()
+    if ctx.gn_trace() is None:
+        raise SystemExit("the persistent Gauss-Newton kernel is not in use on this device: nothing to trace")
+    recs = {1: [], 2: []}
+    for i in range(args.steps):
+        with torch.cuda.stream(stream):
+            flush.zero_()
+        f = pre + i
+        slam.process_scan_raw(dev[f].data_ptr(), 0, 0, dev[f].shape[0], True)
+        t = ctx.gn_trace()
+        words = t.size // 3
+        for mode in (1, 2):
+            r = parse(t[mode * words:(mode + 1) * words])
+            assert r["mode"] == mode
+            recs[mode].append(r)
+    res_min, res_gcd = timer_resolution(recs[1] + recs[2])
+    props = torch.cuda.get_device_properties(0)
+    report = {"device": props.name, "workload": args.workload, "steps": args.steps, "preroll": args.preroll,
+              "timer_min_step_ns": res_min, "timer_gcd_ns": res_gcd, "launches": {}}
+    for mode, name in ((1, "GN_MAIN"), (2, "GN_POST")):
+        ph = [phases(r) for r in recs[mode]]
+        blocks = recs[mode][0]["blocks"]
+        passes = statistics.median(r["passes"] for r in recs[mode])
+        keys = [k for k in ph[0]["passes"][0]]
+        per = {}
+        for k in keys + ["handover", "iteration"]:
+            xs = [p[k] for x in ph for p in x["passes"] if k in p]
+            if xs:
+                per[k] = round(statistics.median(xs) / 1000.0, 3)
+        tail = {k: round(statistics.median(x[k] for x in ph) / 1000.0, 3)
+                for k in ("bookkeeping", "final_publish_to_exit", "launch_first_entry_to_first_release", "launch")}
+        report["launches"][name] = {"blocks": blocks, "passes": passes, "per_pass_median_us": per, "once_us": tail}
+    print("device %s, %d timed scans, timer: smallest step %d ns, gcd %d ns" %
+          (report["device"], args.steps, res_min, res_gcd))
+    for name, L in report["launches"].items():
+        print("%s: %d blocks, %s passes, launch %.2f us" % (name, L["blocks"], L["passes"], L["once_us"]["launch"]))
+        for k, v in L["per_pass_median_us"].items():
+            print("  %-28s %10.3f us" % (k, v))
+        for k, v in L["once_us"].items():
+            print("  %-36s %10.3f us" % (k, v))
+    if args.out:
+        with open(args.out, "w") as f:
+            json.dump(report, f, indent=1)
+
+
+if __name__ == "__main__":
+    main()
diff --git a/semantic_suma_b200/api.py b/semantic_suma_b200/api.py
--- a/semantic_suma_b200/api.py
+++ b/semantic_suma_b200/api.py
@@ -145,6 +145,8 @@
     L.sb_launch_count.argtypes = [vp]; L.sb_launch_count.restype = C.c_uint64
     L.sb_device_count.argtypes = []; L.sb_device_count.restype = C.c_int
     L.sb_profile_name.argtypes = [C.c_int]; L.sb_profile_name.restype = C.c_char_p
+    L.sb_gn_trace_download.argtypes = [vp, C.POINTER(C.c_uint64), C.c_longlong]
+    L.sb_gn_trace_download.restype = C.c_longlong
     L.sb_se3_exp.argtypes = [pd, pd]; L.sb_se3_exp.restype = None
     L.sb_se3_log.argtypes = [pd, pd]; L.sb_se3_log.restype = None
     L.sb_icp_unpack.argtypes = [C.POINTER(C.c_int64), pd]; L.sb_icp_unpack.restype = None
@@ -163,7 +165,7 @@
     "sb_get_statistics", "sb_comm_export", "sb_comm_init", "sb_comm_shutdown", "sb_comm_set_callback",
     "sb_profile_enable", "sb_default_loop_params", "sb_set_loop_closure", "sb_get_loop_info", "sb_get_loop_edges",
     "sb_set_current_pose", "sb_integrate_loop_closures",
-    "sb_profile_kernels", "sb_profile_name", "sb_profile_collect",
+    "sb_profile_kernels", "sb_profile_name", "sb_profile_collect", "sb_gn_trace_download",
 ]
 
 
@@ -245,6 +247,18 @@
         ms = np.zeros(n); cnt = np.zeros(n, np.uint64)
         self.check(lib().sb_profile_collect(self.h, _dp(ms), cnt.ctypes.data_as(C.POINTER(C.c_uint64)), n), "profile")
         return {lib().sb_profile_name(i).decode(): (float(ms[i]), int(cnt[i])) for i in range(n) if cnt[i]}
+
+    def gn_trace(self):
+        n = lib().sb_gn_trace_download(self.h, None, 0)
+        if n < 0:
+            self.check(int(n), "gn_trace")
+        if n == 0:
+            return None
+        a = np.zeros(n, np.uint64)
+        n2 = lib().sb_gn_trace_download(self.h, a.ctypes.data_as(C.POINTER(C.c_uint64)), n)
+        if n2 < 0:
+            self.check(int(n2), "gn_trace")
+        return a
 
     def set_params(self, params):
         self.check(lib().sb_set_params(self.h, C.byref(params)), "set_params")
diff --git a/semantic_suma_b200/csrc/sb_api.cu b/semantic_suma_b200/csrc/sb_api.cu
--- a/semantic_suma_b200/csrc/sb_api.cu
+++ b/semantic_suma_b200/csrc/sb_api.cu
@@ -67,6 +67,7 @@
   unsigned int epoch_base = 1;
   unsigned long long* gn_pub = nullptr;
   int gn_use_cache = 1;
+  unsigned long long* gn_trace = nullptr;
   bool close_loops = false;
   suma_b200::loop::State loop;
   double lastPose_old[16];
@@ -239,6 +240,7 @@
   cudaFree(c->prep.img[0]); cudaFree(c->prep.img[1]);
   cudaFree(c->d_pts); cudaFree(c->d_labels); cudaFree(c->d_probs);
   cudaFree(c->gn); cudaFree(c->gn2); cudaFree(c->acc_slots); cudaFree(c->ticket); cudaFree(c->gn_pub);
+  cudaFree(c->gn_trace);
   if (c->h_pinned) cudaFreeHost(c->h_pinned);
   free_planes(&c->A); free_planes(&c->T); free_planes(&c->G); free_planes(&c->X); free_planes(&c->pool);
   cudaFree(c->d_pool_top); cudaFree(c->d_tile_rec);
@@ -329,6 +331,13 @@
   SB_CUDA(c, cudaMalloc(&c->gn_pub, 64 * 8));
   SB_CUDA(c, cudaMemsetAsync(c->gn_pub, 0, 64 * 8, c->stream));
   if (const char* e = getenv("SUMA_B200_GN_CACHE")) c->gn_use_cache = atoi(e) != 0;
+  if (const char* e = getenv("SUMA_B200_GN_TRACE")) {
+    if (atoi(e) != 0 && c->icp_coop_blocks > 0) {
+      const size_t words = 3 * gn_trace_words(c->icp_coop_blocks);
+      SB_CUDA(c, cudaMalloc(&c->gn_trace, words * 8));
+      SB_CUDA(c, cudaMemsetAsync(c->gn_trace, 0, words * 8, c->stream));
+    }
+  }
   SB_CUDA(c, cudaMemsetAsync(c->ticket, 0, 128, c->stream));
   SB_CUDA(c, cudaMallocHost(&c->h_pinned, 65536));
   int r;
@@ -618,6 +627,7 @@
     job.delta = delta;
     job.epoch_base = next_epoch_base(c, max_iter);
     job.use_cache = c->gn_use_cache;
+    job.trace = c->gn_trace;
     if (launch_gn_persistent(L, c->kp, job, c->acc_slots, c->ticket, c->gn_pub, c->comm_on ? &c->comm : nullptr,
                              c->icp_coop_blocks) == 0)
       return SB_OK;
@@ -923,6 +933,7 @@
     job.delta = p.delta;
     job.epoch_base = next_epoch_base(c, max_iter);
     job.use_cache = c->gn_use_cache;
+    job.trace = c->gn_trace;
     if (launch_gn_persistent(L, c->kp, job, c->acc_slots, c->ticket, c->gn_pub, c->comm_on ? &c->comm : nullptr,
                              c->icp_coop_blocks) != 0) {
       cudaGetLastError();
@@ -950,6 +961,7 @@
     post.delta = p.delta;
     post.epoch_base = next_epoch_base(c, max_iter);
     post.use_cache = 0;
+    post.trace = c->gn_trace;
     if (launch_gn_persistent(L, c->kp, post, c->acc_slots, c->ticket, c->gn_pub, c->comm_on ? &c->comm : nullptr,
                              c->icp_coop_blocks) != 0) {
       cudaGetLastError();
@@ -1143,7 +1155,6 @@
     cudaDeviceGetAttribute(&coop, cudaDevAttrCooperativeLaunch, device);
     int maxb = coop ? gn_persistent_max_blocks(c->sm_count) : 0;
     c->icp_coop_blocks = maxb < c->icp_blocks ? maxb : c->icp_blocks;
-    if (c->icp_coop_blocks > 0) c->icp_coop_blocks = icp_balanced_blocks(p->data_width * p->data_height, c->icp_coop_blocks);
     c->icp_blocks = icp_balanced_blocks(p->data_width * p->data_height, c->icp_blocks);
     if (getenv("SUMA_B200_NO_PERSISTENT_GN")) c->icp_coop_blocks = 0;
     if (getenv("SUMA_B200_ICP_BLOCKS")) {
@@ -1739,6 +1750,17 @@
   return SB_OK;
 }
 int sb_profile_kernels(void) { return K_COUNT; }
+long long sb_gn_trace_download(sb_ctx* c, uint64_t* out, long long cap) {
+  if (!c) return SB_ERR_INVALID;
+  if (!c->gn_trace) return 0;
+  const long long words = 3 * (long long)gn_trace_words(c->icp_coop_blocks);
+  if (out && cap >= words) {
+    cudaSetDevice(c->device);
+    SB_CUDA(c, cudaStreamSynchronize(c->stream));
+    SB_CUDA(c, cudaMemcpy(out, c->gn_trace, (size_t)words * 8, cudaMemcpyDeviceToHost));
+  }
+  return words;
+}
 const char* sb_profile_name(int id) { return kernel_name(id); }
 int sb_profile_collect(sb_ctx* c, double* total_ms, uint64_t* count, int cap) {
   if (!c || !total_ms || !count || cap < K_COUNT) return SB_ERR_INVALID;
diff --git a/semantic_suma_b200/csrc/sb_icp.cu b/semantic_suma_b200/csrc/sb_icp.cu
--- a/semantic_suma_b200/csrc/sb_icp.cu
+++ b/semantic_suma_b200/csrc/sb_icp.cu
@@ -373,25 +373,6 @@
   }
 }
 
-struct GnShared {
-  double A[36];
-  double O[48];
-  double P[16];
-  double E[16];
-  double dx[6];
-  int perm[6];
-  int result;
-};
-
-__device__ __forceinline__ void tri_cr(int k, int& c, int& r) {
-  const int start[6] = {0, 6, 11, 15, 18, 20};
-  c = 0;
-#pragma unroll
-  for (int i = 1; i < 6; ++i)
-    if (k >= start[i]) c = i;
-  r = c + (k - start[c]);
-}
-
 __device__ __forceinline__ unsigned long long globaltimer_ns() {
   unsigned long long t;
   asm volatile("mov.u64 %0, %%globaltimer;" : "=l"(t));
@@ -399,126 +380,176 @@
 }
 constexpr unsigned long long kSpinTimeoutNs = 10ull * 1000ull * 1000ull * 1000ull;
 
-__device__ void gn_step_warp(GnShared& sh, long long raw, int lane, double last_error, double eps, double delta_thr) {
-  const double s = 1.0 / 1073741824.0;
+constexpr unsigned kFull = 0xffffffffu;
+
+__host__ __device__ constexpr int tri_idx(int r, int c) { return c * 6 - (c * (c - 1)) / 2 + (r - c); }
+__device__ __forceinline__ void tri_cr(int k, int& c, int& r) {
+  c = (k >= 6) + (k >= 11) + (k >= 15) + (k >= 18) + (k >= 20);
+  r = c + (k - tri_idx(c, c));
+}
+template <int N>
+__device__ __forceinline__ double pick(const double (&v)[N], int i) {
+  double x = v[0];
+#pragma unroll
+  for (int j = 1; j < N; ++j)
+    if (i == j) x = v[j];
+  return x;
+}
+
+__device__ __forceinline__ int gn_step_lanes(long long raw, int lane, const double* P, double last_error, double eps,
+                                             double delta_thr, double& o, double& pn) {
+  o = lane < 29 ? (double)raw * (1.0 / 1073741824.0) : (double)raw;
+  int r = 0, c = 0;
+  if (lane < 21) tri_cr(lane, c, r);
+  double v = lane < 21 ? o : -o;
+  int perm = lane - 21;
+#pragma unroll
+  for (int k = 0; k < 6; ++k) {
+    double d[6];
+#pragma unroll
+    for (int i = k; i < 6; ++i) d[i] = __shfl_sync(kFull, v, tri_idx(i, i));
+    int piv = k;
+    double best = fabs(d[k]), dk = d[k];
+#pragma unroll
+    for (int i = k + 1; i < 6; ++i) {
+      double a = fabs(d[i]);
+      if (a > best) {
+        best = a;
+        piv = i;
+        dk = d[i];
+      }
+    }
+    if (piv != k) {
+      int src = lane;
+      if (lane < 21) {
+        const int rr = r == k ? piv : r == piv ? k : r, cc = c == k ? piv : c == piv ? k : c;
+        src = rr > cc ? tri_idx(rr, cc) : tri_idx(cc, rr);
+      } else if (lane < 27) {
+        const int i = lane - 21;
+        src = 21 + (i == k ? piv : i == piv ? k : i);
+      }
+      v = __shfl_sync(kFull, v, src);
+      perm = __shfl_sync(kFull, perm, src);
+    }
+    if (dk == 0.0) continue;
+    if (lane < 21 && c == k && r > k) v = v / dk;
+    const bool upd = lane < 21 && c > k;
+    const double lik = __shfl_sync(kFull, v, upd ? tri_idx(r, k) : lane);
+    const double ljk = __shfl_sync(kFull, v, upd ? tri_idx(c, k) : lane);
+    if (upd) v = v - (lik * dk) * ljk;
+  }
+  double maxc = __shfl_sync(kFull, o, 21);
+#pragma unroll
+  for (int i = 0; i < 6; ++i) {
+    const double bi = __shfl_sync(kFull, o, 21 + i);
+    if (bi > maxc) maxc = bi;
+  }
+  double L[21], y[6];
+  int pm[6];
+#pragma unroll
+  for (int j = 0; j < 21; ++j) L[j] = __shfl_sync(kFull, v, j);
+#pragma unroll
+  for (int i = 0; i < 6; ++i) {
+    y[i] = __shfl_sync(kFull, v, 21 + i);
+    pm[i] = __shfl_sync(kFull, perm, 21 + i);
+  }
+#pragma unroll
+  for (int i = 0; i < 6; ++i)
+#pragma unroll
+    for (int k = 0; k < i; ++k) y[i] = y[i] - L[tri_idx(i, k)] * y[k];
+  {
+    double diag[6];
+#pragma unroll
+    for (int i = 0; i < 6; ++i) diag[i] = L[tri_idx(i, i)];
+    const double di = pick(diag, lane), yi = pick(y, lane);
+    const double q = (di == 0.0) ? 0.0 : yi / di;
+#pragma unroll
+    for (int i = 0; i < 6; ++i) y[i] = __shfl_sync(kFull, q, i);
+  }
+#pragma unroll
+  for (int i = 5; i >= 0; --i)
+#pragma unroll
+    for (int k = i + 1; k < 6; ++k) y[i] = y[i] - L[tri_idx(k, i)] * y[k];
+  double dx[6];
+#pragma unroll
+  for (int j = 0; j < 6; ++j) {
+    dx[j] = 0.0;
+#pragma unroll
+    for (int i = 0; i < 6; ++i)
+      if (pm[i] == j) dx[j] = y[i];
+  }
+  int result = 1;
+  double linf = 0.0;
+#pragma unroll
+  for (int i = 0; i < 6; ++i)
+    if (fabs(dx[i]) > linf) linf = fabs(dx[i]);
+  const double current_error = __shfl_sync(kFull, o, 27);
+  if (linf < delta_thr) result = 0;
+  if (fabs(maxc) < eps) result = 0;
+  if (current_error < last_error && fabs(current_error - last_error) < eps) result = 0;
+  double E[16];
+#pragma unroll
+  for (int i = 0; i < 16; ++i) E[i] = (i % 5 == 0) ? 1.0 : 0.0;
+  const double v0 = dx[0], v1 = dx[1], v2 = dx[2], w0 = dx[3], w1 = dx[4], w2 = dx[5];
+  const double theta = sqrt((w0 * w0 + w1 * w1) + w2 * w2);
+  if (theta > 1e-10) {
+    const double K[9] = {0, -w2, w1, w2, 0, -w0, -w1, w0, 0};
+    double K2[9];
+#pragma unroll
+    for (int rr = 0; rr < 3; ++rr)
+#pragma unroll
+      for (int cc = 0; cc < 3; ++cc)
+        K2[rr * 3 + cc] = (K[rr * 3 + 0] * K[0 * 3 + cc] + K[rr * 3 + 1] * K[1 * 3 + cc]) + K[rr * 3 + 2] * K[2 * 3 + cc];
+    double sn, cs;
+    sbm::sincos_(theta, &sn, &cs);
+    const double num = lane == 0 ? sn : lane == 1 ? (1.0 - cs) : (theta - sn);
+    const double den = lane == 0 ? theta : lane == 1 ? (theta * theta) : ((theta * theta) * theta);
+    const double q = num / den;
+    const double alpha = __shfl_sync(kFull, q, 0), beta = __shfl_sync(kFull, q, 1), delta = __shfl_sync(kFull, q, 2);
+    const double gamma = beta;
+    double V[9];
+#pragma unroll
+    for (int rr = 0; rr < 3; ++rr)
+#pragma unroll
+      for (int cc = 0; cc < 3; ++cc) {
+        const double I = (rr == cc) ? 1.0 : 0.0;
+        E[cc * 4 + rr] = (I + alpha * K[rr * 3 + cc]) + beta * K2[rr * 3 + cc];
+        V[rr * 3 + cc] = (I + gamma * K[rr * 3 + cc]) + delta * K2[rr * 3 + cc];
+      }
+    E[12] = (V[0] * v0 + V[1] * v1) + V[2] * v2;
+    E[13] = (V[3] * v0 + V[4] * v1) + V[5] * v2;
+    E[14] = (V[6] * v0 + V[7] * v1) + V[8] * v2;
+  } else {
+    E[12] = v0;
+    E[13] = v1;
+    E[14] = v2;
+  }
+  pn = 0.0;
+  if (lane < 16) {
+    const int cc = lane >> 2, rr = lane & 3;
+    double e[4];
+#pragma unroll
+    for (int k = 0; k < 4; ++k) {
+      double col[4] = {E[k * 4 + 0], E[k * 4 + 1], E[k * 4 + 2], E[k * 4 + 3]};
+      e[k] = pick(col, rr);
+    }
+    pn = ((e[0] * P[cc * 4 + 0] + e[1] * P[cc * 4 + 1]) + e[2] * P[cc * 4 + 2]) + e[3] * P[cc * 4 + 3];
+  }
+  return result;
+}
+
+__device__ __forceinline__ void store_out48(double* out48, int lane, double o) {
   if (lane < 21) {
     int c, r;
     tri_cr(lane, c, r);
-    double v = (double)raw * s;
-    sh.O[c * 6 + r] = v;
-    sh.O[r * 6 + c] = v;
+    out48[c * 6 + r] = o;
+    out48[r * 6 + c] = o;
   } else if (lane < 27) {
-    sh.O[36 + (lane - 21)] = (double)raw * s;
-  } else if (lane == 27) {
-    sh.O[43] = (double)raw * s;
-  } else if (lane == 28) {
-    sh.O[45] = (double)raw * s;
-  } else if (lane == 29) {
-    sh.O[42] = (double)raw;
-  } else if (lane == 30) {
-    sh.O[44] = (double)raw;
+    out48[36 + (lane - 21)] = o;
   } else {
-    sh.O[46] = (double)raw;
-    sh.O[47] = 0.0;
-  }
-  __syncwarp();
-  double* A = sh.A;
-  for (int i = lane; i < 36; i += 32) A[i] = sh.O[i];
-  if (lane < 6) sh.perm[lane] = lane;
-  __syncwarp();
-#pragma unroll 1
-  for (int k = 0; k < 6; ++k) {
-    int piv = k;
-    double best = fabs(A[k * 6 + k]);
-    for (int i = k + 1; i < 6; ++i) {
-      double v = fabs(A[i * 6 + i]);
-      if (v > best) {
-        best = v;
-        piv = i;
-      }
-    }
-    __syncwarp();
-    if (piv != k) {
-      if (lane < 6) {
-        double t = A[k * 6 + lane];
-        A[k * 6 + lane] = A[piv * 6 + lane];
-        A[piv * 6 + lane] = t;
-      }
-      __syncwarp();
-      if (lane < 6) {
-        double t = A[lane * 6 + k];
-        A[lane * 6 + k] = A[lane * 6 + piv];
-        A[lane * 6 + piv] = t;
-      }
-      if (lane == 0) {
-        int t = sh.perm[k];
-        sh.perm[k] = sh.perm[piv];
-        sh.perm[piv] = t;
-      }
-      __syncwarp();
-    }
-    double dk = A[k * 6 + k];
-    if (dk == 0.0) continue;
-    if (lane > k && lane < 6) A[k * 6 + lane] = A[k * 6 + lane] / dk;
-    __syncwarp();
-    if (lane < 21) {
-      int c, r;
-      tri_cr(lane, c, r);
-      if (c > k) {
-        double v = A[c * 6 + r] - (A[k * 6 + r] * dk) * A[k * 6 + c];
-        A[c * 6 + r] = v;
-        A[r * 6 + c] = v;
-      }
-    }
-    __syncwarp();
-  }
-  if (lane == 0) {
-    double y[6], dx[6];
-#pragma unroll
-    for (int i = 0; i < 6; ++i) y[i] = -sh.O[36 + sh.perm[i]];
-#pragma unroll
-    for (int i = 0; i < 6; ++i)
-#pragma unroll
-      for (int k = 0; k < i; ++k) y[i] = y[i] - A[k * 6 + i] * y[k];
-#pragma unroll
-    for (int i = 0; i < 6; ++i) y[i] = (A[i * 6 + i] == 0.0) ? 0.0 : y[i] / A[i * 6 + i];
-#pragma unroll
-    for (int i = 5; i >= 0; --i)
-#pragma unroll
-      for (int k = i + 1; k < 6; ++k) y[i] = y[i] - A[i * 6 + k] * y[k];
-#pragma unroll
-    for (int i = 0; i < 6; ++i) sh.dx[sh.perm[i]] = y[i];
-#pragma unroll
-    for (int i = 0; i < 6; ++i) dx[i] = sh.dx[i];
-    int result = 1;
-    double current_error = sh.O[43];
-    double linf = 0.0, maxc = sh.O[36];
-#pragma unroll
-    for (int i = 0; i < 6; ++i) {
-      if (fabs(dx[i]) > linf) linf = fabs(dx[i]);
-      if (sh.O[36 + i] > maxc) maxc = sh.O[36 + i];
-    }
-    if (linf < delta_thr) result = 0;
-    if (fabs(maxc) < eps) result = 0;
-    if (current_error < last_error && fabs(current_error - last_error) < eps) result = 0;
-    sh.result = result;
-    double E[16];
-    sbg::se3_exp(dx, E);
-#pragma unroll
-    for (int i = 0; i < 16; ++i) sh.E[i] = E[i];
-  }
-  __syncwarp();
-  double pn = 0.0;
-  if (lane < 16) {
-    int c = lane >> 2, r = lane & 3;
-    const double* Ea = sh.E;
-    const double* B = sh.P;
-    pn = ((Ea[0 * 4 + r] * B[c * 4 + 0] + Ea[1 * 4 + r] * B[c * 4 + 1]) + Ea[2 * 4 + r] * B[c * 4 + 2]) +
-         Ea[3 * 4 + r] * B[c * 4 + 3];
-  }
-  __syncwarp();
-  if (lane < 16) sh.P[lane] = pn;
-  __syncwarp();
+    out48[lane == 27 ? 43 : lane == 28 ? 45 : lane == 29 ? 42 : lane == 30 ? 44 : 46] = o;
+    if (lane == 31) out48[47] = 0.0;
+  }
 }
 
 __device__ bool comm_allreduce32_warp(const CommDev& cd, long long& raw, int lane) {
@@ -570,27 +601,57 @@
   M[12] = d.x; M[13] = d.y; M[14] = d.z; M[15] = d.w;
 }
 
+struct GnTrace {
+  unsigned long long* p;
+  int G;
+  __device__ __forceinline__ unsigned long long* step(unsigned it) const {
+    return it < (unsigned)kGnTraceIters ? p + kGnTraceHead + (size_t)it * kGnTraceStep : nullptr;
+  }
+  __device__ __forceinline__ unsigned long long* pass(unsigned it) const {
+    return it < (unsigned)kGnTraceIters
+               ? p + kGnTraceHead + (size_t)kGnTraceIters * kGnTraceStep + ((size_t)it * G + blockIdx.x) * 3
+               : nullptr;
+  }
+  __device__ __forceinline__ unsigned long long* block() const {
+    return p + kGnTraceHead + (size_t)kGnTraceIters * kGnTraceStep + (size_t)kGnTraceIters * G * 3 + (size_t)blockIdx.x * 2;
+  }
+};
+__device__ __forceinline__ unsigned long long stamp_after(long long dep) {
+  return dep != (long long)0x8000000000000001ull ? globaltimer_ns() : 0ull;
+}
+
+__device__ __forceinline__ void block_pixels(const IcpArgs& a, int W, int& b0, int& b1) {
+  const long long base = (long long)a.row_begin * W, n = (long long)(a.row_end - a.row_begin) * W;
+  b0 = (int)(base + n * blockIdx.x / gridDim.x);
+  b1 = (int)(base + n * (blockIdx.x + 1) / gridDim.x);
+}
+
 template <int kGnCachePix>
 __global__ void __launch_bounds__(kIcpThreads, 2) k_gn_persistent(KParams kp, GnJob job, long long* __restrict__ slots,
                                                                unsigned int* ticket, unsigned long long* pub,
                                                                CommDev cd) {
-  __shared__ GnShared sh;
   __shared__ bool is_last;
   __shared__ double s_pose[16];
+  __shared__ double s_next[16];
   __shared__ double s_last_error;
   __shared__ int s_done, s_error;
   __shared__ float4 s_dv[kGnCachePix][kIcpThreads], s_dn[kGnCachePix][kIcpThreads];
   const int lane = threadIdx.x & 31, warp = threadIdx.x >> 5;
   GnState* st = job.st;
   PoseDev* pd = job.pd;
-  if (threadIdx.x == 0) s_error = 0;
-  const int px_begin = job.a.row_begin * kp.W, px_end = job.a.row_end * kp.W;
-  const int px_stride = gridDim.x * blockDim.x, px_first = px_begin + blockIdx.x * blockDim.x + threadIdx.x;
-  const bool cached = job.use_cache && job.mode != GN_POST && (px_end - px_begin) <= kGnCachePix * px_stride;
+  const GnTrace tr{job.trace ? job.trace + (size_t)job.mode * gn_trace_words(gridDim.x) : nullptr, (int)gridDim.x};
+  if (threadIdx.x == 0) {
+    s_error = 0;
+    if (tr.p) tr.block()[0] = globaltimer_ns();
+  }
+  int px_begin, px_end;
+  block_pixels(job.a, kp.W, px_begin, px_end);
+  const bool cached = job.use_cache && job.mode != GN_POST &&
+                      (long long)(job.a.row_end - job.a.row_begin) * kp.W <= (long long)kGnCachePix * gridDim.x * blockDim.x;
   if (cached) {
 #pragma unroll
     for (int j = 0; j < kGnCachePix; ++j) {
-      const int pix = px_first + j * px_stride;
+      const int pix = px_begin + (int)threadIdx.x + j * (int)blockDim.x;
       if (pix < px_end) {
         s_dv[j][threadIdx.x] = __ldg(job.a.data_v + pix);
         s_dn[j][threadIdx.x] = __ldg(job.a.data_n + pix);
@@ -627,19 +688,20 @@
           w = *(volatile unsigned long long*)&pub[lane];
           if (lane < 2) w2 = *(volatile unsigned long long*)&pub[32 + lane];
         }
-        if (__any_sync(0xffffffffu, timed_out)) {
+        if (__any_sync(kFull, timed_out)) {
           if (lane == 0) s_error = 1;
         }
-        const unsigned int lo = __shfl_sync(0xffffffffu, (unsigned int)w, 2 * (lane & 15));
-        const unsigned int hi = __shfl_sync(0xffffffffu, (unsigned int)w, 2 * (lane & 15) + 1);
+        const unsigned int lo = __shfl_sync(kFull, (unsigned int)w, 2 * (lane & 15));
+        const unsigned int hi = __shfl_sync(kFull, (unsigned int)w, 2 * (lane & 15) + 1);
         if (lane < 16) s_pose[lane] = __hiloint2double((int)hi, (int)lo);
         if (lane == 17) s_done = (int)((w >> 63) & 1ull);
-        const unsigned int e_lo = __shfl_sync(0xffffffffu, (unsigned int)w2, 0);
-        const unsigned int e_hi = __shfl_sync(0xffffffffu, (unsigned int)w2, 1);
+        const unsigned int e_lo = __shfl_sync(kFull, (unsigned int)w2, 0);
+        const unsigned int e_hi = __shfl_sync(kFull, (unsigned int)w2, 1);
         if (lane == 18) s_last_error = __hiloint2double((int)e_hi, (int)e_lo);
       }
     }
     __syncthreads();
+    if (tr.p && threadIdx.x == 0 && tr.pass(it)) tr.pass(it)[0] = globaltimer_ns();
     if (s_error) {
       if (threadIdx.x == 0) {
         *(volatile int*)&st->error = 1;
@@ -659,32 +721,45 @@
 #pragma unroll
     for (int i = 0; i < 16; ++i) M[i] = (float)s_pose[i];
     Acc acc;
+#pragma unroll
+    for (int i = 0; i < 29; ++i) acc.s[i] = 0;
+    acc.n_valid = acc.n_outlier = acc.n_invalid = 0;
     if (cached) {
 #pragma unroll
-      for (int i = 0; i < 29; ++i) acc.s[i] = 0;
-      acc.n_valid = acc.n_outlier = acc.n_invalid = 0;
-#pragma unroll
       for (int j = 0; j < kGnCachePix; ++j) {
-        const int pix = px_first + j * px_stride;
+        const int pix = px_begin + (int)threadIdx.x + j * (int)blockDim.x;
         if (pix < px_end) icp_pixel_v(kp, job.a, M, pix, s_dv[j][threadIdx.x], s_dn[j][threadIdx.x], k, acc);
       }
     } else {
-      icp_accumulate(kp, recovery ? job.fb : job.a, M, stats_pass ? 0 : k, acc);
+      const IcpArgs& a = recovery ? job.fb : job.a;
+      int b0, b1;
+      block_pixels(a, kp.W, b0, b1);
+      for (int pix = b0 + (int)threadIdx.x; pix < b1; pix += blockDim.x) icp_pixel(kp, a, M, pix, stats_pass ? 0 : k, acc);
     }
     __syncthreads();
+    if (tr.p && threadIdx.x == 0 && tr.pass(it)) tr.pass(it)[1] = globaltimer_ns();
     block_reduce_to_replica(acc, my_slots);
     __syncthreads();
     if (threadIdx.x == 0) {
       __threadfence();
       unsigned int t = atomicAdd(ticket, 1u);
       is_last = (t == (it + 1u) * gridDim.x - 1u);
+      if (tr.p && tr.pass(it)) {
+        const unsigned long long ts = stamp_after(t);
+        tr.pass(it)[2] = ts;
+        if (is_last) tr.step(it)[0] = ts;
+      }
     }
     __syncthreads();
     if (is_last && warp == 0) {
       __threadfence();
       long long raw = sum_replicas(my_slots, lane);
+      if (tr.p && lane == 0 && tr.step(it)) {
+        tr.step(it)[1] = stamp_after(raw);
+      }
       int done = 0, error = 0;
       double pv = 0.0;
+      double err = 0.0;
       if (stats_pass) {
         job.stats32[lane] = raw;
         const int fb = job.fallback_mode ? *(volatile int*)&pd->fallback : 0;
@@ -705,44 +780,47 @@
         double last_error = (double)3.402823466e+38f;
         if (k > 0) last_error = s_last_error;
         if (cd.epoch) error = comm_allreduce32_warp(cd, raw, lane) ? 0 : 1;
-        if (lane < 16) sh.P[lane] = s_pose[lane];
         int hl = k;
         if (lane < 16) st->history[hl * 16 + lane] = s_pose[lane];
         ++hl;
-        __syncwarp();
-        gn_step_warp(sh, raw, lane, last_error, job.eps, job.delta);
-        if (lane < 16) {
-          pv = sh.P[lane];
-          st->pose[lane] = pv;
-        }
-        for (int i = lane; i < 48; i += 32) st->out48[i] = sh.O[i];
+        double o;
+        const int result = gn_step_lanes(raw, lane, s_pose, last_error, job.eps, job.delta, o, pv);
+        if (tr.p && lane == 0 && tr.step(it)) {
+          tr.step(it)[2] = stamp_after(((long long)__double2hiint(pv) << 32) | (unsigned int)__double2loint(pv));
+        }
+        err = __shfl_sync(kFull, o, 27);
+        if (lane < 16) st->pose[lane] = pv;
+        store_out48(st->out48, lane, o);
         int kk = k;
-        if (sh.result == 0) {
+        if (result == 0) {
           done = 1;
         } else {
           ++kk;
           if (kk >= job.max_iter) {
-            if (lane < 16) st->history[hl * 16 + lane] = sh.P[lane];
+            if (lane < 16) st->history[hl * 16 + lane] = pv;
             ++hl;
             done = 1;
           }
         }
         if (error) done = 1;
         if (lane == 0) {
-          st->last_error = sh.O[43];
+          st->last_error = err;
           st->k = kk;
           st->history_len = hl;
         }
+        if (lane < 16) s_next[lane] = pv;
         __syncwarp();
       }
       if (done && lane == 0 && !error) {
+        if (tr.p) tr.p[4] = globaltimer_ns();
         if (job.mode == GN_MAIN) {
           double T0[16];
           for (int i = 0; i < 16; ++i) T0[i] = job.initialize_identity ? ((i % 5 == 0) ? 1.0 : 0.0) : pd->lastIncrement[i];
-          pose_after_icp_body(sh.P, st->k, pd, T0, job.timestamp, job.fallback_mode);
+          pose_after_icp_body(s_next, st->k, pd, T0, job.timestamp, job.fallback_mode);
         } else if (job.mode == GN_POST) {
           pose_finalize_body(st->pose, pd, 1, job.poses, job.poses_inv, job.t_map);
         }
+        if (tr.p) tr.p[5] = globaltimer_ns();
       }
       if (lane == 0) {
         if (error) {
@@ -751,6 +829,12 @@
         }
         st->done = done;
         if (done) *ticket = 0;
+        if (done && tr.p) {
+          tr.p[0] = job.mode;
+          tr.p[1] = gridDim.x;
+          tr.p[2] = it + 1u;
+          tr.p[3] = kGnTraceIters;
+        }
       }
       if (done) {
         clear_replicas(my_slots, lane);
@@ -758,16 +842,16 @@
       }
       __syncwarp();
       {
-        const double src = __shfl_sync(0xffffffffu, pv, lane >> 1);
+        const double src = __shfl_sync(kFull, pv, lane >> 1);
         const unsigned int half = (lane & 1) ? (unsigned int)__double2hiint(src) : (unsigned int)__double2loint(src);
         const unsigned int tag = ((job.epoch_base + it + 1u) & 0x7fffffffu) | (done ? 0x80000000u : 0u);
         *(volatile unsigned long long*)&pub[lane] = ((unsigned long long)tag << 32) | (unsigned long long)half;
         if (lane < 2) {
-          const double le = stats_pass ? 0.0 : sh.O[43];
-          const unsigned int eh = lane ? (unsigned int)__double2hiint(le) : (unsigned int)__double2loint(le);
+          const unsigned int eh = lane ? (unsigned int)__double2hiint(err) : (unsigned int)__double2loint(err);
           *(volatile unsigned long long*)&pub[32 + lane] = ((unsigned long long)tag << 32) | (unsigned long long)eh;
         }
       }
+      if (tr.p && lane == 0 && tr.step(it)) tr.step(it)[3] = globaltimer_ns();
       if (!done) clear_replicas(my_slots, lane);
     }
     if (is_last) __syncthreads();
@@ -789,6 +873,7 @@
       o[3] = make_float4(c[12], c[13], c[14], c[15]);
     }
   }
+  if (tr.p && threadIdx.x == 0) tr.block()[1] = globaltimer_ns();
 }
 
 int gn_persistent_max_blocks(int sm_count) {
diff --git a/semantic_suma_b200/csrc/sb_internal.cuh b/semantic_suma_b200/csrc/sb_internal.cuh
--- a/semantic_suma_b200/csrc/sb_internal.cuh
+++ b/semantic_suma_b200/csrc/sb_internal.cuh
@@ -168,7 +168,12 @@
   double eps, delta;
   unsigned int epoch_base;
   int use_cache;
-};
+  unsigned long long* trace;
+};
+constexpr int kGnTraceHead = 16, kGnTraceIters = 32, kGnTraceStep = 4;
+SB_HD size_t gn_trace_words(int blocks) {
+  return kGnTraceHead + (size_t)kGnTraceIters * kGnTraceStep + (size_t)kGnTraceIters * blocks * 3 + (size_t)blocks * 2;
+}
 void launch_gn_init(const Launch& L, GnState* st, const Mat4d& T0, long long* acc32);
 int launch_gn_persistent(const Launch& L, const KParams& kp, const GnJob& job, long long* slots, unsigned int* ticket,
                          unsigned long long* pub, const CommDev* comm, int blocks);
```
